# shoeffner/ann3depth

Hardware: AMD Instinct MI355X
Metric: images/sec (640x480->55x74 MSDN train step) (higher is better)
Workload: dtype f32

## Files before the change

### ann3depth_amd/_lib.py

```python
import ctypes
import os
from ctypes import c_char_p, c_float, c_int, c_int32, c_int64, c_size_t, c_uint8, c_uint32, c_void_p, POINTER

LIB_PATH = os.environ.get('A3D_LIB') or os.path.join(os.path.dirname(os.path.abspath(__file__)), 'liba3d.so')


class A3dError(RuntimeError):
    pass


class ConvDesc(ctypes.Structure):
    _fields_ = [(n, c_int32) for n in ('n', 'h', 'w', 'c', 'k', 'r', 's', 'stride', 'pad_t', 'pad_l', 'ho', 'wo',
                                       'ldx', 'ldy', 'precision', 'storage', 'hints')]


class SecondOutput(ctypes.Structure):
    _fields_ = [('ptr', c_void_p), ('ld', c_int32), ('step', c_int32), ('offset', c_int32), ('bf16', c_int32), ('cols', c_int32)]


class ExampleView(ctypes.Structure):
    _fields_ = [('image_height', c_int64), ('image_width', c_int64), ('image_channels', c_int64),
                ('depth_height', c_int64), ('depth_width', c_int64), ('depth_channels', c_int64),
                ('image', c_void_p), ('image_bytes', c_size_t), ('depth', c_void_p), ('depth_bytes', c_size_t)]


class TimingRecord(ctypes.Structure):
    _fields_ = [(n, c_int32) for n in ('mode', 'bm', 'bn', 'waves_m', 'nwaves', 'bk', 'avec', 'bvec', 'prec', 'lds_dma', 'splitk', 'm', 'n', 'k')] + \
               [('ms', c_float), ('flops', ctypes.c_double)]


_P = c_void_p
_D = POINTER(ConvDesc)

SIGNATURES = {
    'a3d_version': (c_char_p, []),
    'a3d_last_error': (c_int, [c_char_p, c_size_t]),
    'a3d_conv2d_fwd_ws_bytes': (c_size_t, [_D]),
    'a3d_conv2d_fwd': (c_int, [_D, _P, _P, _P, _P, c_int, _P, c_size_t, _P]),
    'a3d_conv2d_bwd_data_ws_bytes': (c_size_t, [_D]),
    'a3d_conv2d_bwd_data': (c_int, [_D, _P, _P, _P, _P, _P, c_size_t, _P]),
    'a3d_conv2d_bwd_filter_ws_bytes': (c_size_t, [_D]),
    'a3d_conv2d_bwd_filter': (c_int, [_D, _P, _P, _P, _P, _P, c_size_t, _P]),
    'a3d_conv2d_fwd_prepared_filter_bytes': (c_size_t, [_D]),
    'a3d_conv2d_fwd_prepare_filter': (c_int, [_D, _P, _P, c_size_t, _P]),
    'a3d_conv2d_bwd_filter_pooled_ws_bytes': (c_size_t, [_D]),
    'a3d_conv2d_bwd_filter_pooled': (c_int, [_D, _P, _P, c_int, _P, _P, c_int, c_int, _P, _P, _P, c_size_t, _P]),
    'a3d_conv2d_bwd_both_supported': (c_int, [_D]),
    'a3d_conv2d_bwd_both_ws_bytes': (c_size_t, [_D]),
    'a3d_conv2d_bwd_both': (c_int, [_D, _P, _P, _P, _P, _P, _P, c_int, c_int, c_int, _P, _P, c_size_t, _P]),
    'a3d_dense_fwd_ws_bytes': (c_size_t, [c_int, c_int, c_int]),
    'a3d_dense_fwd': (c_int, [c_int, c_int, c_int, _P, _P, _P, _P, c_int, _P, _P, c_size_t, _P]),
    'a3d_dense_bwd_data_ws_bytes': (c_size_t, [c_int, c_int, c_int]),
    'a3d_dense_bwd_data': (c_int, [c_int, c_int, c_int, _P, _P, _P, _P, c_int, c_float, _P, c_size_t, _P]),
    'a3d_dense_bwd_filter_ws_bytes': (c_size_t, [c_int, c_int, c_int]),
    'a3d_dense_bwd_filter': (c_int, [c_int, c_int, c_int, _P, _P, _P, _P, _P, c_size_t, _P]),
    'a3d_maxpool2x2_fwd': (c_int, [c_int, c_int, c_int, c_int, _P, _P, c_int, _P, _P]),
    'a3d_maxpool2x2_bwd': (c_int, [c_int, c_int, c_int, c_int, _P, _P, c_int, _P, c_int, _P]),
    'a3d_resize_bilinear_tf1': (c_int, [c_int, c_int, c_int, c_int, _P, c_int, c_int, _P, _P]),
    'a3d_resize_bilinear_tf1_pair': (c_int, [c_int, c_int, c_int, c_int, _P, c_int, c_int, _P, c_int, _P, c_int, c_int, _P, _P]),
    'a3d_resize_bilinear_tf1_ex': (c_int, [c_int, c_int, c_int, c_int, _P, c_int, c_int, c_int, _P, c_int, _P, c_int, c_int, c_int,
                                           _P, _P]),
    'a3d_warp_bilinear_pair': (c_int, [c_int, c_int, c_int, c_int, _P, c_int, c_int, c_int, _P, c_int, _P, c_int, c_int, c_int,
                                       _P, _P, _P]),
    'a3d_extract_patches': (c_int, [c_int, c_int, c_int, c_int, _P, c_int, c_int, _P, _P]),
    'a3d_silog_loss_fwd': (c_int, [c_int, c_int, _P, _P, _P, _P, _P]),
    'a3d_silog_loss_bwd': (c_int, [c_int, c_int, _P, _P, _P, _P, _P]),
    'a3d_dropout_keep_mask': (c_int, [c_size_t, ctypes.c_uint64, ctypes.c_uint64, c_float, _P, _P]),
    'a3d_adam_apply_tf1': (c_int, [c_size_t, _P, _P, _P, _P, c_float, c_float, c_float, c_float, c_float, c_float,
                                   c_float, _P]),
    'a3d_adam_apply_tf1_flag': (c_int, [c_size_t, _P, _P, _P, _P, c_float, c_float, c_float, c_float, c_float, c_float,
                                        c_float, _P, _P]),
    'a3d_dense_fwd_ex': (c_int, [c_int, c_int, c_int, _P, _P, _P, _P, c_int, _P, c_int, c_int, _P, c_size_t, _P]),
    'a3d_dense_bwd_data_ex': (c_int, [c_int, c_int, c_int, _P, _P, _P, _P, c_int, c_float, c_int, c_int, _P, c_size_t, _P]),
    'a3d_dense_fwd_ex2': (c_int, [c_int, c_int, c_int, _P, _P, _P, _P, c_int, c_int, c_int, _P, c_int, c_int, POINTER(SecondOutput), _P,
                                  c_size_t, _P]),
    'a3d_dense_bwd_data_ex2': (c_int, [c_int, c_int, c_int, _P, _P, _P, _P, c_int, c_float, c_int, c_int, POINTER(SecondOutput), _P,
                                       c_size_t, _P]),
    'a3d_conv2d_fwd_ex2': (c_int, [_D, _P, _P, _P, _P, c_int, POINTER(SecondOutput), _P, c_size_t, _P]),
    'a3d_silog_loss_bwd_ex': (c_int, [c_int, c_int, _P, _P, _P, _P, _P, c_int, _P]),
    'a3d_depth_metrics_ws_bytes': (c_size_t, [c_int, c_int, c_int]),
    'a3d_depth_metrics': (c_int, [c_int, c_int, c_int, _P, c_int, c_int, _P, c_int, c_float, c_float, c_float, c_float, _P, _P,
                                  c_size_t, _P]),
    'a3d_cast_bf16': (c_int, [c_size_t, _P, _P, c_int, _P]),
    'a3d_cast_rows': (c_int, [c_size_t, c_int, _P, c_int, c_int, _P, c_int, c_int, _P]),
    'a3d_pad_channels_bf16': (c_int, [c_size_t, c_int, _P, c_int, _P, _P]),
    'a3d_stream_create': (c_int, [c_int, ctypes.POINTER(ctypes.c_void_p)]),
    'a3d_stream_destroy': (c_int, [_P]),
    'a3d_maxpool2x2_fwd_bf16': (c_int, [c_int, c_int, c_int, c_int, _P, c_int, _P, c_int, _P, _P]),
    'a3d_maxpool2x2_bwd_bf16': (c_int, [c_int, c_int, c_int, c_int, _P, c_int, _P, c_int, _P, c_int, _P]),
    'a3d_copy_channel_bf16': (c_int, [c_size_t, _P, c_int, c_int, _P, c_int, c_int, _P]),
    'a3d_maxpool2x2_bwd_idx_bf16': (c_int, [c_int, c_int, c_int, c_int, _P, _P, c_int, _P, c_int, _P, c_int, _P]),
    'a3d_maxpool2x2_bwd_idx_bf16s': (c_int, [c_int, c_int, c_int, c_int, _P, _P, c_int, _P, c_int, _P, c_int, _P]),
    'a3d_dense_bwd_filter_adam_tf1': (c_int, [c_int, c_int, c_int, _P, _P, _P, _P, _P, _P, _P, _P, c_float, c_float, c_float,
                                              c_float, c_float, c_float, _P]),
    'a3d_dense_bwd_filter_adam_tf1_ex': (c_int, [c_int, c_int, c_int, _P, _P, _P, _P, _P, _P, _P, _P, c_float, c_float, c_float,
                                                 c_float, c_float, c_float, c_int, _P]),
    'a3d_superpixel_mean': (c_int, [c_int, c_int, c_int, c_int, _P, c_int, _P, _P]),
    'a3d_superpixel_hist': (c_int, [c_int, c_int, c_int, _P, c_int, _P, _P]),
    'a3d_pair_similarity': (c_int, [c_int, c_int, c_int, _P, c_int, _P, _P, _P, c_int, _P, _P, c_float, _P, _P, _P]),
    'a3d_crf_loss': (c_int, [c_int, c_int, _P, _P, _P, _P, _P, c_int, c_float, _P, _P, _P, _P]),
    'a3d_crf_map': (c_int, [c_int, c_int, _P, _P, _P, _P, c_int, _P, _P, _P]),
    'a3d_sgd_apply': (c_int, [c_size_t, _P, _P, c_float, _P]),
    'a3d_conv2d_pool_fwd': (c_int, [_D, _P, _P, _P, _P, c_int, _P, c_int, _P, c_size_t, _P]),
    'a3d_maxpool2x2_bwd_idx': (c_int, [c_int, c_int, c_int, c_int, _P, _P, c_int, _P, c_int, _P, c_int, _P]),
    'a3d_copy_channel': (c_int, [c_size_t, _P, c_int, c_int, _P, c_int, c_int, _P]),
    'a3d_comm_standin': (c_int, [_P, c_size_t, _P, c_size_t, c_int, c_float, _P]),
    'a3d_timing_enable': (c_int, [c_int]),
    'a3d_timing_collect': (c_int, [POINTER(TimingRecord), c_int]),
    'a3d_timing_select': (c_int, [POINTER(TimingRecord)]),
    'a3d_crc32c': (c_uint32, [_P, c_size_t]),
    'a3d_masked_crc32c': (c_uint32, [_P, c_size_t]),
    'a3d_tfrecord_next': (c_int, [_P, c_size_t, c_int, POINTER(c_size_t), POINTER(c_size_t), POINTER(c_size_t)]),
    'a3d_example_parse': (c_int, [_P, c_size_t, POINTER(ExampleView)]),
    'a3d_decode_raw_plus_half': (c_int, [_P, c_size_t, _P]),
    'a3d_record_decode': (c_int, [_P, c_size_t, c_int, _P, c_size_t, _P, c_size_t, POINTER(ExampleView)]),
    'a3d_record_decode_u8': (c_int, [_P, c_size_t, c_int, _P, _P, c_size_t, _P, _P, c_size_t, POINTER(ExampleView),
                                     POINTER(c_int)]),
    'a3d_records_decode': (c_int, [POINTER(c_void_p), POINTER(c_size_t), c_int, c_int, POINTER(c_int64), _P, _P, _P, _P,
                                   POINTER(c_int32), c_int, POINTER(c_int32)]),
    'a3d_h2d_gather': (c_int, [_P, _P, POINTER(c_int32), c_int, c_int, c_size_t, _P]),
    'a3d_sizeof_conv_desc': (c_size_t, []),
    'a3d_example_write': (c_int64, [_P, c_int, c_int, c_int, _P, c_int, c_int, c_int, _P, c_size_t]),
}

EXT_SIGNATURES = {
    'a3dx_resize_bilinear_tf1_valid': (c_int, [c_int, c_int, c_int, c_int, _P, c_int, c_int, c_int, _P, c_int, _P, c_int, c_int,
                                               c_int, _P, c_float, c_float, _P]),
    'a3dx_warp_bilinear_pair_valid': (c_int, [c_int, c_int, c_int, c_int, _P, c_int, c_int, c_int, _P, c_int, _P, c_int, c_int,
                                              c_int, _P, _P, c_float, c_float, _P]),
    'a3dx_silog_masked_loss_fwd': (c_int, [c_int, c_int, _P, _P, _P, _P, _P]),
    'a3dx_silog_masked_loss_bwd_ex': (c_int, [c_int, c_int, _P, _P, _P, _P, _P, c_int, _P]),
}

PAIR_SIGNATURES = {
    'a3dp_crf_loss_grad': (c_int, [c_int, c_int, _P, _P, _P, _P, _P, c_int, c_float, _P, _P, _P, _P, _P]),
    'a3dp_pair_dense_bwd': (c_int, [c_int, c_int, c_int, _P, _P, _P, _P, _P]),
    'a3dp_sgd_apply_floor': (c_int, [c_size_t, _P, _P, c_float, c_float, _P]),
}

TEXTURE_SIGNATURES = {
    'a3dt_superpixel_lbp_hist': (c_int, [c_int, c_int, c_int, _P, c_int, _P, _P]),
    'a3dt_pair_similarity3': (c_int, [c_int, c_int, c_int, _P, c_int, _P, _P, _P, _P, c_int, _P, _P, c_float, _P, _P, _P]),
}

GRADLOSS_SIGNATURES = {
    'a3dg_silog_grad_loss_fwd': (c_int, [c_int, c_int, c_int, _P, _P, c_int, c_float, _P, _P, _P]),
    'a3dg_silog_grad_loss_bwd_ex': (c_int, [c_int, c_int, c_int, _P, _P, c_int, c_float, _P, _P, _P, c_int, _P]),
}

CRF_VALID_SIGNATURES = {
    'a3dv_superpixel_mean_valid': (c_int, [c_int, c_int, c_int, _P, c_int, c_int, _P, _P, _P]),
    'a3dv_crf_loss_observed': (c_int, [c_int, c_int, _P, _P, _P, _P, _P, c_int, _P, _P, _P, _P, _P, _P, _P]),
}

FCSP_SIGNATURES = {
    'a3df_superpixel_pool_fwd': (c_int, [c_int, c_int, c_int, c_int, _P, c_int, c_int, c_int, c_int, _P, _P, _P, c_int, _P]),
    'a3df_superpixel_pool_bwd': (c_int, [c_int, c_int, c_int, c_int, _P, c_int, c_int, c_int, c_int, _P, _P, _P, c_int, _P]),
}

CRF_BAND_SIGNATURES = {
    'a3db_crf_band_nll': (c_int, [c_int, c_int, c_int, _P, _P, _P, _P, _P, c_int, _P, _P, _P, _P, _P, _P, _P]),
    'a3db_crf_band_map': (c_int, [c_int, c_int, c_int, _P, _P, _P, _P, c_int, _P, _P, _P]),
}

_lib = None


def load():
    global _lib
    if _lib is not None:
        return _lib
    if not os.path.exists(LIB_PATH):
        raise A3dError(f'{LIB_PATH} not found: build it with `python -c "import __graft_entry__ as g; g.build()"` '
                       f'or `make -C ann3depth_amd/csrc` (there is no fallback path)')
    import torch
    lib = ctypes.CDLL(LIB_PATH)
    for name, (res, args) in (list(SIGNATURES.items()) + list(EXT_SIGNATURES.items()) + list(PAIR_SIGNATURES.items())
                              + list(TEXTURE_SIGNATURES.items()) + list(GRADLOSS_SIGNATURES.items())
                              + list(CRF_VALID_SIGNATURES.items()) + list(FCSP_SIGNATURES.items())
                              + list(CRF_BAND_SIGNATURES.items())):
        try:
            fn = getattr(lib, name)
        except AttributeError as e:
            raise A3dError(f'liba3d.so lacks symbol {name}: stale build?') from e
        fn.restype = res
        fn.argtypes = args
    if lib.a3d_sizeof_conv_desc() != ctypes.sizeof(ConvDesc):
        raise A3dError(f'liba3d.so reads a {lib.a3d_sizeof_conv_desc()}-byte a3d_conv_desc, this binding passes '
                       f'{ctypes.sizeof(ConvDesc)} bytes: stale build?')
    _lib = lib
    return lib


def last_error():
    buf = ctypes.create_string_buffer(512)
    load().a3d_last_error(buf, 512)
    return buf.value.decode(errors='replace')


def check(rc, what):
    if rc != 0:
        raise A3dError(f'{what} failed ({rc}): {last_error()}')
```

### ann3depth_amd/csrc/a3d_internal.h

```cpp
#pragma once
#include <hip/hip_runtime.h>
#include <stddef.h>
#include <stdint.h>

#include <algorithm>

#include "../../include/a3d.h"
#include "igemm_plan.h"

namespace a3d {

int set_error(int code, const char* fmt, ...);

#define A3D_CHECK_ARG(cond, ...)                                 \
  do {                                                           \
    if (!(cond)) return ::a3d::set_error(A3D_EINVAL, __VA_ARGS__); \
  } while (0)

inline void clear_stale_error() { (void)hipGetLastError(); }

inline int check_launch(const char* what) {
  hipError_t e = hipGetLastError();
  if (e != hipSuccess) return set_error(A3D_ELAUNCH, "%s: %s", what, hipGetErrorString(e));
  return A3D_OK;
}

inline unsigned grid_for(size_t total, int per_block = 256, unsigned cap = 8192) {
  size_t g = (total + per_block - 1) / per_block;
  return (unsigned)std::min<size_t>(std::max<size_t>(g, 1), cap);
}

inline bool aligned16(const void* p) { return (reinterpret_cast<uintptr_t>(p) & 15) == 0; }

struct IgemmParams;
int launch_igemm(int mode, const GemmPlan& plan, int avec, int bvec, IgemmParams& p, void* ws, hipStream_t st);
int take_second_output(IgemmParams& p, const a3d_second_output* o);

struct TimingSlot {
  hipEvent_t start, stop;
  a3d_timing_record rec;
};
bool timing_wanted(const a3d_timing_record& r);
int timing_begin(TimingSlot& slot, hipStream_t st);
void timing_end(TimingSlot& slot, hipStream_t st);
a3d_timing_record timing_record(int mode, int prec, int bm, int bn, int waves_m, int nwaves, int bk, int avec, int bvec, int lds_dma,
                                int m, int n, int k);
template <typename Launch>
int timed_launch(const a3d_timing_record& rec, hipStream_t st, Launch&& launch) {
  if (!timing_wanted(rec)) return launch();
  TimingSlot slot{};
  slot.rec = rec;
  int rc = timing_begin(slot, st);
  if (rc != A3D_OK) return rc;
  rc = launch();
  timing_end(slot, st);
  return rc;
}

bool dense_dw_applicable(int m, int k, int n);
bool dense_stream_applicable(int m, int k, int n);
size_t dense_stream_ws_bytes(int m, int k, int n);
int dense_fwd_stream(int m, int k, int n, const float* x, const float* w, const float* bias, float* y, int act,
                     const uint8_t* keep, float keep_scale, void* ws, size_t ws_bytes, hipStream_t st);
struct ReduceParams;
int launch_splitk_reduce(const ReduceParams& r, hipStream_t st);
int dense_dw_launch(int m, int k, int n, const float* x, const float* dz, float* dw, float* db, hipStream_t st);

size_t colsum_bf16_ws_bytes(int n);
bool colsum_bf16_ok(int n);
int colsum_bf16(const void* dz, int rows, int n, int ld, float* out, void* ws, int* nparts, hipStream_t st);

bool stencil1_applicable(const a3d_conv_desc* d);
size_t stencil1_bwdf_ws_bytes(const a3d_conv_desc* d);
int stencil1_fwd(const a3d_conv_desc* d, const float* x, const float* w, const float* bias, float* y, int act,
                 hipStream_t st);
int stencil1_bwd_filter(const a3d_conv_desc* d, const float* x, const float* dz, float* dw, float* db, void* ws,
                        hipStream_t st);
bool stencil1_bwd_both_applicable(const a3d_conv_desc* d);
size_t stencil1_bwd_both_ws_bytes(const a3d_conv_desc* d);
int stencil1_bwd_both(const a3d_conv_desc* d, const float* x, const float* dz, const float* w, float* dw, float* db,
                      void* dx, int lddx, int dx_bf16, int relu_mask, unsigned* state, void* ws, hipStream_t st);

bool fewch_bwdf_applicable(const a3d_conv_desc* d, bool pooled);
size_t fewch_bwdf_ws_bytes(const a3d_conv_desc* d, bool pooled);
bool fewch_extents_ok(const a3d_conv_desc* d, bool pooled, int ldz, int esz, int ld_arg);
int fewch_bwd_filter(const a3d_conv_desc* d, const float* x, int src, const void* dz, int ldz, const void* pooled_act,
                     const uint8_t* argmax, int ld_arg, float* dw, float* db, void* ws, hipStream_t st);

int fewch_reduce_launch(const float* slabs, int splits, int Mp, int NP, int M, int N, float* dw, float* db, hipStream_t st);
bool fewch16_bwdf_applicable(const a3d_conv_desc* d, bool pooled);
size_t fewch16_bwdf_ws_bytes(const a3d_conv_desc* d, bool pooled);
int fewch16_bwd_filter(const a3d_conv_desc* d, const float* x, bool pooled, const void* dz, int ldz, const void* pooled_act,
                       const uint8_t* argmax, int ld_arg, float* dw, float* db, void* ws, hipStream_t st);

bool conv3_applicable(const a3d_conv_desc* d, unsigned x_off);
size_t conv3_ws_bytes(const a3d_conv_desc* d);
int conv3_pack(const a3d_conv_desc* d, const float* w, float* wp, hipStream_t st);
int conv3_fwd(const a3d_conv_desc* d, const float* x, const float* w, const float* bias, float* y, int act, int pool,
              int ld_out, uint8_t* argmax, void* ws, size_t ws_bytes, hipStream_t st, bool prepared = false);

bool conv3b_applicable(const a3d_conv_desc* d);
size_t conv3b_filter_bytes(const a3d_conv_desc* d);
int conv3b_pack(const a3d_conv_desc* d, const float* w, void* wp, hipStream_t st);
int conv3b_fwd(const a3d_conv_desc* d, const void* x, const float* w, const float* bias, void* y, int act, int pool, int ld_out,
               uint8_t* argmax, void* ws, size_t ws_bytes, hipStream_t st, bool prepared);

}
```

### ann3depth_amd/csrc/dense.hip

```cpp
#include <algorithm>
#include <cmath>
#include <cstdlib>

#include "a3d_internal.h"
#include "igemm.h"

namespace a3d {


template <int CW>
struct VecOf;
template <>
struct VecOf<4> { typedef float type __attribute__((ext_vector_type(4), aligned(4))); };
template <>
struct VecOf<2> { typedef float type __attribute__((ext_vector_type(2), aligned(4))); };

template <bool ADAM, int CW>
__global__ __launch_bounds__(256) void dense_dw_kernel(const float* __restrict__ x, const float* __restrict__ dz,
                                                       float* __restrict__ dw, float* __restrict__ db,
                                                       float* __restrict__ var_w, float* __restrict__ m_w,
                                                       float* __restrict__ v_w, float* __restrict__ var_b,
                                                       float* __restrict__ m_b, float* __restrict__ v_b, int M, int K,
                                                       int N, float omb1, float gscale) {
  typedef typename VecOf<CW>::type vec;
// ... 390 lines not shown
      m_b[col] = mn;
      const bool poison = !isfinite(__fmul_rn(g, g));
      if (poison) v_b[col] = qnan;
      if (poison || !isfinite(mn)) var_b[col] = qnan;
    }
  }
  __syncthreads();

  for (int g = g0; g < g1; ++g) {
    f32x16 acc[G][CW];
#pragma unroll
    for (int gq = 0; gq < G; ++gq)
#pragma unroll
      for (int j = 0; j < CW; ++j)
#pragma unroll
        for (int v = 0; v < 16; ++v) acc[gq][j][v] = 0.f;
    if constexpr (BF) {
#pragma unroll
      for (int t = 0; t < 4; ++t) {
        const dbf16x8 a = *reinterpret_cast<const dbf16x8*>(&xsb[li * XLD + 16 * t + 8 * lh]);
#pragma unroll
        for (int gq = 0; gq < G; ++gq)
#pragma unroll
          for (int j = 0; j < CW; ++j)
            acc[gq][j] = __builtin_amdgcn_mfma_f32_32x32x16_bf16(a, bqb[t][gq][j], acc[gq][j], 0, 0, 0);
      }
    } else {
#pragma unroll
    for (int u = 0; u < TSTEPS; ++u) {
      const float a = xs[(2 * u + lh) * 32 + li];
#pragma unroll
      for (int gq = 0; gq < G; ++gq)
#pragma unroll
        for (int j = 0; j < CW; ++j)
          acc[gq][j] = __builtin_amdgcn_mfma_f32_32x32x2f32(a, bq[u][gq][j], acc[gq][j], 0, 0, 0);
    }
    }
#pragma unroll
    for (int hh = 0; hh < 2; ++hh) {
      if (hh) __syncthreads();
#pragma unroll
      for (int gq = 0; gq < G; ++gq)
#pragma unroll
        for (int vv = 0; vv < 8; ++vv) {
          vec t;
#pragma unroll
          for (int j = 0; j < CW; ++j) t[j] = acc[gq][j][8 * hh + vv];
          *reinterpret_cast<vec*>(&tile[((vv & 3) + 8 * (vv >> 2) + 4 * lh) * TLD + wave * WCOLS + (32 * gq + li) * CW]) = t;
        }
      __syncthreads();
      if (hh == 0) {
        load_x(xv, g + 1);
        __builtin_amdgcn_sched_barrier(0);
      }
#pragma unroll
      for (int r = 4 * hh; r < 4 * hh + 4; ++r) {
        const __amdgpu_buffer_rsrc_t rr = row_rsrc(g, r), rn = row_rsrc(g + 1, r);
        const int row = 32 * g + wrow(r);
#pragma unroll
        for (int h = 0; h < NI; ++h) {
          const int c = (h * 64 + lane) * CW;
          const vec g4 = *reinterpret_cast<const vec*>(&tile[(4 * wave + (r & 3)) * TLD + c]);
          const uint32_t off = piece_off(h);
          uvec mn;
          float chk = 0.f;
#pragma unroll
          for (int j = 0; j < CW; ++j) {
            const float gr = use_scale ? __fmul_rn(g4[j], gscale) : g4[j];
            const float mo = mreg[NI * r + h][j];
            const float t = __fadd_rn(mo, __fmul_rn(__fsub_rn(gr, mo), omb1));
            mn[j] = __float_as_uint(t);
            chk += __fmul_rn(gr, gr) + fabsf(t);
          }
          if constexpr (CW == 4) __builtin_amdgcn_raw_buffer_store_b128(mn, rr, (int)off, 0, kAuxStream);
          else __builtin_amdgcn_raw_buffer_store_b64(mn, rr, (int)off, 0, kAuxStream);
          load_vec_buf<CW, kAuxStream>(rn, off, mreg[NI * r + h]);
          if (!isfinite(chk) & (off != kOOB) & (row < K)) {
#pragma unroll
            for (int j = 0; j < CW; ++j) {
              const float gr = use_scale ? __fmul_rn(g4[j], gscale) : g4[j];
              const bool poison = !isfinite(__fmul_rn(gr, gr));
              const size_t o = (size_t)row * N + nb + c + j;
              if (poison) v_w[o] = qnan;
              if (poison || !isfinite(__uint_as_float(mn[j]))) var_w[o] = qnan;
            }
          }
        }
      }
    }
    park_x(xv);
    __syncthreads();
  }
}

typedef float f32x4a __attribute__((ext_vector_type(4), aligned(4)));

struct DenseStreamParams {
  const float* x;
  const float* w;
  float* out;
  const float* bias;
  const uint8_t* keep;
  const float* mask;
  float scale;
  int act;
  int M, K, N, splits, span;
};

template <int MB>
__global__ __launch_bounds__(256) void dense_fwd_stream_kernel(const DenseStreamParams p) {
  __shared__ __attribute__((aligned(16))) float red[4 * 16 * 132];
  const int tid = threadIdx.x, lane = tid & 63, wave = tid >> 6, li = lane & 31, lh = lane >> 5;
  const int n0 = blockIdx.x * 128, split = blockIdx.y;
  const int kb0 = split * p.span, kb1 = min(p.K, kb0 + p.span);
  const int wspan = ((kb1 - kb0 + 3) / 4 + 15) / 16 * 16;
  const int k0 = kb0 + wave * wspan, k1 = min(kb1, k0 + wspan);
  const __amdgpu_buffer_rsrc_t rw = make_rsrc(p.w, (unsigned long long)p.K * p.N * 4ull);
  const __amdgpu_buffer_rsrc_t rx = make_rsrc(p.x, (unsigned long long)p.M * p.K * 4ull);
  const int col0 = n0 + 4 * li;

  f32x16 acc[MB][4];
#pragma unroll
  for (int b = 0; b < MB; ++b)
#pragma unroll
    for (int c = 0; c < 4; ++c)
#pragma unroll
      for (int v = 0; v < 16; ++v) acc[b][c][v] = 0.f;

  constexpr int U = MB == 1 ? 2 : 1, ROWS = 8 * U;
  struct Chunk { float w[U][4][4]; float a[MB][U][4]; };
  auto load = [&](Chunk& c, int kc) {
#pragma unroll
    for (int u = 0; u < U; ++u) {
#pragma unroll
      for (int j = 0; j < 4; ++j) {
        const int k = kc + 8 * u + 4 * lh + j;
        load_vec_buf<4, kAuxStream>(rw, ((k < k1) & (col0 < p.N)) ? (uint32_t)(((size_t)k * p.N + col0) * 4) : kOOB, c.w[u][j]);
      }
#pragma unroll
      for (int b = 0; b < MB; ++b) {
        const int m = 32 * b + li, k = kc + 8 * u + 4 * lh;
        load_vec_buf<4>(rx, ((m < p.M) & (k < k1)) ? (uint32_t)(((size_t)m * p.K + k) * 4) : kOOB, c.a[b][u]);
      }
    }
  };
  auto compute = [&](const Chunk& c) {
#pragma unroll
    for (int u = 0; u < U; ++u)
#pragma unroll
      for (int j = 0; j < 4; ++j)
#pragma unroll
        for (int b = 0; b < MB; ++b)
#pragma unroll
          for (int e = 0; e < 4; ++e)
            acc[b][e] = __builtin_amdgcn_mfma_f32_32x32x2f32(c.a[b][u][j], c.w[u][j][e], acc[b][e], 0, 0, 0);
  };
  if (k0 < k1) {
    Chunk ca, cb;
    load(ca, k0);
    for (int kc = k0; kc < k1; kc += 2 * ROWS) {
      load(cb, kc + ROWS);
      compute(ca);
      load(ca, kc + 2 * ROWS);
      compute(cb);
    }
  }

#pragma unroll
  for (int b = 0; b < MB; ++b) {
#pragma unroll
    for (int hh = 0; hh < 2; ++hh) {
      if (b || hh) __syncthreads();
      float* mine = red + wave * (16 * 132);
#pragma unroll
      for (int vv = 0; vv < 8; ++vv) {
        const int v = 8 * hh + vv;
        const f32x4 q = {acc[b][0][v], acc[b][1][v], acc[b][2][v], acc[b][3][v]};
        *reinterpret_cast<f32x4*>(mine + ((vv & 3) + 8 * (vv >> 2) + 4 * lh) * 132 + 4 * li) = q;
      }
      __syncthreads();
      float sv[4][2];
      bool okv[4][2];
#pragma unroll
      for (int r = 0; r < 4; ++r) {
        const int lr = wave * 4 + r, m = 32 * b + 16 * hh + lr;
#pragma unroll
        for (int h = 0; h < 2; ++h) {
          const int c = lane + 64 * h;
          okv[r][h] = m < p.M && n0 + c < p.N;
          float s = red[lr * 132 + c];
          s += red[(16 + lr) * 132 + c];
          s += red[(32 + lr) * 132 + c];
          s += red[(48 + lr) * 132 + c];
          sv[r][h] = s;
        }
      }
      if (p.splits > 1) {
#pragma unroll
        for (int r = 0; r < 4; ++r)
#pragma unroll
          for (int h = 0; h < 2; ++h)
            if (okv[r][h]) p.out[((size_t)split * p.M + 32 * b + 16 * hh + wave * 4 + r) * p.N + n0 + lane + 64 * h] = sv[r][h];
      } else {
        float bias[2] = {0.f, 0.f};
        uint8_t kp[4][2];
#pragma unroll
        for (int h = 0; h < 2; ++h)
          if (p.bias && n0 + lane + 64 * h < p.N) bias[h] = p.bias[n0 + lane + 64 * h];
        if (p.keep) {
#pragma unroll
          for (int r = 0; r < 4; ++r)
#pragma unroll
            for (int h = 0; h < 2; ++h)
              kp[r][h] = okv[r][h] ? p.keep[(size_t)(32 * b + 16 * hh + wave * 4 + r) * p.N + n0 + lane + 64 * h] : (uint8_t)0;
        }
#pragma unroll
        for (int r = 0; r < 4; ++r)
#pragma unroll
          for (int h = 0; h < 2; ++h) {
            float s = sv[r][h];
            if (p.bias) s += bias[h];
            if (p.act == EPI_RELU) s = fmaxf(s, 0.f);
            else if (p.act == EPI_SIGMOID) s = 1.f / (1.f + expf(-s));
            if (p.keep) s = kp[r][h] ? s * p.scale : 0.f;
            sv[r][h] = s;
          }
#pragma unroll
        for (int r = 0; r < 4; ++r)
#pragma unroll
          for (int h = 0; h < 2; ++h)
            if (okv[r][h]) p.out[(size_t)(32 * b + 16 * hh + wave * 4 + r) * p.N + n0 + lane + 64 * h] = sv[r][h];
      }
    }
  }
}

static int pick_span(int extent, int groups, int quantum) {
  const int target = 512;
  const int want = std::max(1, target / std::max(1, groups));
  int span = (extent + want - 1) / want;
  span = std::max(quantum, (span + quantum - 1) / quantum * quantum);
  return span;
}
bool dense_stream_applicable(int m, int k, int n) {
  return m >= 1 && m <= 64 && (long)k * n >= (1L << 20) && k % 4 == 0;
}
size_t dense_stream_ws_bytes(int m, int k, int n) {
  if (!dense_stream_applicable(m, k, n)) return 0;
  const int sf = pick_span(k, (n + 127) / 128, 64);
  return (size_t)((k + sf - 1) / sf) * m * n * 4;
}
int dense_fwd_stream(int m, int k, int n, const float* x, const float* w, const float* bias, float* y, int act,
                     const uint8_t* keep, float keep_scale, void* ws, size_t ws_bytes, hipStream_t st) {
  DenseStreamParams p{};
  p.x = x; p.w = w; p.bias = bias; p.keep = keep; p.scale = keep_scale; p.act = act; p.M = m; p.K = k; p.N = n;
  p.span = pick_span(k, (n + 127) / 128, 64);
  p.splits = (k + p.span - 1) / p.span;
  if (p.splits > 1 && (size_t)p.splits * m * n * 4 > ws_bytes) return set_error(A3D_EWORKSPACE, "dense_fwd: workspace too small");
  p.out = p.splits > 1 ? static_cast<float*>(ws) : y;
  clear_stale_error();
  const dim3 grid((n + 127) / 128, p.splits);
  if (m <= 32) hipLaunchKernelGGL(dense_fwd_stream_kernel<1>, grid, dim3(256), 0, st, p);
  else hipLaunchKernelGGL(dense_fwd_stream_kernel<2>, grid, dim3(256), 0, st, p);
  int rc = check_launch("dense_fwd_stream");
  if (rc != A3D_OK || p.splits == 1) return rc;
  ReduceParams r{};
  r.ws = p.out; r.C = y; r.bias = bias; r.keep = keep; r.mask_scale = keep_scale; r.M = m; r.N = n; r.ldc = n;
  r.splitk = p.splits; r.act = act; r.mode = MODE_FWD; r.slab = (size_t)m * n; r.sub_step = 1;
  r.div_phw = make_fastdiv(1); r.div_pw = make_fastdiv(1);
  return launch_splitk_reduce(r, st);
}
bool dense_dw_applicable(int m, int k, int n) { return m >= 1 && m <= 64 && k >= 1 && n >= 1; }

int dense_dw_launch(int m, int k, int n, const float* x, const float* dz, float* dw, float* db, hipStream_t st) {
  clear_stale_error();
  hipLaunchKernelGGL((dense_dw_kernel<false, 4>), dim3((n + 127) / 128, (k + 127) / 128), dim3(256), 0, st, x, dz, dw, db,
                     nullptr, nullptr, nullptr, nullptr, nullptr, nullptr, m, k, n, 0.f, 1.f);
  return check_launch("dense_dw");
}

}

using namespace a3d;

#ifdef A3D_STAMPS
extern "C" int a3d_debug_dense_stamps(unsigned long long* out, size_t bytes) {
  (void)hipDeviceSynchronize();
  return (int)hipMemcpyFromSymbol(out, HIP_SYMBOL(g_dense_stamps), std::min(bytes, sizeof(g_dense_stamps)));
}
#endif

extern "C" int a3d_dense_bwd_filter_adam_tf1(int m, int k, int n, const float* x, const float* dz, float* var_w, float* m_w,
                                             float* v_w, float* var_b, float* m_b, float* v_b, float lr, float beta1,
                                             float beta2, float beta1_power, float beta2_power, float grad_scale,
                                             void* stream) {
  return a3d_dense_bwd_filter_adam_tf1_ex(m, k, n, x, dz, var_w, m_w, v_w, var_b, m_b, v_b, lr, beta1, beta2, beta1_power,
                                          beta2_power, grad_scale, A3D_PREC_F32, stream);
}

extern "C" int a3d_dense_bwd_filter_adam_tf1_ex(int m, int k, int n, const float* x, const float* dz, float* var_w, float* m_w,
                                                float* v_w, float* var_b, float* m_b, float* v_b, float lr, float beta1,
                                                float beta2, float beta1_power, float beta2_power, float grad_scale,
                                                int precision, void* stream) {
  A3D_CHECK_ARG(precision == A3D_PREC_F32 || precision == A3D_PREC_BF16, "dense_bwd_filter_adam: precision %d (float32 or bf16)", precision);
  A3D_CHECK_ARG(m > 0 && k > 0 && n > 0 && x && dz && var_w && m_w && v_w, "dense_bwd_filter_adam: bad arguments");
  A3D_CHECK_ARG((var_b && m_b && v_b) || (!var_b && !m_b && !v_b), "dense_bwd_filter_adam: bias slots come as a set");
  A3D_CHECK_ARG(dense_dw_applicable(m, k, n), "dense_bwd_filter_adam: batches of at most 64 rows only");
  const float alpha = lr * sqrtf(1.f - beta2_power) / (1.f - beta1_power);
  A3D_CHECK_ARG(alpha == 0.f && 1.f - beta2 == 0.f,
                "dense_bwd_filter_adam: only the reference's frozen optimizer (beta2 == 1); otherwise call "
                "a3d_dense_bwd_filter and a3d_adam_apply_tf1");
  clear_stale_error();
  const uintptr_t slots = reinterpret_cast<uintptr_t>(m_w) | reinterpret_cast<uintptr_t>(dz) | reinterpret_cast<uintptr_t>(var_w) |
                          reinterpret_cast<uintptr_t>(v_w);
  const dim3 rows_grid((n + 511) / 512, (k + 31) / 32);
  static const bool no_stream = tune_int("A3D_NO_DENSE_STREAM", 0) != 0;
  const bool slim = m <= 32 && n % 2 == 0;
  const bool bf_cols = precision == A3D_PREC_BF16 && m > 32;
  const int bcols = slim ? 256 : ((m <= 32 || bf_cols) ? 512 : 256), colblocks = (n + bcols - 1) / bcols;
  const int gpb = std::max(1, ((k + 31) / 32 * colblocks + (slim ? 1023 : 511)) / (slim ? 1024 : 512));
  const dim3 stream_grid(colblocks, ((k + 31) / 32 + gpb - 1) / gpb);
  const bool stream_ok = m <= 64 && k % 4 == 0 && (reinterpret_cast<uintptr_t>(x) & 15) == 0 && !no_stream;
  const hipStream_t hst = static_cast<hipStream_t>(stream);
#define A3D_DW_STREAM(CWV, MBV, ...)                                                                                     \
  hipLaunchKernelGGL((dense_dw_adam_stream_kernel<CWV, MBV, ##__VA_ARGS__>), stream_grid, dim3(256), 0, hst, x, dz, var_w, m_w, v_w, var_b, \
                     m_b, v_b, m, k, n, 1.f - beta1, grad_scale, gpb)
  const bool bf = precision == A3D_PREC_BF16 && m > 32 && stream_ok;
  if (bf && n % 4 == 0 && (slots & 15) == 0) A3D_DW_STREAM(4, 2, 1, true);
  else if (bf && n % 2 == 0 && (slots & 7) == 0) A3D_DW_STREAM(2, 2, 1, true);
  else if (stream_ok && slim && (slots & 7) == 0) A3D_DW_STREAM(2, 1, 2);
  else if (stream_ok && m <= 32 && n % 4 == 0 && (slots & 15) == 0) A3D_DW_STREAM(4, 1);
  else if (stream_ok && m <= 32 && n % 2 == 0 && (slots & 7) == 0) A3D_DW_STREAM(2, 1);
  else if (stream_ok && n % 2 == 0 && (slots & 7) == 0) A3D_DW_STREAM(2, 2);
#undef A3D_DW_STREAM
  else if (n % 4 == 0 && (slots & 15) == 0)
    hipLaunchKernelGGL(dense_dw_adam_rows_kernel<4>, rows_grid, dim3(256), 0, static_cast<hipStream_t>(stream), x, dz, var_w,
                       m_w, v_w, var_b, m_b, v_b, m, k, n, 1.f - beta1, grad_scale);
  else if (n % 2 == 0 && (slots & 7) == 0)
    hipLaunchKernelGGL(dense_dw_adam_rows_kernel<2>, rows_grid, dim3(256), 0, static_cast<hipStream_t>(stream), x, dz, var_w,
                       m_w, v_w, var_b, m_b, v_b, m, k, n, 1.f - beta1, grad_scale);
  else
    hipLaunchKernelGGL((dense_dw_kernel<true, 4>), dim3((n + 127) / 128, (k + 127) / 128), dim3(256), 0,
                       static_cast<hipStream_t>(stream), x, dz, nullptr, nullptr, var_w, m_w, v_w, var_b, m_b, v_b, m, k, n,
                       1.f - beta1, grad_scale);
  return check_launch("dense_dw_adam");
}
```

### ann3depth_amd/csrc/igemm_host.hip

```cpp
#include <algorithm>

#include "a3d_internal.h"
#include "igemm.h"
#include "igemm_cfgs.h"

namespace a3d {

int launch_igemm_multi_bwd_d(int avec, int bvec, IgemmMulti& ps, unsigned grid_x, unsigned count, hipStream_t st);
int launch_igemm_bf16_multi_bwd_d(int bn, IgemmMulti& ps, unsigned grid_x, unsigned count, hipStream_t st);


struct RunForm {
  int vec;
  int rl, rlp;
  int kp;
  int np;
  size_t bytes;
};
static bool run_form_ok(const a3d_conv_desc* d, unsigned x_off, RunForm* rf, bool bwd_filter = false) {
  if (d->pad_t || d->pad_l || d->ldx != d->c || d->c % 4 == 0 || d->c > 4) return false;
  const int step = d->stride * d->c, row = d->w * d->c;
  int vec = 0;
  bool anywhere = false;
  if (step % 4 == 0 && row % 4 == 0 && x_off == 0) vec = 4;
  else if (step % 2 == 0 && row % 2 == 0 && (x_off & 7) == 0) vec = 2;
  else if (bwd_filter && d->precision == A3D_PREC_F32 && !d->storage && (x_off & 3) == 0) {
    vec = 2;
    anywhere = true;
  }
  if (vec == 4 && d->precision == A3D_PREC_F32) {
    const int rl = d->s * d->c;
    const int kp4 = d->r * ((rl + 3) / 4 * 4), kp2 = d->r * ((rl + 1) / 2 * 2);
    if ((kp2 + 127) / 128 < (kp4 + 127) / 128) vec = 2;
  }
  if (!vec) return false;
  rf->vec = vec;
  rf->rl = d->s * d->c;
  rf->rlp = (rf->rl + vec - 1) / vec * vec;
  rf->kp = d->r * rf->rlp;
  rf->np = (d->k + 3) / 4 * 4;
  rf->bytes = ((size_t)rf->kp * rf->np * 4 + 255) / 256 * 256;
  if (anywhere) return (d->wo - 1) * step + rf->rl <= row && (d->ho - 1) * d->stride + d->r <= d->h;
  return (d->wo - 1) * step + rf->rlp <= row;
}

__global__ __launch_bounds__(256) void pad_filter_kernel(const float* w, float* wp, int r, int rl, int rlp, int n, int np) {
  const int total = r * rlp * np;
  for (int i = blockIdx.x * 256 + threadIdx.x; i < total; i += gridDim.x * 256) {
    const int col = i % np, row = i / np;
    const int q = row % rlp, rr = row / rlp;
    wp[i] = (q < rl && col < n) ? w[(size_t)(rr * rl + q) * n + col] : 0.f;
  }
}
__global__ __launch_bounds__(256) void unpad_filter_kernel(const float* wp, float* w, int r, int rl, int rlp, int n) {
  const int total = r * rl * n;
  for (int i = blockIdx.x * 256 + threadIdx.x; i < total; i += gridDim.x * 256) {
    const int col = i % n, row = i / n;
    const int q = row % rl, rr = row / rl;
    w[i] = wp[(size_t)(rr * rlp + q) * n + col];
  }
}

struct Operands {
  bool known = false;
  unsigned x = 0, w = 0, y = 0;
  unsigned aux = 0;
  int act = A3D_ACT_NONE, pool = 0, ld_out = 0;
  bool argmax = false, prepared = false;
  bool db = true;
};
static const Operands kOnGrid{};
static Operands launch_operands(const void* x, const void* w, const void* y, const void* aux) {
  auto off16 = [](const void* p) { return (unsigned)(reinterpret_cast<uintptr_t>(p) & 15); };
  Operands o;
  o.known = true;
  o.x = off16(x); o.w = off16(w); o.y = off16(y); o.aux = off16(aux);
  return o;
}

enum GemmForm { kAsStored, kLdsDma, kRunForm, kBf16Image };
struct Route {
  bool ok = false;
  RunForm rf{};
  GemmProblem g{};
  GemmPlan plan{};
  size_t repack = 0;
  size_t bytes = 0;
};
static size_t upto(size_t need, const Route& r) { return r.ok ? std::max(need, r.bytes) : need; }
static void fit_workspace(Route& r, const Operands& o, size_t ws_bytes, size_t per_split = 0) {
  if (r.bytes <= ws_bytes || !(o.x | o.w | o.y | o.aux) || r.repack > ws_bytes) return;
  r.plan = plan_within(r.g, r.plan, ws_bytes - r.repack, per_split);
  r.bytes = r.repack + r.plan.ws_bytes + (r.plan.splitk > 1 ? (size_t)r.plan.splitk * per_split : 0);
}
#define A3D_CHECK_WS(ws, who) A3D_CHECK_ARG(aligned16(ws), who ": ws must be 16-byte aligned")

static const int kAll16 = A3D_STORE_X_BF16 | A3D_STORE_W_BF16 | A3D_STORE_Y_BF16;
static bool stored16(const a3d_conv_desc* d, int bits) { return (d->storage & bits) == bits; }
static bool ring_ok(const a3d_conv_desc* d, const Operands& o, int both, unsigned out_off, int taps) {
  if (d->precision != A3D_PREC_BF16 || !stored16(d, both) || d->c % 8 || d->k % 8) return false;
  return !o.known || (d->ldx % 8 == 0 && d->ldy % 8 == 0 && taps <= 128 && !out_off);
}

static int ilog2_exact(int v) {
  for (int l = 0; l < 8; ++l)
    if ((1 << l) == v) return l;
  return -1;
}

static int check_desc(const a3d_conv_desc* d) {
  A3D_CHECK_ARG(d != nullptr, "conv: null descriptor");
  A3D_CHECK_ARG(d->n > 0 && d->h > 0 && d->w > 0 && d->c > 0 && d->k > 0 && d->r > 0 && d->s > 0, "conv: bad dims");
  A3D_CHECK_ARG(ilog2_exact(d->stride) >= 0 && d->stride <= 4, "conv: stride %d unsupported (1, 2 or 4)", d->stride);
  A3D_CHECK_ARG(d->pad_t >= 0 && d->pad_l >= 0 && d->pad_t < d->r && d->pad_l < d->s, "conv: bad padding");
  A3D_CHECK_ARG(d->ho > 0 && d->wo > 0, "conv: bad output size");
  A3D_CHECK_ARG((d->ho - 1) * d->stride - d->pad_t < d->h && (d->wo - 1) * d->stride - d->pad_l < d->w,
                "conv: output size inconsistent with input");
  A3D_CHECK_ARG(d->ldx >= d->c && d->ldy >= d->k, "conv: pixel strides smaller than channel counts");
  A3D_CHECK_ARG(d->precision >= A3D_PREC_F32 && d->precision <= A3D_PREC_BF16, "conv: unknown precision %d", d->precision);
  const double lim = 2147483647.0;
  A3D_CHECK_ARG((double)d->n * d->h * d->w * d->ldx < lim && (double)d->n * d->ho * d->wo * d->ldy < lim &&
                    (double)d->r * d->s * d->c * d->k < lim,
                "conv: tensor too large for 31-bit indexing");
  return A3D_OK;
}

static GemmProblem fwd_problem(const a3d_conv_desc* d) {
  GemmProblem g;
  g.mode = MODE_FWD;
  g.M = d->n * d->ho * d->wo; g.N = d->k; g.K = d->r * d->s * d->c;
  g.avec = (d->c % 4 == 0 && d->ldx % 4 == 0) ? 4 : 1;
  g.bvec = (d->k % 4 == 0) ? 4 : 1;
  return g;
}
static GemmProblem bwd_d_problem(const a3d_conv_desc* d) {
  GemmProblem g;
  g.mode = MODE_BWD_D;
  g.M = d->n * d->h * d->w; g.N = d->c; g.K = d->r * d->s * d->k;
  g.avec = (d->k % 4 == 0 && d->ldy % 4 == 0) ? 4 : 1;
  g.bvec = (d->k % 4 == 0) ? 4 : 1;
  return g;
}
static GemmProblem bwd_f_problem(const a3d_conv_desc* d) {
  GemmProblem g;
  g.mode = MODE_BWD_F;
  g.M = d->r * d->s * d->c; g.N = d->k; g.K = d->n * d->ho * d->wo;
  g.avec = (d->c % 4 == 0 && d->ldx % 4 == 0) ? 4 : 1;
  g.bvec = (d->k % 4 == 0 && d->ldy % 4 == 0) ? 4 : 1;
  return g;
}

static void storage_vecs(GemmProblem& g, bool a16, bool b16, bool c16) {
  if (c16) g.no_glds = 1;
  if (a16) g.avec = 4;
  if (b16) g.bvec = 4;
}
static int apply_storage(IgemmParams& p, int precision, bool a16, bool b16, bool c16, int a_c, int a_ld, int b_c, int b_ld,
                         const void* a, const void* b, const void* c, const char* an, const char* bn, const char* cn) {
  if (!a16 && !b16 && !c16) return A3D_OK;
  A3D_CHECK_ARG(precision == A3D_PREC_BF16 || (precision == A3D_PREC_F32 && !a16 && !b16),
                "bf16 operands need precision A3D_PREC_BF16");
  A3D_CHECK_ARG(!a16 || (a_c % 8 == 0 && a_ld % 8 == 0 && aligned16(a)), "bf16 %s: channels / stride must be multiples of 8, base 16-byte aligned", an);
  A3D_CHECK_ARG(!b16 || ((b_c < 0 || b_c % 8 == 0) && b_ld % 8 == 0 && aligned16(b)), "bf16 %s: channels / stride must be multiples of 8, base 16-byte aligned", bn);
  A3D_CHECK_ARG(!c16 || aligned16(c), "bf16 %s: base must be 16-byte aligned", cn);
  p.a16 = a16; p.b16 = b16; p.c16 = c16;
  return A3D_OK;
}

static void fill_common(IgemmParams& p, const GemmProblem& g) {
  p = IgemmParams{};
  p.M = g.M; p.N = g.N; p.K = g.K;
  p.mask_scale = 1.f;
  p.mask_act = EPI_RELU;
  p.sub_step = 1;
}

static void fill_staging(IgemmParams& p, int mode, unsigned long long a_elems, unsigned long long b_elems, int taps_r,
                         int taps_s) {
  p.a_elems = a_elems;
  p.b_elems = b_elems;
  p.ntaps = std::max(1, taps_r * taps_s);
  p.cpt = std::max(1, p.Cg / 32);
  p.uni = (mode != MODE_BWD_F) && p.Cg % 32 == 0 && p.K == p.ntaps * p.Cg;
  p.kperm = p.uni && p.ntaps > 1 && p.cpt > 1;
  p.div_cpt = make_fastdiv(p.cpt);
  p.div_taps = make_fastdiv(p.ntaps);
  p.cpt64 = std::max(1, p.Cg / 64);
  p.uni64 = p.uni && p.Cg % 64 == 0;
  p.kperm64 = p.uni64 && p.ntaps > 1 && p.cpt64 > 1;
  p.div_cpt64 = make_fastdiv(p.cpt64);
}

static void fill_gather(IgemmParams& p, const a3d_conv_desc* d, int ld, int S, int Cg) {
  p.H = d->h; p.W = d->w; p.ld = ld; p.pHW = d->h * d->w;
  p.stride = d->stride; p.lstride = ilog2_exact(d->stride); p.pad_t = d->pad_t; p.pad_l = d->pad_l;
  p.S = S; p.Cg = Cg;
  p.div_phw = make_fastdiv(d->ho * d->wo); p.div_pw = make_fastdiv(d->wo);
  p.div_c = make_fastdiv(Cg); p.div_s = make_fastdiv(S);
  p.div_c_half = make_fastdiv(std::max(1, Cg / 2));
}
static void fill_pool(IgemmParams& p, const a3d_conv_desc* d, uint8_t* argmax, int ld_out) {
  const int ph = d->ho / 2, pw = d->wo / 2;
  p.pool = 1;
  p.argmax = argmax;
  p.div_phw = make_fastdiv(ph * pw * 4); p.div_pw = make_fastdiv(pw);
  p.ldc = ld_out;
}

static int fwd_rows(const a3d_conv_desc* d, int pool) {
  return pool ? d->n * (d->ho / 2) * (d->wo / 2) * 4 : d->n * d->ho * d->wo;
}

static a3d_timing_record conv3_record(const a3d_conv_desc* d, int m) {
  return timing_record(MODE_FWD, A3D_PREC_F32, 64, d->k > 64 ? 96 : 64, 1, 1, 8, 4, 4, 2, m, d->k, d->r * d->s * d->c);
}
static a3d_timing_record conv3b_record(const a3d_conv_desc* d, int m) {
  return timing_record(MODE_FWD, A3D_PREC_BF16, 64, d->k > 64 ? 96 : 64, 1, 1, 16, 4, 4, 2, m, d->k, d->r * d->s * 3);
}
static a3d_timing_record fewch_record(const a3d_conv_desc* d) {
  return timing_record(MODE_BWD_F, A3D_PREC_F32, 128, (d->k + 31) / 32 * 32, 4, 4, 2, 1, 1, 4, d->r * d->s * d->c, d->k, d->n * d->ho * d->wo);
}
static a3d_timing_record fewch16_record(const a3d_conv_desc* d) {
  return timing_record(MODE_BWD_F, A3D_PREC_BF16, 128, (d->k + 31) / 32 * 32, 4, 4, 16, 1, 1, 4, d->r * d->s * d->c, d->k, d->n * d->ho * d->wo);
}

static bool bf16_image_form_ok(const a3d_conv_desc* d, const Operands& o, RunForm* rf) {
  rf->vec = 4;
  rf->rl = d->s * 4;
  rf->rlp = (d->s * 2 + 3) / 4 * 4 * 2;
  rf->kp = d->r * rf->rlp;
  rf->np = (d->k + 7) / 8 * 8;
  rf->bytes = ((size_t)rf->kp * rf->np * 2 + 255) / 256 * 256;
  if (!(d->storage & A3D_STORE_X_BF16) || d->c != 4 || d->ldx != 4) return false;
  if (!o.known) return true;
  if ((d->storage & A3D_STORE_W_BF16) || d->precision != A3D_PREC_BF16) return false;
  if (d->pad_t || d->pad_l || d->stride % 2 || (d->w * 2) % 4 || o.x) return false;
  return (d->wo - 1) * d->stride * 2 + rf->rlp / 2 <= d->w * 2;
}
__global__ __launch_bounds__(256) void pad_filter_bf16_kernel(const float* w, __bf16* wp, int r, int rl, int rlp, int n, int np) {
  const int total = r * rlp * np;
  for (int i = blockIdx.x * 256 + threadIdx.x; i < total; i += gridDim.x * 256) {
    const int col = i % np, row = i / np;
    const int q = row % rlp, rr = row / rlp;
    wp[i] = (__bf16)((q < rl && col < n) ? w[(size_t)(rr * rl + q) * n + col] : 0.f);
  }
}
static int pad_filter(const a3d_conv_desc* d, const RunForm& rf, bool bf16, const float* w, void* wp, hipStream_t st) {
  const dim3 grid((rf.kp * rf.np + 255) / 256), block(256);
  clear_stale_error();
  if (bf16)
    hipLaunchKernelGGL(pad_filter_bf16_kernel, grid, block, 0, st, w, static_cast<__bf16*>(wp), d->r, rf.rl, rf.rlp, d->k, rf.np);
  else
    hipLaunchKernelGGL(pad_filter_kernel, grid, block, 0, st, w, static_cast<float*>(wp), d->r, rf.rl, rf.rlp, d->k, rf.np);
  return check_launch(bf16 ? "pad_filter_bf16" : "pad_filter");
}

static bool fwd_form_ok(const a3d_conv_desc* d, const Operands& o, GemmForm form, RunForm* rf) {
  if (form == kRunForm) return run_form_ok(d, o.x, rf);
  if (form == kBf16Image) return bf16_image_form_ok(d, o, rf);
  if (form == kAsStored || !ring_ok(d, o, A3D_STORE_X_BF16 | A3D_STORE_W_BF16, o.y, d->r * d->s)) return form == kAsStored;
  return !o.known || (o.act != A3D_ACT_SIGMOID && (!o.pool || ((d->storage & A3D_STORE_Y_BF16) && o.ld_out % 8 == 0 &&
                                                               (!o.argmax || (d->k % 16 == 0 && !o.aux)))));
}
static Route fwd_gemm(const a3d_conv_desc* d, const Operands& o, GemmForm form) {
  Route r;
  if (!(r.ok = fwd_form_ok(d, o, form, &r.rf))) return r;
  GemmProblem& g = r.g;
  g = fwd_problem(d);
  g.M = fwd_rows(d, o.pool); g.plain = o.pool ? 1 : 0;
  if (o.x) g.avec = 1;
  if (o.w) g.bvec = 1;
  if (form == kRunForm || form == kBf16Image) {
    g.K = r.rf.kp; g.avec = r.rf.vec;
    if (!o.prepared) r.repack = r.rf.bytes;
  }
  if (form == kBf16Image) { g.bvec = 4; g.no_glds = 1; }
  if (form == kLdsDma) { g.ring_ok = 1; g.avec = g.bvec = 4; }
  if (o.known) {
    if (d->hints & A3D_HINT_SHARE_CU) g.no_glds = 1;
    if (form == kRunForm) g.bvec = 4;
    storage_vecs(g, d->storage & A3D_STORE_X_BF16, d->storage & A3D_STORE_W_BF16, d->storage & A3D_STORE_Y_BF16);
  }
  r.plan = plan_gemm(g, d->precision);
  r.bytes = r.repack + r.plan.ws_bytes;
  return r;
}

}

using namespace a3d;

extern "C" {

size_t a3d_conv2d_fwd_ws_bytes(const a3d_conv_desc* d) {
  if (check_desc(d) != A3D_OK || stencil1_applicable(d)) return 0;
  size_t need = 0;
  for (GemmForm form : {kAsStored, kLdsDma, kRunForm, kBf16Image}) need = upto(need, fwd_gemm(d, kOnGrid, form));
  RunForm rf;
  if (bf16_image_form_ok(d, kOnGrid, &rf)) need = std::max(need, conv3b_filter_bytes(d));
  if (conv3_applicable(d, kOnGrid.x)) need = std::max(need, conv3_ws_bytes(d));
  return need;
}

static int conv_fwd_impl(const a3d_conv_desc* d, const float* x, const float* w, const float* bias, float* y, int act,
                         int pool, int ld_out, uint8_t* argmax, void* ws, size_t ws_bytes, void* stream,
                         const a3d_second_output* out2 = nullptr) {
  int rc = check_desc(d);
  if (rc != A3D_OK) return rc;
  if (!ws) ws_bytes = 0;
  Operands o = launch_operands(x, w, y, argmax);
  o.act = act; o.pool = pool; o.ld_out = ld_out; o.argmax = argmax != nullptr;
  o.prepared = (d->hints & A3D_HINT_W_PREPARED) != 0;
  RunForm rf;
  const bool image = fwd_form_ok(d, o, kBf16Image, &rf);
  A3D_CHECK_ARG(!(out2 && out2->ptr) || (!pool && !stencil1_applicable(d) && !image && !conv3_applicable(d, o.x)),
                "conv2d_fwd_ex2: a second output on the implicit-GEMM forwards only (no fused pool, no few-channel / one-filter kernels)");
  A3D_CHECK_ARG(x && w && y, "conv2d_fwd: null tensor");
  A3D_CHECK_WS(ws, "conv2d_fwd");
  A3D_CHECK_ARG(act == A3D_ACT_NONE || act == A3D_ACT_RELU || act == A3D_ACT_SIGMOID, "conv2d_fwd: bad act");
  if (pool) {
    A3D_CHECK_ARG(d->precision == A3D_PREC_F32 || image ||
                      (d->precision == A3D_PREC_BF16 && (stored16(d, kAll16) || d->storage == A3D_STORE_Y_BF16)),
                  "conv2d_pool_fwd: fp32, the bf16 image form (4-channel bf16 image, a3d_pad_channels_bf16), or bf16 arithmetic on "
                  "bf16 x, w and y (LDS-DMA kernel)");
    A3D_CHECK_ARG(d->ho >= 2 && d->wo >= 2 && ld_out >= d->k, "conv2d_pool_fwd: output smaller than one pool window");
    A3D_CHECK_ARG(!stencil1_applicable(d), "conv2d_pool_fwd: single-output-channel convs are not supported");
  } else if (stencil1_applicable(d)) {
    A3D_CHECK_ARG(!d->storage, "conv2d_fwd: single-output-channel convs take float32 tensors");
    return stencil1_fwd(d, x, w, bias, y, act, static_cast<hipStream_t>(stream));
  }
  hipStream_t st = static_cast<hipStream_t>(stream);
  if (image && conv3b_applicable(d))
    return timed_launch(conv3b_record(d, fwd_rows(d, pool)), st,
                        [&] { return conv3b_fwd(d, x, w, bias, y, act, pool, ld_out, argmax, ws, ws_bytes, st, o.prepared); });
  if (!image && conv3_applicable(d, o.x))
    return timed_launch(conv3_record(d, fwd_rows(d, pool)), st,
                        [&] { return conv3_fwd(d, x, w, bias, y, act, pool, ld_out, argmax, ws, ws_bytes, st, o.prepared); });
  const bool run = !image && fwd_form_ok(d, o, kRunForm, &rf) && (o.prepared || rf.bytes <= ws_bytes), padded = run || image;
  Route r = fwd_gemm(d, o, image ? kBf16Image : run ? kRunForm : fwd_form_ok(d, o, kLdsDma, &rf) ? kLdsDma : kAsStored);
  fit_workspace(r, o, ws_bytes);
  A3D_CHECK_ARG(!o.prepared || (padded && !o.w && !o.x),
                "conv2d_fwd: A3D_HINT_W_PREPARED on a launch that reads the filter as stored, or with x off the 16-byte grid");
  IgemmParams p;
  fill_common(p, r.g);
  const int sb = d->storage;
  if (image) {
    p.a16 = 1; p.b16 = 1; p.c16 = (sb & A3D_STORE_Y_BF16) ? 1 : 0;
  } else {
    A3D_CHECK_ARG(!sb || ((!pool || sb == A3D_STORE_Y_BF16 || (sb == kAll16 && d->precision == A3D_PREC_BF16)) &&
                          !(run && (sb & A3D_STORE_W_BF16))),
                  "conv2d_fwd: the fused pool takes float32 inputs (its output may be bf16) or bf16 x, w and y; 3-channel filters stay float32");
    rc = apply_storage(p, d->precision, sb & A3D_STORE_X_BF16, sb & A3D_STORE_W_BF16, sb & A3D_STORE_Y_BF16, d->c, d->ldx, d->k, d->k,
                       x, w, y, "x", "w", "y");
    if (rc != A3D_OK) return rc;
    A3D_CHECK_ARG(!(pool && (p.a16 || p.b16)) || r.plan.ring,
                  "conv2d_pool_fwd: on bf16 inputs the fused pool is the LDS-DMA kernel's (channels and strides in whole 16-byte pieces, k %% 16 == 0)");
  }
  if (r.bytes > ws_bytes) return set_error(A3D_EWORKSPACE, "conv2d_fwd: need %zu workspace bytes", r.bytes);
  A3D_CHECK_ARG(!image || (r.plan.prec == A3D_PREC_BF16 && !o.y), "conv2d_fwd: bf16 image form needs the bf16 kernel");
  A3D_CHECK_ARG(!(p.a16 || p.b16) || r.plan.prec == A3D_PREC_BF16, "conv2d_fwd: bf16 operands need vectorisable tensors");
  A3D_CHECK_ARG(!p.c16 || r.plan.prec == A3D_PREC_BF16 || !is_glds_cfg(r.plan.cfg), "conv2d_fwd: no bf16 output from the LDS-DMA kernels");
  const float* filter = w;
  if (padded && !o.prepared) {
    rc = pad_filter(d, r.rf, image, w, ws, st);
    if (rc != A3D_OK) return rc;
    filter = static_cast<const float*>(ws);
  }
  const int ldb = padded ? r.rf.np : d->k;
  p.A = x; p.B = filter; p.C = y; p.bias = bias; p.act = act;
  p.share = (d->hints & A3D_HINT_SHARE_CU) ? 1 : 0;
  p.npix = r.g.M; p.nrsc = r.g.K;
  fill_gather(p, d, d->ldx, padded ? 1 : d->s, padded ? r.rf.rlp : d->c);
  p.ldb = ldb; p.ldc = d->ldy;
  if (pool) fill_pool(p, d, argmax, ld_out);
  fill_staging(p, MODE_FWD, (unsigned long long)d->n * d->h * d->w * d->ldx, (unsigned long long)r.g.K * ldb, d->r, padded ? 1 : d->s);
  rc = take_second_output(p, out2);
  if (rc != A3D_OK) return rc;
  return launch_igemm(MODE_FWD, r.plan, r.g.avec, r.g.bvec, p, static_cast<char*>(ws) + r.repack, st);
}

int a3d_conv2d_fwd(const a3d_conv_desc* d, const float* x, const float* w, const float* bias, float* y, int act,
                   void* ws, size_t ws_bytes, void* stream) {
  return conv_fwd_impl(d, x, w, bias, y, act, 0, 0, nullptr, ws, ws_bytes, stream);
}

static int fwd_filter_form(const a3d_conv_desc* d, RunForm* rf) {
  if (check_desc(d) != A3D_OK || stencil1_applicable(d)) return 0;
  const Operands o = launch_operands(nullptr, nullptr, nullptr, nullptr);
  if (bf16_image_form_ok(d, o, rf)) return 1;
  if (conv3_applicable(d, o.x)) return 2;
  if (run_form_ok(d, o.x, rf)) return 3;
  return 0;
}

size_t a3d_conv2d_fwd_prepared_filter_bytes(const a3d_conv_desc* d) {
  RunForm rf{};
  switch (fwd_filter_form(d, &rf)) {
    case 1: return conv3b_applicable(d) ? conv3b_filter_bytes(d) : rf.bytes;
    case 2: return conv3_ws_bytes(d);
    case 3: return rf.bytes;
    default: return 0;
  }
}

int a3d_conv2d_fwd_prepare_filter(const a3d_conv_desc* d, const float* w, void* prepared, size_t prepared_bytes, void* stream) {
  int rc = check_desc(d);
  if (rc != A3D_OK) return rc;
  A3D_CHECK_ARG(w && prepared && aligned16(prepared), "conv2d_fwd_prepare_filter: null or misaligned buffer");
  const size_t need = a3d_conv2d_fwd_prepared_filter_bytes(d);
  A3D_CHECK_ARG(need > 0, "conv2d_fwd_prepare_filter: this forward reads the filter as stored");
  if (prepared_bytes < need) return set_error(A3D_EWORKSPACE, "conv2d_fwd_prepare_filter: need %zu bytes", need);
  hipStream_t st = static_cast<hipStream_t>(stream);
  RunForm rf{};
  switch (fwd_filter_form(d, &rf)) {
    case 1: return conv3b_applicable(d) ? conv3b_pack(d, w, prepared, st) : pad_filter(d, rf, true, w, prepared, st);
    case 2: return conv3_pack(d, w, static_cast<float*>(prepared), st);
    default: return pad_filter(d, rf, false, w, prepared, st);
  }
}

int a3d_conv2d_fwd_ex2(const a3d_conv_desc* d, const float* x, const float* w, const float* bias, float* y, int act,
                       const a3d_second_output* out2, void* ws, size_t ws_bytes, void* stream) {
  return conv_fwd_impl(d, x, w, bias, y, act, 0, 0, nullptr, ws, ws_bytes, stream, out2);
}

int a3d_conv2d_pool_fwd(const a3d_conv_desc* d, const float* x, const float* w, const float* bias, float* y_pooled,
                        int ld_pooled, uint8_t* argmax, int act, void* ws, size_t ws_bytes, void* stream) {
  return conv_fwd_impl(d, x, w, bias, y_pooled, act, 1, ld_pooled, argmax, ws, ws_bytes, stream);
}

struct BwdDClass {
  int ph, pw, hc, wc, r0, s0, rp, sp, off_y, off_x;
  GemmProblem g;
};
static bool bwd_d_class(const a3d_conv_desc* d, int ph, int pw, BwdDClass* c) {
  const int st = d->stride;
  c->ph = ph; c->pw = pw;
  c->hc = (d->h - ph + st - 1) / st;
  c->wc = (d->w - pw + st - 1) / st;
  if (c->hc <= 0 || c->wc <= 0) return false;
  c->r0 = (ph + d->pad_t) % st;
  c->s0 = (pw + d->pad_l) % st;
  c->rp = c->r0 < d->r ? (d->r - c->r0 + st - 1) / st : 0;
  c->sp = c->s0 < d->s ? (d->s - c->s0 + st - 1) / st : 0;
  c->off_y = (ph + d->pad_t - c->r0) / st;
  c->off_x = (pw + d->pad_l - c->s0) / st;
  c->g = bwd_d_problem(d);
  c->g.M = d->n * c->hc * c->wc;
  c->g.K = c->rp * c->sp * d->k;
  return true;
}
static int bwd_d_classes(const a3d_conv_desc* d, BwdDClass (&cls)[16]) {
  int n = 0;
  for (int ph = 0; ph < d->stride; ++ph)
    for (int pw = 0; pw < d->stride; ++pw)
      if (bwd_d_class(d, ph, pw, &cls[n])) ++n;
  return n;
}

static Route bwd_d_gemm(const a3d_conv_desc* d, const BwdDClass& c, const Operands& o, GemmForm form, const GemmPlan* tiles = nullptr) {
  Route r;
  r.ok = form == kAsStored || (d->stride == 1 && !o.aux && ring_ok(d, o, A3D_STORE_Y_BF16 | A3D_STORE_W_BF16, o.x, c.rp * c.sp));
  if (!r.ok) return r;
  r.g = c.g;
  if (o.y) r.g.avec = 1;
  if (o.w) r.g.bvec = 1;
  if (form == kLdsDma) { r.g.ring_ok = 1; r.g.avec = r.g.bvec = 4; }
  if (o.known) storage_vecs(r.g, d->storage & A3D_STORE_Y_BF16, d->storage & A3D_STORE_W_BF16, d->storage & A3D_STORE_X_BF16);
  r.plan = tiles ? *tiles : plan_gemm(r.g, d->precision);
  r.bytes = r.plan.ws_bytes;
  return r;
}

size_t a3d_conv2d_bwd_data_ws_bytes(const a3d_conv_desc* d) {
  if (check_desc(d) != A3D_OK) return 0;
  BwdDClass cls[16];
  const int ncls = bwd_d_classes(d, cls);
  size_t need = 0;
  for (int i = 0; i < ncls; ++i)
    for (GemmForm form : {kAsStored, kLdsDma}) need = upto(need, bwd_d_gemm(d, cls[i], kOnGrid, form));
  return need;
}

static void fill_bwd_d_class(IgemmParams& p, const a3d_conv_desc* d, const BwdDClass& c, const float* dz, const float* w, float* dx,
                             const float* relu_mask) {
  p.A = dz; p.B = w; p.C = dx; p.mask = relu_mask;
  p.npix = p.M; p.nrsc = p.K;
  p.H = d->ho; p.W = d->wo; p.ld = d->ldy; p.pHW = d->ho * d->wo;
  p.stride = 1; p.lstride = 0; p.pad_t = c.off_y; p.pad_l = c.off_x;
  p.S = std::max(c.sp, 1); p.Cg = d->k; p.Cn = d->c;
  p.div_phw = make_fastdiv(c.hc * c.wc); p.div_pw = make_fastdiv(c.wc);
  p.div_c = make_fastdiv(d->k); p.div_s = make_fastdiv(std::max(c.sp, 1));
  p.div_c_half = make_fastdiv(std::max(1, d->k / 2));
  p.ldb = 0; p.ldc = d->ldx;
  p.sub_step = d->stride; p.sub_ph = c.ph; p.sub_pw = c.pw; p.tap_r0 = c.r0; p.tap_s0 = c.s0; p.S_full = d->s;
  p.outW = d->w; p.outHW = d->h * d->w;
  fill_staging(p, MODE_BWD_D, (unsigned long long)d->n * d->ho * d->wo * d->ldy, (unsigned long long)d->r * d->s * d->c * d->k, c.rp,
               c.sp);
}

int a3d_conv2d_bwd_data(const a3d_conv_desc* d, const float* dz, const float* w, float* dx, const float* relu_mask,
                        void* ws, size_t ws_bytes, void* stream) {
  int rc = check_desc(d);
  if (rc != A3D_OK) return rc;
  A3D_CHECK_ARG(dz && w && dx, "conv2d_bwd_data: null tensor");
  A3D_CHECK_WS(ws, "conv2d_bwd_data");
  if (!ws) ws_bytes = 0;
  const Operands o = launch_operands(dx, w, dz, relu_mask);
  hipStream_t st = static_cast<hipStream_t>(stream);
  BwdDClass cls[16];
  const int ncls = bwd_d_classes(d, cls);
  long tiles64 = 0;
  for (int i = 0; i < ncls; ++i) tiles64 += (long)((cls[i].g.M + 63) / 64) * ((cls[i].g.N + 63) / 64);
  const bool multi32 = d->stride == 2 && d->precision == A3D_PREC_F32 && !d->storage && tune_int("A3D_FORCE_CFG", -1) < 0 && tiles64 >= 256;
  const bool multi16 = d->stride == 2 && d->precision == A3D_PREC_BF16 && stored16(d, kAll16) && !o.y && !o.w &&
                       tune_int("A3D_FORCE_SPLITK", 0) <= 0;
  IgemmMulti multi;
  int avec = 4, bvec = 4, multi16_bn = 0;
  unsigned multi_grid = 0;
  double multi_flops = 0;
  for (int i = 0; i < ncls; ++i) {
    const BwdDClass& c = cls[i];
    GemmPlan tiles64{};
    tiles64.cfg = 4; tiles64.splitk = 1; tiles64.ktiles_per_split = std::max(1, (c.g.K + 31) / 32);
    tiles64.tiles_m = (c.g.M + 63) / 64; tiles64.tiles_n = (c.g.N + 63) / 64;
    Route r = bwd_d_gemm(d, c, o, kLdsDma);
    if (!r.ok) r = bwd_d_gemm(d, c, o, kAsStored, multi32 ? &tiles64 : nullptr);
    IgemmParams p;
    fill_common(p, r.g);
    rc = apply_storage(p, d->precision, d->storage & A3D_STORE_Y_BF16, d->storage & A3D_STORE_W_BF16, d->storage & A3D_STORE_X_BF16,
                       d->k, d->ldy, d->k, d->k, dz, w, dx, "dz", "w", "dx");
    if (rc != A3D_OK) return rc;
    A3D_CHECK_ARG(!p.c16 || !o.aux, "conv2d_bwd_data: bf16 mask must be 16-byte aligned");
    A3D_CHECK_ARG(!d->storage || r.plan.prec == A3D_PREC_BF16, "conv2d_bwd_data: bf16 storage needs vectorisable operands");
    if (multi16) {
      multi16_bn = r.plan.bf16_bn;
      r.plan.splitk = 1; r.plan.ktiles_per_split = std::max(1, (r.g.K + 63) / 64);
    } else if (!multi32) {
      fit_workspace(r, o, ws_bytes);
      if (r.bytes > ws_bytes) return set_error(A3D_EWORKSPACE, "conv2d_bwd_data: need %zu workspace bytes", r.bytes);
    }
    fill_bwd_d_class(p, d, c, dz, w, dx, relu_mask);
    if (!multi32 && !multi16) {
      rc = launch_igemm(MODE_BWD_D, r.plan, r.g.avec, r.g.bvec, p, ws, st);
      if (rc != A3D_OK) return rc;
      continue;
    }
    p.splitk = 1; p.ktiles_per_split = r.plan.ktiles_per_split; p.tiles_m = r.plan.tiles_m; p.tiles_n = r.plan.tiles_n;
    p.slab = (size_t)p.M * p.N;
    multi.p[i] = p;
    avec = std::min(avec, r.g.avec); bvec = std::min(bvec, r.g.bvec);
    multi_grid = std::max(multi_grid, (unsigned)((long)r.plan.tiles_m * r.plan.tiles_n));
    multi_flops += 2.0 * p.M * p.N * p.K;
  }
  if (!multi32 && !multi16) return A3D_OK;
  a3d_timing_record rec = multi16 ? timing_record(MODE_BWD_D, A3D_PREC_BF16, 128, multi16_bn, 4, 8, 64, 4, 4, 0, d->n * d->h * d->w, d->c,
                                                  d->r * d->s * d->k)
                                  : timing_record(MODE_BWD_D, A3D_PREC_F32, 64, 64, 2, 4, 32, avec, bvec, 0, d->n * d->h * d->w, d->c,
                                                  d->r * d->s * d->k);
  rec.flops = multi_flops;
  return timed_launch(rec, st, [&] {
    return multi16 ? launch_igemm_bf16_multi_bwd_d(multi16_bn, multi, multi_grid, (unsigned)ncls, st)
                   : launch_igemm_multi_bwd_d(avec, bvec, multi, multi_grid, (unsigned)ncls, st);
  });
}

static bool bwd_f_ring_ok(const a3d_conv_desc* d, const Operands& o) {
  return d->precision == A3D_PREC_BF16 && stored16(d, A3D_STORE_X_BF16 | A3D_STORE_Y_BF16) && d->c % 8 == 0 && d->ldx % 8 == 0 &&
         d->k % 8 == 0 && d->ldy % 8 == 0 && (double)d->n * d->h * d->w * d->ldx * 2.0 < 2147483647.0 && colsum_bf16_ok(d->k) &&
         d->ldy == d->k && !o.w;
}
static Route bwd_f_gemm(const a3d_conv_desc* d, const Operands& o, GemmForm form) {
  Route r;
  r.ok = form == kRunForm ? run_form_ok(d, o.x, &r.rf, true) : form == kLdsDma ? bwd_f_ring_ok(d, o) : true;
  if (!r.ok) return r;
  GemmProblem& g = r.g;
  g = bwd_f_problem(d);
  if (o.x) g.avec = 1;
  if (o.y) g.bvec = 1;
  if (form == kRunForm) {
    g.M = r.rf.kp; g.avec = r.rf.vec;
    r.repack = r.rf.bytes;
  }
  if (o.known) storage_vecs(g, d->storage & A3D_STORE_X_BF16, d->storage & A3D_STORE_Y_BF16, false);
  g.ring_ok = form == kLdsDma;
  r.plan = plan_gemm(g, d->precision);
  if (r.plan.ring) r.bytes = r.plan.ws_bytes + (o.db ? colsum_bf16_ws_bytes(d->k) : 0);
  else r.bytes = r.repack + r.plan.ws_bytes + (r.plan.splitk > 1 && o.db ? (size_t)r.plan.splitk * g.N * 4 : 0);
  return r;
}

int a3d_conv2d_bwd_both_supported(const a3d_conv_desc* d) {
  return check_desc(d) == A3D_OK && !d->storage && stencil1_bwd_both_applicable(d);
}

size_t a3d_conv2d_bwd_both_ws_bytes(const a3d_conv_desc* d) {
  return a3d_conv2d_bwd_both_supported(d) ? stencil1_bwd_both_ws_bytes(d) : 0;
}

int a3d_conv2d_bwd_both(const a3d_conv_desc* d, const float* x, const float* dz, const float* w, float* dw, float* db,
                        void* dx, int lddx, int dx_bf16, int relu_mask, uint32_t* state, void* ws, size_t ws_bytes,
                        void* stream) {
  int rc = check_desc(d);
  if (rc != A3D_OK) return rc;
  A3D_CHECK_ARG(x && dz && w && dw && dx && state, "conv2d_bwd_both: null tensor");
  A3D_CHECK_ARG(a3d_conv2d_bwd_both_supported(d),
                "conv2d_bwd_both: one output channel, 5x5, stride 1, an even channel count <= 64, float32 tensors, x below 1 GiB");
  A3D_CHECK_ARG(lddx >= d->c && lddx % 2 == 0, "conv2d_bwd_both: lddx must be even and >= c");
  A3D_CHECK_ARG((reinterpret_cast<uintptr_t>(x) & 7) == 0 && (reinterpret_cast<uintptr_t>(w) & 7) == 0 &&
                    (reinterpret_cast<uintptr_t>(dx) & (dx_bf16 ? 3 : 7)) == 0 && (reinterpret_cast<uintptr_t>(ws) & 3) == 0,
                "conv2d_bwd_both: x, w and dx must be aligned to a channel pair");
  if (stencil1_bwd_both_ws_bytes(d) > ws_bytes) return set_error(A3D_EWORKSPACE, "conv2d_bwd_both: workspace too small");
  return stencil1_bwd_both(d, x, dz, w, dw, db, dx, lddx, dx_bf16, relu_mask, state, ws, static_cast<hipStream_t>(stream));
}

static bool fewch_wanted(const a3d_conv_desc* d, bool pooled) {
  return !d->storage && fewch_bwdf_applicable(d, pooled) && tune_int("A3D_FEWCH", 1) != 0;
}

static int fewch_timed(const a3d_conv_desc* d, const float* x, int src, const void* dz, int ldz, const void* pooled_act,
                       const uint8_t* argmax, int ld_arg, float* dw, float* db, void* ws, hipStream_t st) {
  return timed_launch(fewch_record(d), st, [&] { return fewch_bwd_filter(d, x, src, dz, ldz, pooled_act, argmax, ld_arg, dw, db, ws, st); });
}

static bool fewch16_wanted(const a3d_conv_desc* d, bool pooled) {
  return !d->storage && fewch16_bwdf_applicable(d, pooled) && tune_int("A3D_FEWCH16", 1) != 0;
}

static bool fewch_pooled_ok(const a3d_conv_desc* d) { return !d->storage && fewch_bwdf_applicable(d, true); }

size_t a3d_conv2d_bwd_filter_pooled_ws_bytes(const a3d_conv_desc* d) {
  if (check_desc(d) != A3D_OK) return 0;
  if (fewch16_wanted(d, true)) return fewch16_bwdf_ws_bytes(d, true);
  return fewch_pooled_ok(d) ? fewch_bwdf_ws_bytes(d, true) : 0;
}

int a3d_conv2d_bwd_filter_pooled(const a3d_conv_desc* d, const float* x, const void* dpool, int ld_dpool, const void* pooled,
                                 const uint8_t* argmax, int ld_argmax, int pooled_bf16, float* dw, float* db, void* ws,
                                 size_t ws_bytes, void* stream) {
  int rc = check_desc(d);
  if (rc != A3D_OK) return rc;
  A3D_CHECK_ARG(x && dpool && argmax && dw, "conv2d_bwd_filter_pooled: null tensor");
  A3D_CHECK_WS(ws, "conv2d_bwd_filter_pooled");
  if (fewch16_wanted(d, true)) {
    A3D_CHECK_ARG(pooled_bf16 && ld_dpool >= d->k && ld_argmax >= d->k && ld_dpool % 4 == 0 &&
                      (reinterpret_cast<uintptr_t>(dpool) & 7) == 0 && (reinterpret_cast<uintptr_t>(pooled) & 7) == 0 &&
                      (reinterpret_cast<uintptr_t>(x) & 15) == 0,
                  "conv2d_bwd_filter_pooled: bf16 arithmetic takes bf16 pooled tensors in whole aligned 4-channel groups");
    A3D_CHECK_ARG(fewch_extents_ok(d, true, ld_dpool, 2, ld_argmax), "conv2d_bwd_filter_pooled: pooled tensors of 2 GiB or more");
    if (fewch16_bwdf_ws_bytes(d, true) > ws_bytes) return set_error(A3D_EWORKSPACE, "conv2d_bwd_filter_pooled: workspace too small");
    hipStream_t st = static_cast<hipStream_t>(stream);
    return timed_launch(fewch16_record(d), st,
                        [&] { return fewch16_bwd_filter(d, x, true, dpool, ld_dpool, pooled, argmax, ld_argmax, dw, db, ws, st); });
  }
  A3D_CHECK_ARG(fewch_pooled_ok(d),
                "conv2d_bwd_filter_pooled: an unpadded conv of <= 4 densely packed float32 input channels and 33..96 filters (fp32 "
                "arithmetic; or bf16 arithmetic with bf16 pooled tensors)");
  A3D_CHECK_ARG(ld_dpool >= d->k && ld_argmax >= d->k, "conv2d_bwd_filter_pooled: pixel strides below the filter count");
  A3D_CHECK_ARG(ld_dpool % 4 == 0 && aligned16(x) && (reinterpret_cast<uintptr_t>(dpool) & (pooled_bf16 ? 7 : 15)) == 0 &&
                    (reinterpret_cast<uintptr_t>(pooled) & (pooled_bf16 ? 7 : 15)) == 0,
                "conv2d_bwd_filter_pooled: x, dpool and pooled in whole aligned 4-channel groups (ld_dpool % 4 == 0)");
  A3D_CHECK_ARG(fewch_extents_ok(d, true, ld_dpool, pooled_bf16 ? 2 : 4, ld_argmax), "conv2d_bwd_filter_pooled: pooled tensors of 2 GiB or more");
  if (fewch_bwdf_ws_bytes(d, true) > ws_bytes) return set_error(A3D_EWORKSPACE, "conv2d_bwd_filter_pooled: workspace too small");
  return fewch_timed(d, x, pooled_bf16 ? 2 : 1, dpool, ld_dpool, pooled, argmax, ld_argmax, dw, db, ws,
                     static_cast<hipStream_t>(stream));
}

size_t a3d_conv2d_bwd_filter_ws_bytes(const a3d_conv_desc* d) {
  if (check_desc(d) != A3D_OK) return 0;
  if (stencil1_applicable(d)) return stencil1_bwdf_ws_bytes(d);
  size_t need = fewch_wanted(d, false) ? fewch_bwdf_ws_bytes(d, false) : 0;
  for (GemmForm form : {kAsStored, kLdsDma, kRunForm}) need = upto(need, bwd_f_gemm(d, kOnGrid, form));
  return need;
}

int a3d_conv2d_bwd_filter(const a3d_conv_desc* d, const float* x, const float* dz, float* dw, float* db, void* ws,
                          size_t ws_bytes, void* stream) {
  int rc = check_desc(d);
  if (rc != A3D_OK) return rc;
  A3D_CHECK_ARG(x && dz && dw, "conv2d_bwd_filter: null tensor");
  A3D_CHECK_WS(ws, "conv2d_bwd_filter");
  if (!ws) ws_bytes = 0;
  if (stencil1_applicable(d)) {
    A3D_CHECK_ARG(!d->storage, "conv2d_bwd_filter: single-output-channel convs take float32 tensors");
    if (stencil1_bwdf_ws_bytes(d) > ws_bytes) return set_error(A3D_EWORKSPACE, "conv2d_bwd_filter: workspace too small");
    return stencil1_bwd_filter(d, x, dz, dw, db, ws, static_cast<hipStream_t>(stream));
  }
  if (fewch_wanted(d, false) && aligned16(x) && fewch_extents_ok(d, false, d->ldy, 4, 0)) {
    if (fewch_bwdf_ws_bytes(d, false) > ws_bytes) return set_error(A3D_EWORKSPACE, "conv2d_bwd_filter: workspace too small");
    return fewch_timed(d, x, 0, dz, d->ldy, nullptr, nullptr, 0, dw, db, ws, static_cast<hipStream_t>(stream));
  }
  Operands o = launch_operands(x, dw, dz, nullptr);
  o.db = db != nullptr;
  RunForm rf;
  const bool run = run_form_ok(d, o.x, &rf, true) && rf.bytes <= ws_bytes;
  Route r = bwd_f_gemm(d, o, run ? kRunForm : bwd_f_ring_ok(d, o) ? kLdsDma : kAsStored);
  fit_workspace(r, o, ws_bytes, o.db ? (size_t)r.g.N * 4 : 0);
  const GemmPlan& plan = r.plan;
  float* out = run ? static_cast<float*>(ws) : dw;
  IgemmParams p;
  fill_common(p, r.g);
  rc = apply_storage(p, d->precision, d->storage & A3D_STORE_X_BF16, d->storage & A3D_STORE_Y_BF16, false, d->c, d->ldx, -1, d->ldy,
                     x, dz, dw, "x", "dz", "dw");
  if (rc != A3D_OK) return rc;
  A3D_CHECK_ARG(!d->storage || plan.prec == A3D_PREC_BF16, "conv2d_bwd_filter: bf16 storage needs vectorisable operands");
  if (r.bytes > ws_bytes) return set_error(A3D_EWORKSPACE, "conv2d_bwd_filter: need %zu workspace bytes", r.bytes);
  hipStream_t st = static_cast<hipStream_t>(stream);
  if (plan.ring && db) {
    float* parts = reinterpret_cast<float*>(static_cast<char*>(ws) + plan.ws_bytes);
    int nparts = 0;
    rc = colsum_bf16(dz, r.g.K, d->k, d->ldy, plan.splitk > 1 ? nullptr : db, parts, &nparts, st);
    if (rc != A3D_OK) return rc;
    if (plan.splitk > 1) { p.dbias_parts = parts; p.dbias_parts_out = db; p.dbias_parts_n = nparts; }
    db = nullptr;
  }
  p.A = x; p.B = dz; p.C = out; p.dbias = db;
  p.npix = r.g.K; p.nrsc = r.g.M;
  fill_gather(p, d, d->ldx, run ? 1 : d->s, run ? rf.rlp : d->c);
  p.ldb = d->ldy; p.ldc = d->k;
  fill_staging(p, MODE_BWD_F, (unsigned long long)d->n * d->h * d->w * d->ldx, (unsigned long long)d->n * d->ho * d->wo * d->ldy, d->r,
               run ? 1 : d->s);
  if (run) { p.unpad_dst = dw; p.unpad_rl = rf.rl; p.unpad_rlp = rf.rlp; }
  rc = launch_igemm(MODE_BWD_F, plan, r.g.avec, r.g.bvec, p, static_cast<char*>(ws) + r.repack, st);
  if (rc != A3D_OK || !run || p.unpad_done) return rc;
  clear_stale_error();
  hipLaunchKernelGGL(unpad_filter_kernel, dim3((d->r * rf.rl * d->k + 255) / 256), dim3(256), 0, st, out, dw, d->r,
                     rf.rl, rf.rlp, d->k);
  return check_launch("unpad_filter");
}

static a3d_conv_desc dense_desc(int m, int k, int n) {
  a3d_conv_desc d{};
  d.n = m; d.h = 1; d.w = 1; d.c = k; d.k = n; d.r = 1; d.s = 1; d.stride = 1; d.ho = 1; d.wo = 1;
  d.ldx = k; d.ldy = n;
  return d;
}

size_t a3d_dense_fwd_ws_bytes(int m, int k, int n) {
  a3d_conv_desc d = dense_desc(m, k, n);
  if (check_desc(&d) != A3D_OK) return 0;
  return std::max(plan_gemm(fwd_problem(&d), A3D_PREC_F32).ws_bytes, dense_stream_ws_bytes(m, k, n));
}

int a3d_dense_fwd(int m, int k, int n, const float* x, const float* w, const float* bias, float* y, int act,
                  const uint8_t* drop_keep, void* ws, size_t ws_bytes, void* stream) {
  return a3d_dense_fwd_ex(m, k, n, x, w, bias, y, act, drop_keep, A3D_PREC_F32, 0, ws, ws_bytes, stream);
}

int a3d_dense_fwd_ex(int m, int k, int n, const float* x, const float* w, const float* bias, float* y, int act,
                     const uint8_t* drop_keep, int precision, int storage, void* ws, size_t ws_bytes, void* stream) {
  return a3d_dense_fwd_ex2(m, k, n, x, w, bias, y, n, n, act, drop_keep, precision, storage, nullptr, ws, ws_bytes, stream);
}

int a3d_dense_fwd_ex2(int m, int k, int n, const float* x, const float* w, const float* bias, float* y, int ldy, int ncols_y, int act,
                      const uint8_t* drop_keep, int precision, int storage, const a3d_second_output* out2, void* ws,
                      size_t ws_bytes, void* stream) {
  A3D_CHECK_ARG(m > 0 && k > 0 && n > 0, "dense_fwd: bad dims");
  A3D_CHECK_ARG(ncols_y > 0 && ncols_y <= n && ldy >= ncols_y, "dense_fwd: y rows of %d columns at pitch %d from a GEMM of %d", ncols_y, ldy, n);
  A3D_CHECK_ARG((storage & ~(A3D_STORE_W_BF16 | A3D_STORE_X_BF16)) == 0, "dense_fwd: the weights and x may be bf16, y is float32");
  a3d_conv_desc d = dense_desc(m, k, n);
  d.precision = precision;
  int rc = check_desc(&d);
  if (rc != A3D_OK) return rc;
  A3D_CHECK_ARG(x && w && y, "dense_fwd: null tensor");
  A3D_CHECK_WS(ws, "dense_fwd");
  if (precision == A3D_PREC_F32 && !storage && dense_stream_applicable(m, k, n) && aligned16(x) && !out2 && ldy == n && ncols_y == n &&
      !tune_int("A3D_NO_DENSE_KERNELS", 0))
    return dense_fwd_stream(m, k, n, x, w, bias, y, act, drop_keep, 2.f, ws, ws_bytes, static_cast<hipStream_t>(stream));
  GemmProblem g = fwd_problem(&d);
  if (!aligned16(x)) g.avec = 1;
  if (!aligned16(w)) g.bvec = 1;
  IgemmParams p;
  fill_common(p, g);
  rc = apply_storage(p, precision, storage & A3D_STORE_X_BF16, storage & A3D_STORE_W_BF16, false, k, k, n, n, x, w, y, "x", "w", "y");
  if (rc != A3D_OK) return rc;
  A3D_CHECK_ARG(!p.a16 || aligned16(y), "dense_fwd: beside a bf16 x, y must be 16-byte aligned (the LDS-DMA kernel alone reads a bf16 x)");
  storage_vecs(g, p.a16, p.b16, p.c16);
  g.ring_ok = p.a16 && p.b16 && precision == A3D_PREC_BF16 && k % 8 == 0 && n % 8 == 0 && aligned16(y) && act != A3D_ACT_SIGMOID;
  g.need_reduce = ncols_y != n;
  GemmPlan plan = plan_gemm(g, precision);
  if (!aligned16(x) || !aligned16(w) || !aligned16(y)) plan = plan_within(g, plan, ws ? ws_bytes : 0, 0);
  A3D_CHECK_ARG(!storage || plan.prec == A3D_PREC_BF16, "dense_fwd: bf16 weights need vectorisable operands");
  A3D_CHECK_ARG(!p.a16 || plan.ring, "dense_fwd: a bf16 x is taken by the LDS-DMA kernel only (bf16 weights, k and n multiples of 8)");
  if (plan.ws_bytes > ws_bytes) return set_error(A3D_EWORKSPACE, "dense_fwd: need %zu workspace bytes", plan.ws_bytes);
  p.A = x; p.B = w; p.C = y; p.bias = bias; p.act = act; p.keep = drop_keep; p.mask_scale = 2.f;
  p.npix = m; p.nrsc = k;
  fill_gather(p, &d, k, 1, k);
  p.ldb = n; p.ldc = ldy; p.c_cols = ncols_y == n ? 0 : ncols_y;
  rc = take_second_output(p, out2);
  if (rc != A3D_OK) return rc;
  fill_staging(p, MODE_FWD, (unsigned long long)m * k, (unsigned long long)k * n, 1, 1);
  return launch_igemm(MODE_FWD, plan, g.avec, g.bvec, p, ws, static_cast<hipStream_t>(stream));
}

size_t a3d_dense_bwd_data_ws_bytes(int m, int k, int n) {
  a3d_conv_desc d = dense_desc(m, k, n);
  return a3d_conv2d_bwd_data_ws_bytes(&d);
}

int a3d_dense_bwd_data(int m, int k, int n, const float* dz, const float* w, float* dx, const float* mask,
                       int mask_act, float scale, void* ws, size_t ws_bytes, void* stream) {
  return a3d_dense_bwd_data_ex(m, k, n, dz, w, dx, mask, mask_act, scale, A3D_PREC_F32, 0, ws, ws_bytes, stream);
}

int a3d_dense_bwd_data_ex(int m, int k, int n, const float* dz, const float* w, float* dx, const float* mask, int mask_act,
                          float scale, int precision, int storage, void* ws, size_t ws_bytes, void* stream) {
  return a3d_dense_bwd_data_ex2(m, k, n, dz, w, dx, mask, mask_act, scale, precision, storage, nullptr, ws, ws_bytes, stream);
}

int a3d_dense_bwd_data_ex2(int m, int k, int n, const float* dz, const float* w, float* dx, const float* mask, int mask_act,
                           float scale, int precision, int storage, const a3d_second_output* out2, void* ws, size_t ws_bytes,
                           void* stream) {
  A3D_CHECK_ARG(m > 0 && k > 0 && n > 0, "dense_bwd_data: bad dims");
  A3D_CHECK_ARG(precision >= A3D_PREC_F32 && precision <= A3D_PREC_BF16, "dense_bwd_data: unknown precision %d", precision);
  A3D_CHECK_ARG(!mask || mask_act == A3D_ACT_RELU || mask_act == A3D_ACT_SIGMOID, "dense_bwd_data: bad mask_act");
  a3d_conv_desc d = dense_desc(m, k, n);
  int rc = check_desc(&d);
  if (rc != A3D_OK) return rc;
  A3D_CHECK_ARG(dz && w && dx, "dense_bwd_data: null tensor");
  A3D_CHECK_WS(ws, "dense_bwd_data");
  GemmProblem g = bwd_d_problem(&d);
  if (!aligned16(dz)) g.avec = 1;
  if (!aligned16(w)) g.bvec = 1;
  IgemmParams p;
  fill_common(p, g);
  rc = apply_storage(p, precision, storage & A3D_STORE_Y_BF16, storage & A3D_STORE_W_BF16, storage & A3D_STORE_X_BF16, n, n, n, n, dz, w,
                     dx, "dz", "w", "dx");
  if (rc != A3D_OK) return rc;
  A3D_CHECK_ARG(!p.c16 || aligned16(mask), "dense_bwd_data: bf16 mask must be 16-byte aligned");
  storage_vecs(g, p.a16, p.b16, p.c16);
  g.ring_ok = p.a16 && p.b16 && precision == A3D_PREC_BF16 && k % 8 == 0 && n % 8 == 0 && aligned16(dx) &&
              (!mask || (aligned16(mask) && mask_act == A3D_ACT_RELU));
  GemmPlan plan = plan_gemm(g, precision);
  if (!aligned16(dz) || !aligned16(w) || !aligned16(dx) || !aligned16(mask)) plan = plan_within(g, plan, ws ? ws_bytes : 0, 0);
  A3D_CHECK_ARG(!storage || plan.prec == A3D_PREC_BF16, "dense_bwd_data: bf16 weights need vectorisable operands");
  A3D_CHECK_ARG(!(p.a16 || p.c16) || plan.ring, "dense_bwd_data: bf16 dz / dx are taken by the LDS-DMA kernel only (bf16 weights, k and n multiples of 8, ReLU mask)");
  if (plan.ws_bytes > ws_bytes) return set_error(A3D_EWORKSPACE, "dense_bwd_data: need %zu workspace bytes", plan.ws_bytes);
  p.A = dz; p.B = w; p.C = dx; p.mask = mask; p.mask_scale = scale; p.mask_act = mask_act;
  p.npix = m; p.nrsc = n;
  fill_gather(p, &d, n, 1, n);
  p.Cn = k;
  p.ldc = k;
  p.S_full = 1;
  rc = take_second_output(p, out2);
  if (rc != A3D_OK) return rc;
  fill_staging(p, MODE_BWD_D, (unsigned long long)m * n, (unsigned long long)k * n, 1, 1);
  return launch_igemm(MODE_BWD_D, plan, g.avec, g.bvec, p, ws, static_cast<hipStream_t>(stream));
}

size_t a3d_dense_bwd_filter_ws_bytes(int m, int k, int n) {
  a3d_conv_desc d = dense_desc(m, k, n);
  return a3d_conv2d_bwd_filter_ws_bytes(&d);
}

int a3d_dense_bwd_filter(int m, int k, int n, const float* x, const float* dz, float* dw, float* db, void* ws,
                         size_t ws_bytes, void* stream) {
  A3D_CHECK_ARG(m > 0 && k > 0 && n > 0, "dense_bwd_filter: bad dims");
  A3D_CHECK_WS(ws, "dense_bwd_filter");
  if (dense_dw_applicable(m, k, n) && (long)k * n >= (1L << 16) && !tune_int("A3D_NO_DENSE_KERNELS", 0)) {
    A3D_CHECK_ARG(x && dz && dw, "dense_bwd_filter: null tensor");
    return dense_dw_launch(m, k, n, x, dz, dw, db, static_cast<hipStream_t>(stream));
  }
  a3d_conv_desc d = dense_desc(m, k, n);
  return a3d_conv2d_bwd_filter(&d, x, dz, dw, db, ws, ws_bytes, stream);
}

}
```

### ann3depth_amd/models.py

```python
import collections
import contextlib
import ctypes
import math
import os

import numpy as np
import torch

from . import _lib, augment as augment_, ops

NET_H, NET_W = 228, 304
OUT_H, OUT_W = 55, 74
SAMPLES_COARSE = 2000000
SAMPLES_FINE = 1500000

ConvSpec = collections.namedtuple('ConvSpec', 'name cin cout k stride padding relu')

MSDN_CONVS = [
    ConvSpec('coarse/conv/conv2d_0', 3, 96, 11, 4, 'VALID', True),
    ConvSpec('coarse/conv/conv2d_1', 96, 256, 5, 1, 'SAME', True),
    ConvSpec('coarse/conv/conv2d_2', 256, 384, 3, 1, 'SAME', True),
    ConvSpec('coarse/conv/conv2d_3', 384, 384, 3, 1, 'SAME', True),
    ConvSpec('coarse/conv/conv2d_4', 384, 256, 3, 2, 'VALID', True),
    ConvSpec('fine/first/conv2d', 3, 63, 9, 2, 'VALID', True),
    ConvSpec('fine/second/conv2d', 64, 64, 5, 1, 'SAME', True),
    ConvSpec('fine/third', 64, 1, 5, 1, 'SAME', False),
]
MSDN_DENSES = [('coarse/dense/dense_0', 12288, 4096), ('coarse/dense/dense_1', 4096, OUT_H * OUT_W)]

MSDN_OPTIMIZERS = collections.OrderedDict([
    ('CoarseConv', (0.001, ['coarse/conv'])),
    ('CoarseDense', (0.1, ['coarse/dense'])),
    ('FineA', (0.001, ['fine/first', 'fine/third'])),
    ('FineB', (0.01, ['fine/second'])),
])


def glorot_uniform(rng, shape):
    if len(shape) == 2:
        fan_in, fan_out = shape
    else:
        rf = int(np.prod(shape[:-2]))
        fan_in, fan_out = shape[-2] * rf, shape[-1] * rf
    limit = math.sqrt(6.0 / (fan_in + fan_out))
    return rng.uniform(-limit, limit, size=shape).astype(np.float32)


def phase_of(global_step, batchsize):
    steps_coarse = SAMPLES_COARSE // batchsize
    steps_fine = SAMPLES_FINE // batchsize
    if global_step < steps_coarse:
        return 1
    if global_step < steps_coarse + steps_fine:
        return 2
    return 3


class ParamGroup:
    ALIGN = 64

    def __init__(self, name, lr, shapes, device, beta1=0.9, beta2=1.0, eps=1e-8, slots=True, multiple=1):
        self.name, self.lr, self.beta1, self.beta2, self.eps = name, lr, beta1, beta2, eps
        self.offsets = collections.OrderedDict()
        off = 0
        for n, shp in shapes.items():
            self.offsets[n] = (off, tuple(shp))
            off += -(-int(np.prod(shp)) // self.ALIGN) * self.ALIGN
        off = -(-off // (multiple * self.ALIGN)) * (multiple * self.ALIGN)
        self.count = off
        self.var = torch.zeros(off, device=device)
        self.grad = torch.zeros(off, device=device)
        self.m = torch.zeros(off, device=device) if slots else None
        self.v = torch.zeros(off, device=device) if slots else None
        self.beta1_power = np.float32(beta1)
        self.beta2_power = np.float32(beta2)

    def view(self, buf, name):
        off, shp = self.offsets[name]
        return buf[off:off + int(np.prod(shp))].view(shp)

    def apply(self, grad_scale=1.0):
        ops.adam_apply_tf1(self.var, self.m, self.v, self.grad, self.lr, self.beta1, self.beta2, self.eps,
                           float(self.beta1_power), float(self.beta2_power), grad_scale)
        self.beta1_power = self.beta1_power * np.float32(self.beta1)
        self.beta2_power = self.beta2_power * np.float32(self.beta2)

    def apply_slice(self, a, b, grad_scale=1.0, poisoned=None):
        ops.adam_apply_tf1(self.var[a:b], self.m[a:b], self.v[a:b], self.grad[a:b], self.lr, self.beta1, self.beta2,
                           self.eps, float(self.beta1_power), float(self.beta2_power), grad_scale, poisoned=poisoned)

    def frozen(self):
        return self.beta2 == 1.0 and float(self.beta2_power) == 1.0

    def advance(self):
        self.beta1_power = self.beta1_power * np.float32(self.beta1)
        self.beta2_power = self.beta2_power * np.float32(self.beta2)

    def apply_sgd(self, grad_scale=1.0):
        ops.sgd_apply(self.var, self.grad, self.lr * grad_scale)


class MSDNReplica:

    def __init__(self, batchsize, device='cuda', params=None, seed=3000, global_step=0, beta2=1.0, reducer=None,
                 precision='fp32', keep_dense_grads=True, overlap=True, valid_range=None, grad_weight=0.0):
        grad_weight = float(grad_weight)
        if not grad_weight >= 0:
            raise ValueError(f'grad_weight {grad_weight!r}: the weight of the gradient-matching term is a number >= 0')
        self.grad_weight = grad_weight
        if valid_range is not None:
            lo, hi = (float(v) for v in valid_range)
            if not lo <= hi:
                raise ValueError(f'valid_range {valid_range!r}: (min_depth, max_depth) with min_depth <= max_depth')
            valid_range = (lo, hi)
        self.valid_range = valid_range
        self.keep_dense_grads = keep_dense_grads or reducer is not None or batchsize > 64
        self.bf16s = precision == 'bf16s'
        self._c4_32_fresh = False
        if self.bf16s:
            precision = 'bf16'
        self.precision = precision
        self.B = B = batchsize
        self.device = torch.device(device)
        self.global_step = global_step
        self.reducer = reducer
        dev = self.device
        self.overlap = overlap
        self._shared_desc = {}
        self._prep = {}
        self._alone = ()
        self._deferred = None
        self._m_sharded = False
        self.dense_exchange = None
        if reducer is not None:
            want = os.environ.get('A3D_DP_DENSE', 'scatter')
            if want not in ('scatter', 'allreduce'):
                raise ValueError(f'A3D_DP_DENSE={want!r}: scatter or allreduce')
            self.dense_exchange = 'reduce_scatter' if (want == 'scatter' and reducer.inplace_ok(dev)) else 'all_reduce'
            if want == 'scatter' and self.dense_exchange == 'all_reduce':
                print('MSDNReplica: in-place reduce-scatter failed its self-check on this backend; the dense bucket is '
                      'all-reduced instead', flush=True)
        self._dense_pieces = None
        self._poison = None
        self._poison_seen = []
        self.fuse_pool = precision == 'fp32'
        self.side = None
        if self.overlap and dev.type == 'cuda':
            handle = ctypes.c_void_p()
            with torch.cuda.device(dev):
                ops.check(_lib.load().a3d_stream_create(1, ctypes.byref(handle)), 'a3d_stream_create')
            self.side = torch.cuda.ExternalStream(handle.value, device=dev)
            self._side_handle = handle.value
        shapes = collections.OrderedDict()
        for c in MSDN_CONVS:
            shapes[c.name + '/kernel'] = (c.k, c.k, c.cin, c.cout)
            shapes[c.name + '/bias'] = (c.cout,)
        for n, i, o in MSDN_DENSES:
            shapes[n + '/kernel'] = (i, o)
            shapes[n + '/bias'] = (o,)
        self.shapes = shapes
        self.groups = collections.OrderedDict()
        self.group_of = {}
        for gname, (lr, scopes) in MSDN_OPTIMIZERS.items():
            gshapes = collections.OrderedDict((n, s) for n, s in shapes.items()
                                              if any(n.startswith(sc + '/') for sc in scopes))
            world = reducer.world_size if (reducer is not None and gname == 'CoarseDense') else 1
            self.groups[gname] = ParamGroup(gname, lr, gshapes, dev, beta2=beta2, multiple=world)
            for n in gshapes:
                self.group_of[n] = gname
        if params is None:
            rng = np.random.default_rng(seed)
            params = {n: (glorot_uniform(rng, s) if n.endswith('/kernel') else np.zeros(s, np.float32))
                      for n, s in shapes.items()}
        self.load_params(params)

        def buf(*shape):
            return torch.empty(shape, device=dev)

        def abuf(*shape):
            return torch.empty(shape, device=dev, dtype=torch.bfloat16 if self.bf16s else torch.float32)
        self.conv = {c.name: c for c in MSDN_CONVS}
        self.x = buf(B, NET_H, NET_W, 3)
        self.t = buf(B, OUT_H, OUT_W, 1)
        self.c0 = None if self.bf16s else buf(B, 55, 74, 96)
        self.c1 = None if self.bf16s else buf(B, 27, 37, 256)
        self.p0 = abuf(B, 27, 37, 96); self.p1 = abuf(B, 13, 18, 256)
        self.c2 = abuf(B, 13, 18, 384); self.c3 = abuf(B, 13, 18, 384); self.c4 = abuf(B, 6, 8, 256)
        self.drop = buf(B, 4096)
        self.coarse = buf(B, OUT_H, OUT_W, 1)
        self.f1 = buf(B, 110, 148, 63) if not self.bf16s else None
        self.cat = abuf(B, OUT_H, OUT_W, 64)
        self.f2 = buf(B, OUT_H, OUT_W, 64)
        self.fine = buf(B, OUT_H, OUT_W, 1)
        self.loss_coarse = buf(1); self.loss_fine = buf(1)
        if grad_weight > 0:
            self.loss_quad_c = buf(4); self.loss_quad_f = buf(4)
            self.loss_pair_c = self.loss_quad_c[:2]; self.loss_pair_f = self.loss_quad_f[:2]
            self.loss_coarse = self.loss_pair_c[:1]; self.loss_fine = self.loss_pair_f[:1]
        elif valid_range is not None:
            self.loss_pair_c = buf(2); self.loss_pair_f = buf(2)
            self.loss_coarse = self.loss_pair_c[:1]; self.loss_fine = self.loss_pair_f[:1]
        self.loss_out_c, self.loss_out_f = ((self.loss_quad_c, self.loss_quad_f) if grad_weight > 0 else
                                            (self.loss_pair_c, self.loss_pair_f) if valid_range is not None else
                                            (self.loss_coarse, self.loss_fine))
        self.a0 = torch.empty((B, 27, 37, 96), dtype=torch.uint8, device=dev)
        self.a1 = torch.empty((B, 13, 18, 256), dtype=torch.uint8, device=dev)
        self.af1 = torch.empty((B, OUT_H, OUT_W, 63), dtype=torch.uint8, device=dev)
        self.pooled_fwd = None
        silog_ws = ops.silog_grad_ws if grad_weight > 0 else ops.silog_ws if valid_range is None else ops.silog_masked_ws
        self.ws_c = silog_ws(B, dev); self.ws_f = silog_ws(B, dev)
        self.t_one = buf(B, 1, 1, 1) if valid_range is not None else None
        self.dz1 = buf(B, OUT_H * OUT_W); self.dz0 = buf(B, 4096)
        self.dc4 = abuf(B, 6, 8, 256); self.dc3 = abuf(B, 13, 18, 384); self.dc2 = abuf(B, 13, 18, 384)
        self.dp1 = abuf(B, 13, 18, 256); self.dc1 = abuf(B, 27, 37, 256)
        self.dp0 = abuf(B, 27, 37, 96); self.dc0 = None
        self.dfine = buf(B, OUT_H, OUT_W, 1); self.df2 = abuf(B, OUT_H, OUT_W, 64)
        self.dcat = abuf(B, OUT_H, OUT_W, 64); self.df1 = None
        if self.bf16s:
            self.c4_32 = buf(B, 6, 8, 256)
            self.dz0_16 = torch.empty((B, 4096), device=dev, dtype=torch.bfloat16)
            self.dense_bf16_x = B <= 64
            if not self.dense_bf16_x:
                self.dc4_32 = buf(B, 6, 8, 256)
            NP = (OUT_H * OUT_W + 7) // 8 * 8
            self.w1pad = torch.zeros((4096, NP), device=dev, dtype=torch.bfloat16)
            self.b1pad = torch.zeros((1, NP), device=dev)
            self.drop16 = torch.empty((B, 4096), device=dev, dtype=torch.bfloat16)
            self.dz1_16 = torch.zeros((B, NP), device=dev, dtype=torch.bfloat16)
        def D(*a):
            return ops.conv_desc(*a, precision=precision)
        self.d = {
            'coarse/conv/conv2d_0': D(B, NET_H, NET_W, 3, 96, 11, 11, 4, 'VALID'),
            'coarse/conv/conv2d_1': D(B, 27, 37, 96, 256, 5, 5, 1, 'SAME'),
            'coarse/conv/conv2d_2': D(B, 13, 18, 256, 384, 3, 3, 1, 'SAME'),
            'coarse/conv/conv2d_3': D(B, 13, 18, 384, 384, 3, 3, 1, 'SAME'),
            'coarse/conv/conv2d_4': D(B, 13, 18, 384, 256, 3, 3, 2, 'VALID'),
            'fine/first/conv2d': D(B, NET_H, NET_W, 3, 63, 9, 9, 2, 'VALID'),
            'fine/second/conv2d': D(B, OUT_H, OUT_W, 64, 64, 5, 5, 1, 'SAME'),
            'fine/third': D(B, OUT_H, OUT_W, 64, 1, 5, 5, 1, 'SAME'),
        }
        self.d_few = {}
        if dev.type == 'cuda':
            few_prec = 'bf16' if self.bf16s else 'fp32'
            for n, dd in (('coarse/conv/conv2d_0', ops.conv_desc(B, NET_H, NET_W, 3, 96, 11, 11, 4, 'VALID', precision=few_prec)),
                          ('fine/first/conv2d', ops.conv_desc(B, NET_H, NET_W, 3, 63, 9, 9, 2, 'VALID', precision=few_prec))):
                if ops.conv2d_bwd_filter_pooled_supported(dd):
                    self.d_few[n] = dd
        self.store = {}
        self.wcopy = {}
        if self.bf16s:
            X, W, Y = ops.STORE_X, ops.STORE_W, ops.STORE_Y
            for n in ('coarse/conv/conv2d_1', 'coarse/conv/conv2d_2', 'coarse/conv/conv2d_3', 'coarse/conv/conv2d_4'):
                self.store[n] = {'fwd': X | W | Y, 'bwd_d': X | W | Y, 'bwd_f': X | Y}
            self.store['coarse/conv/conv2d_0'] = {'bwd_f': Y}
            self.d['fine/first/conv2d'].precision = ops.PREC['fp32']
            self.store['fine/second/conv2d'] = {'fwd': X | W, 'bwd_d': W | X | Y, 'bwd_f': X | Y}
            self.x4 = torch.empty((B, NET_H, NET_W, 4), device=dev, dtype=torch.bfloat16)
            self.w0_4 = torch.zeros((11, 11, 4, 96), device=dev)
            self.d0_4 = ops.with_storage(ops.conv_desc(B, NET_H, NET_W, 4, 96, 11, 11, 4, 'VALID', ldy=96, precision='bf16'),
                                         X | Y)
            self.w4 = torch.zeros((9, 9, 4, 63), device=dev)
            self.d4 = ops.with_storage(ops.conv_desc(B, NET_H, NET_W, 4, 63, 9, 9, 2, 'VALID', ldy=64, precision='bf16'),
                                       X | Y)
            for n in list(self.store) + ['coarse/dense/dense_0']:
                if n == 'coarse/dense/dense_0' or self.store[n].get('fwd', 0) & W:
                    self.wcopy[n] = torch.empty(self.shapes[n + '/kernel'], device=dev, dtype=torch.bfloat16)
            self.refresh_weight_copies()

    def __del__(self):
        handle, self._side_handle = getattr(self, '_side_handle', None), None
        if handle:
            try:
                torch.cuda.synchronize(self.device)
                ops.drop_workspace(handle)
                _lib.load().a3d_stream_destroy(handle)
            except Exception:
                pass

    SHARE_CU = ('fine/first/conv2d', 'fine/second/conv2d')

    def _desc(self, name, which):
        d = self.d[name]
        bits = self.store.get(name, {}).get(which, 0)
        if which == 'fwd' and self.side is not None and name in self.SHARE_CU and name not in self._alone:
            key = (name, bits)
            if key not in self._shared_desc:
                e = ops.with_storage(d, bits)
                e.hints = ops.HINT_SHARE_CU
                self._shared_desc[key] = e
            return self._shared_desc[key]
        return ops.with_storage(d, bits) if bits else d

    def _w(self, name, which='fwd'):
        if name in self.wcopy and (name not in self.store or self.store[name][which] & ops.STORE_W):
            return self.wcopy[name]
        return self._v(name + '/kernel')

    def _prepared(self, key, desc, w):
        if self.device.type != 'cuda':
            return desc, w
        pf = self._prep.get(key)
        if pf is None:
            pf = self._prep[key] = ops.PreparedFilter(desc, self.device)
            pf.source = w
            if pf.ok:
                pf.refresh(w)
        return (pf.desc_prepared, pf.buf) if pf.ok else (desc, w)

    def _refresh_prepared(self):
        for pf in self._prep.values():
            if pf.ok:
                pf.refresh(pf.source)

    def refresh_weight_copies(self):
        for n, c in self.wcopy.items():
            ops.cast_bf16(self._v(n + '/kernel'), c)
        if self.bf16s:
            self.w4[:, :, :3, :] = self._v('fine/first/conv2d/kernel')
            self.w0_4[:, :, :3, :] = self._v('coarse/conv/conv2d_0/kernel')
            n = 'coarse/dense/dense_1'
            ops.cast_rows(self._v(n + '/kernel'), self.w1pad)
            ops.cast_rows(self._v(n + '/bias').view(1, -1), self.b1pad)

    def _weights_moved(self, *groups):
        if not all(g.frozen() for g in groups):
            if self.wcopy:
                self.refresh_weight_copies()
            self._refresh_prepared()

    def settle(self):
        if self._deferred is not None:
            works, group, scale = self._deferred
            self._deferred = None
            if works and isinstance(works[0], tuple):
                self._poll_poison()
                for work, a, b in works:
                    self.reducer.wait(work)
                    group.apply_slice(a, b, scale, poisoned=self._poison)
                group.advance()
                self._m_sharded = True
                self._watch_poison()
                return
            for work in works:
                self.reducer.wait(work)
            group.apply(scale)
            self._weights_moved(group)

    def _dense_buckets(self):
        if self._dense_pieces is None:
            gd = self.groups['CoarseDense']
            q = self.reducer.world_size * ParamGroup.ALIGN
            c = -(-gd.offsets['coarse/dense/dense_1/kernel'][0] // q) * q
            third = -(-(c // 3) // q) * q
            self._dense_pieces = ([(c, gd.count)], [(0, third), (third, 2 * third), (2 * third, c)])
        return self._dense_pieces

    def _my_slice(self, a, b):
        n = (b - a) // self.reducer.world_size
        return a + self.reducer.rank * n, a + (self.reducer.rank + 1) * n

    def _watch_poison(self):
        red = self.reducer
        work = red.any(self._poison)
        red.wait(work)
        if not hasattr(self, '_poison_ring'):
            ring = torch.empty(4, dtype=torch.int32)
            self._poison_ring = (ring.pin_memory() if self.device.type == 'cuda' else ring, 0)
        ring, nxt = self._poison_ring
        self._poison_ring = (ring, (nxt + 1) % 4)
        host = ring[nxt:nxt + 1]
        host.copy_(self._poison, non_blocking=True)
        ev = None
        if self.device.type == 'cuda':
            ev = torch.cuda.Event()
            ev.record()
        self._poison_seen.append((ev, host))

    def _poll_poison(self, block=False):
        while self._poison_seen and (block or len(self._poison_seen) >= 2):
            ev, host = self._poison_seen.pop(0)
            if ev is not None:
                ev.synchronize()
            if int(host.item()):
                self._resync()

    def _resync(self):
        gd = self.groups['CoarseDense']
        early, late = self._dense_buckets()
        for a, b in early + late:
            for buf in (gd.var, gd.v, gd.m):
                self.reducer.all_gather(buf[a:b])
        self._poison.zero_()
        self._poison_seen = []
        self._m_sharded = False

    def gather_state(self):
        self.settle()
        if self._m_sharded:
            self._poll_poison(block=True)
        if self._m_sharded:
            gd = self.groups['CoarseDense']
            early, late = self._dense_buckets()
            for a, b in early + late:
                self.reducer.all_gather(gd.m[a:b])
            self._m_sharded = False

    def load_params(self, params):
        self.settle()
        for n, shp in self.shapes.items():
            g = self.groups[self.group_of[n]]
            a = np.asarray(params[n], np.float32)
            assert a.shape == tuple(shp), (n, a.shape, shp)
            g.view(g.var, n).copy_(torch.from_numpy(np.ascontiguousarray(a)))
        if getattr(self, 'wcopy', None):
            self.refresh_weight_copies()
        if getattr(self, '_prep', None):
            self._refresh_prepared()

    def _v(self, name):
        g = self.groups[self.group_of[name]]
        return g.view(g.var, name)

    def _g(self, name):
        g = self.groups[self.group_of[name]]
        return g.view(g.grad, name)

    def var(self, name):
        self.settle()
        return self._v(name)

    def grad(self, name):
        self.settle()
        return self._g(name)

    def slot(self, name, which):
        self.gather_state()
        g = self.groups[self.group_of[name]]
        return g.view(g.m if which == 'm' else g.v, name)

    def state_dict(self):
        self.gather_state()
        sd = collections.OrderedDict()
        for n in self.shapes:
            sd[n] = self.var(n)
            sd[n + '/' + self.group_of[n]] = self.slot(n, 'm')
            sd[n + '/' + self.group_of[n] + '_1'] = self.slot(n, 'v')
        for gname, g in self.groups.items():
            sd[gname + '/beta1_power'] = torch.tensor(float(g.beta1_power))
            sd[gname + '/beta2_power'] = torch.tensor(float(g.beta2_power))
        sd['global_step'] = torch.tensor(self.global_step, dtype=torch.int64)
        return sd

    def load_state_dict(self, sd):
        self.gather_state()
        for n in self.shapes:
            self.var(n).copy_(sd[n])
            self.slot(n, 'm').copy_(sd[n + '/' + self.group_of[n]])
            self.slot(n, 'v').copy_(sd[n + '/' + self.group_of[n] + '_1'])
        for gname, g in self.groups.items():
            g.beta1_power = np.float32(sd[gname + '/beta1_power'].item())
            g.beta2_power = np.float32(sd[gname + '/beta2_power'].item())
        self.global_step = int(sd['global_step'].item())
        if self.wcopy:
            self.refresh_weight_copies()
        self._refresh_prepared()

    uses_dropout = True

    def load_tf_variables(self, tensors):
        missing = [n for n in self.shapes if n not in tensors]
        if missing:
            raise KeyError(f'TensorFlow checkpoint lacks {len(missing)} model variables, e.g. {missing[:3]}')
        self.load_params(tensors)
        for n in self.shapes:
            for which, suffix in (('m', ''), ('v', '_1')):
                key = n + '/' + self.group_of[n] + suffix
                if key in tensors:
                    self.slot(n, which).copy_(torch.from_numpy(np.ascontiguousarray(tensors[key], np.float32)))
        if 'global_step' in tensors:
            self.global_step = int(np.asarray(tensors['global_step']).reshape(-1)[0])
        steps_coarse, steps_fine = SAMPLES_COARSE // self.B, SAMPLES_FINE // self.B
        applied = {'CoarseConv': min(self.global_step, steps_coarse), 'CoarseDense': min(self.global_step, steps_coarse),
                   'FineA': min(max(self.global_step - steps_coarse, 0), steps_fine),
                   'FineB': min(max(self.global_step - steps_coarse, 0), steps_fine)}
        for gname, g in self.groups.items():
            for attr, beta in (('beta1_power', g.beta1), ('beta2_power', g.beta2)):
                key = f'{gname}/{attr}'
                if key in tensors:
                    setattr(g, attr, np.float32(np.asarray(tensors[key]).reshape(-1)[0]))
                else:
                    power = np.float32(beta)
                    for _ in range(min(applied[gname], 4096)):
                        power = power * np.float32(beta)
                    setattr(g, attr, power)

    def tf_variables(self):
        out = {}
        for k, v in self.state_dict().items():
            a = v.detach().cpu().numpy()
            out[k] = a.astype(np.int64) if k == 'global_step' else a.astype(np.float32)
        return out

    def summary_scalars(self, out):
        rec = {'loss/coarse_loss': float(out['coarse_loss']), 'loss/fine_loss': float(out['fine_loss']),
               'optimizers/Phase': out['phase']}
        if self.valid_range is not None:
            rec['valid_fraction'] = float(self.loss_pair_c[1])
        if self.grad_weight > 0:
            rec['loss/coarse_grad'] = float(self.loss_quad_c[3])
            rec['loss/fine_grad'] = float(self.loss_quad_f[3])
        return rec

    def summary_images(self):
        target = self.t if self.valid_range is None else torch.nan_to_num(self.t[:3], nan=0.0)
        return [('summaries/Input', self.x, 3), ('summaries/Coarse', self.coarse, 3), ('summaries/Fine', self.fine, 3),
                ('summaries/Target', target, 3)]

    def broadcast_state(self, dist, src=0):
        self.gather_state()
        for g in self.groups.values():
            for buf in (g.var, g.m, g.v):
                dist.broadcast(buf, src)
        st = torch.tensor([self.global_step] + [float(x) for g in self.groups.values()
                                                for x in (g.beta1_power, g.beta2_power)],
                          dtype=torch.float64, device=self.device)
        dist.broadcast(st, src)
        self.global_step = int(st[0].item())
        for i, g in enumerate(self.groups.values()):
            g.beta1_power, g.beta2_power = np.float32(st[1 + 2 * i].item()), np.float32(st[2 + 2 * i].item())
        if self.wcopy:
            self.refresh_weight_copies()
        self._refresh_prepared()

    def _kb(self, name):
        return self._v(name + '/kernel'), self._v(name + '/bias')

    FEW_CHANNEL = ('coarse/conv/conv2d_0', 'fine/first/conv2d')

    def _fwd_operands(self, name):
        d, w = self._desc(name, 'fwd'), self._w(name)
        if name in self.FEW_CHANNEL:
            d, w = self._prepared((name, d.storage, d.hints, d.precision), d, w)
        return d, w

    def _conv(self, name, x, y):
        d, w = self._fwd_operands(name)
        ops.conv2d_fwd(d, x, w, self._v(name + '/bias'), y, 'relu' if self.conv[name].relu else None)

    @contextlib.contextmanager
    def _beside(self):
        if self.side is None:
            yield
            return
        self.side.wait_stream(torch.cuda.current_stream())
        with torch.cuda.stream(self.side):
            yield

    def _join(self):
        if self.side is not None:
            torch.cuda.current_stream().wait_stream(self.side)

    def prepool_equivalent(self, which):
        src = {'c0': (self.c0, self.p0, self.a0, 1), 'c1': (self.c1, self.p1, self.a1, 1),
               'f1': (self.f1, self.cat, self.af1, 2)}[which]
        full, pooled, arg, phase = src
        if self.pooled_fwd != phase and not self.bf16s:
            return full
        if full is None:
            full = torch.empty((pooled.shape[0],) + {'c0': (55, 74, 96), 'c1': (27, 37, 256), 'f1': (110, 148, 63)}[which],
                               device=self.device)
        pooled = pooled.float()
        c = arg.shape[-1]
        out = torch.zeros_like(full)
        ph, pw = arg.shape[1], arg.shape[2]
        win = out[:, :2 * ph, :2 * pw, :].reshape(full.shape[0], ph, 2, pw, 2, c)
        a = arg.long()
        for pos in range(4):
            win[:, :, pos >> 1, :, pos & 1, :] = torch.where(a == pos, pooled[..., :c], torch.zeros_like(pooled[..., :c]))
        return out

    def _conv_pool(self, name, x, y_pooled, argmax=None):
        d, w = self._fwd_operands(name)
        ops.conv2d_pool_fwd(d, x, w, self._v(name + '/bias'), y_pooled, 'relu', argmax)

    def _fine_first_image_form(self, argmax=None):
        d, w = self._prepared(('fine/first/image', 0, 0, 0), self.d4, self.w4)
        ops.conv2d_pool_fwd(d, self.x4, w, self._v('fine/first/conv2d/bias'), self.cat, 'relu', argmax)

    def forward(self, images, depths, keep_mask, join=True, phase=None, warp=None):
        if depths is None:
            pass
        elif self.valid_range is not None:
            lo, hi = self.valid_range
            if warp is not None:
                ops.warp_bilinear_pair_valid(images, self.x, depths, self.t, warp, lo, hi)
            elif images.shape[:3] == depths.shape[:3]:
                ops.resize_bilinear_tf1_pair_valid(images, self.x, depths, self.t, lo, hi)
            else:
                ops.resize_bilinear_tf1(images, self.x)
                ops.resize_bilinear_tf1_valid(depths, self.t, lo, hi, scratch=self.t_one)
        elif warp is not None:
            ops.warp_bilinear_pair(images, self.x, depths, self.t, warp)
        elif images.shape[:3] == depths.shape[:3]:
            ops.resize_bilinear_tf1_pair(images, self.x, depths, self.t)
        else:
            ops.resize_bilinear_tf1(images, self.x)
            ops.resize_bilinear_tf1(depths, self.t)
        B = self.B
        self.dropout_on = keep_mask is not None
        self._alone = ('fine/second/conv2d',) if phase == 2 else ()
        if self.bf16s:
            ops.pad_channels_bf16(self.x, self.x4)
        fused = self.fuse_pool and phase in (1, 2, 3)
        self.pooled_fwd = phase if fused else None
        lean_fine = fused
        if fused:
            train = phase == 1
            self._conv_pool('coarse/conv/conv2d_0', self.x, self.p0, self.a0 if train else None)
            self._conv_pool('coarse/conv/conv2d_1', self.p0, self.p1, self.a1 if train else None)
        elif self.bf16s:
            d, w = self._prepared(('conv2d_0/image', 0, 0, 0), self.d0_4, self.w0_4)
            ops.conv2d_pool_fwd(d, self.x4, w, self._v('coarse/conv/conv2d_0/bias'), self.p0, 'relu', self.a0)
            self._conv_pool('coarse/conv/conv2d_1', self.p0, self.p1, self.a1)
        else:
            self._conv('coarse/conv/conv2d_0', self.x, self.c0)
            ops.maxpool2x2_fwd(self.c0, self.p0)
            self._conv('coarse/conv/conv2d_1', self.p0, self.c1)
            ops.maxpool2x2_fwd(self.c1, self.p1)
        def fine_first():
            with self._beside():
                if lean_fine:
                    self._conv_pool('fine/first/conv2d', self.x, self.cat, self.af1 if phase == 2 else None)
                elif self.bf16s:
                    self._fine_first_image_form(None if phase in (1, 3) else self.af1)
                else:
                    self._conv('fine/first/conv2d', self.x, self.f1)
        self._conv('coarse/conv/conv2d_2', self.p1, self.c2)
        self._conv('coarse/conv/conv2d_3', self.c2, self.c3)
        fine_first()
        self._c4_32_fresh = False
        if self.bf16s and self.dense_bf16_x and phase == 1:
            n4 = 'coarse/conv/conv2d_4'
            ops.conv2d_fwd(self._desc(n4, 'fwd'), self.c3, self._w(n4), self._v(n4 + '/bias'), self.c4, 'relu',
                           out2=ops.second_output(self.c4_32.view(-1, 256)))
            self._c4_32_fresh = True
        else:
            self._conv('coarse/conv/conv2d_4', self.c3, self.c4)
        if not self._sharded_in_flight():
            self.settle()
        w, b = self._kb('coarse/dense/dense_0')
        if self.bf16s and self.dense_bf16_x:
            ops.dense_fwd_ex(self.c4.view(B, -1), self.wcopy['coarse/dense/dense_0'], b, self.drop, 'relu',
                             drop_keep=keep_mask, precision='bf16', storage=ops.STORE_W | ops.STORE_X,
                             out2=ops.second_output(self.drop16))
        elif self.bf16s:
            ops.cast_bf16(self.c4, self.c4_32)
            ops.dense_fwd_ex(self.c4_32.view(B, -1), self.wcopy['coarse/dense/dense_0'], b, self.drop, 'relu',
                             drop_keep=keep_mask, precision='bf16', storage=ops.STORE_W)
        else:
            ops.dense_fwd(self.c4.view(B, -1), w, b, self.drop, 'relu', drop_keep=keep_mask)
        w, b = self._kb('coarse/dense/dense_1')
        cat_done = self.bf16s and self.dense_bf16_x
        if cat_done:
            ops.dense_fwd_ex(self.drop16, self.w1pad, self.b1pad, self.coarse.view(B, -1), None, precision='bf16',
                             storage=ops.STORE_W | ops.STORE_X, n=self.w1pad.shape[1],
                             out2=ops.second_output(self.cat, cols=OUT_H * OUT_W, step=64, offset=63, ld=OUT_H * OUT_W))
        else:
            ops.dense_fwd(self.drop, w, b, self.coarse.view(B, -1))
        with self._beside():
            if cat_done:
                pass
            elif lean_fine or self.bf16s:
                ops.copy_channel(self.coarse, 0, self.cat, 63)
            else:
                ops.maxpool2x2_fwd(self.f1, self.cat, extra=self.coarse)
            self._conv('fine/second/conv2d', self.cat, self.f2)
            self._conv('fine/third', self.f2, self.fine)
            if depths is not None:
                self._loss_fwd(self.fine, self.loss_out_f, self.ws_f)
        if depths is not None:
            self._loss_fwd(self.coarse, self.loss_out_c, self.ws_c)
        if join:
            self._join()

    def predict(self, images, n=None):
        B = self.B
        n = images.shape[0] if n is None else int(n)
        if not 0 < n <= min(B, images.shape[0]):
            raise ValueError(f'predict: n = {n} rows of a batch of {images.shape[0]} images, replica batch {B}')
        ops.resize_bilinear_tf1(images[:n], self.x[:n])
        if n < B:
            self.x[n:].zero_()
        self.forward(images, None, None, join=True, phase=3)
        return self.coarse.view(B, OUT_H, OUT_W), self.fine.view(B, OUT_H, OUT_W)

    def _loss_fwd(self, out, loss, ws):
        if self.grad_weight > 0:
            ops.silog_grad_loss_fwd(out, self.t, OUT_H, OUT_W, self.valid_range is not None, self.grad_weight, loss, ws)
        elif self.valid_range is None:
            ops.silog_loss_fwd(out, self.t, loss, ws)
        else:
            ops.silog_masked_loss_fwd(out, self.t, loss, ws)

    def _loss_bwd(self, out, ws, dout, dout16=None):
        if self.grad_weight > 0:
            ops.silog_grad_loss_bwd(out, self.t, OUT_H, OUT_W, self.valid_range is not None, self.grad_weight, ws, dout, dout16)
        elif self.valid_range is None:
            ops.silog_loss_bwd(out, self.t, ws, dout, dout16)
        else:
            ops.silog_masked_loss_bwd(out, self.t, ws, dout, dout16)

    def _sharded_in_flight(self):
        d = self._deferred
        return d is not None and bool(d[0]) and isinstance(d[0][0], tuple)

    def _fused_dense_adam(self):
        return not self.keep_dense_grads and self.groups['CoarseDense'].frozen()

    def _bwd_data(self, name, dz, dx, relu_mask=None):
        ops.conv2d_bwd_data(self._desc(name, 'bwd_d'), dz, self._w(name, 'bwd_d'), dx, relu_mask=relu_mask)

    def _bwd_filter(self, name, x, dz):
        if name in self.d:
            ops.conv2d_bwd_filter(self._desc(name, 'bwd_f'), x, dz, self._g(name + '/kernel'), self._g(name + '/bias'))
        elif self._fused_dense_adam():
            g = self.groups[self.group_of[name + '/kernel']]
            kw = [g.view(buf, name + '/kernel') for buf in (g.var, g.m, g.v)]
            kb = [g.view(buf, name + '/bias') for buf in (g.var, g.m, g.v)]
            ops.dense_bwd_filter_adam_tf1(x, dz, *kw, *kb, g.lr, g.beta1, g.beta2, float(g.beta1_power),
                                          float(g.beta2_power), 1.0, precision='bf16' if self.bf16s else 'fp32')
        else:
            ops.dense_bwd_filter(x, dz, self._g(name + '/kernel'), self._g(name + '/bias'))

    def backward_coarse(self, after_dense=None, after_conv2=None, after_dense1=None):
        B = self.B
        bf16_x = self.bf16s and self.dense_bf16_x
        self._loss_bwd(self.coarse, self.ws_c, self.dz1.view(B, OUT_H, OUT_W, 1),
                       dout16=self.dz1_16 if bf16_x else None)
        self.settle()
        n = 'coarse/dense/dense_1'
        self._bwd_filter(n, self.drop, self.dz1)
        if after_dense1 is not None:
            after_dense1()
        if bf16_x:
            ops.dense_bwd_data_ex(self.dz1_16, self.w1pad, self.dz0, mask=self.drop, scale=2.0 if self.dropout_on else 1.0,
                                  precision='bf16', storage=ops.STORE_W | ops.STORE_Y,
                                  out2=ops.second_output(self.dz0_16))
        else:
            ops.dense_bwd_data(self.dz1, self._v(n + '/kernel'), self.dz0, mask=self.drop, scale=2.0 if self.dropout_on else 1.0)
        n = 'coarse/dense/dense_0'
        if bf16_x and not self._c4_32_fresh:
            ops.cast_bf16(self.c4, self.c4_32)
        flat = (self.c4_32 if self.bf16s else self.c4).view(B, -1)
        self._bwd_filter(n, flat, self.dz0)
        if bf16_x:
            ops.dense_bwd_data_ex(self.dz0_16, self.wcopy[n], self.dc4.view(B, -1), mask=self.c4.view(B, -1), scale=1.0,
                                  precision='bf16', storage=ops.STORE_W | ops.STORE_X | ops.STORE_Y)
        elif self.bf16s:
            ops.dense_bwd_data_ex(self.dz0, self.wcopy[n], self.dc4_32.view(B, -1), mask=flat, scale=1.0, precision='bf16',
                                  storage=ops.STORE_W)
            ops.cast_bf16(self.dc4_32, self.dc4)
        else:
            ops.dense_bwd_data(self.dz0, self._v(n + '/kernel'), self.dc4.view(B, -1), mask=flat, scale=1.0)
        if after_dense is not None:
            after_dense()
        n = 'coarse/conv/conv2d_4'
        self._bwd_filter(n, self.c3, self.dc4)
        self._bwd_data(n, self.dc4, self.dc3, relu_mask=self.c3)
        self._join()
        dw = self._bwd_filter
        n = 'coarse/conv/conv2d_3'
        dw(n, self.c2, self.dc3)
        self._bwd_data(n, self.dc3, self.dc2, relu_mask=self.c2)
        n = 'coarse/conv/conv2d_2'
        dw(n, self.p1, self.dc2)
        if after_conv2 is not None:
            after_conv2()
        self._bwd_data(n, self.dc2, self.dp1)
        pooled = self.pooled_fwd == 1 or self.bf16s
        if pooled:
            ops.maxpool2x2_bwd_idx(self.a1, self.p1, self.dp1, self.dc1, relu_mask=True)
        else:
            ops.maxpool2x2_bwd(self.c1, self.dp1, self.dc1, relu_mask=True)
        n = 'coarse/conv/conv2d_1'
        dw(n, self.p0, self.dc1)
        self._bwd_data(n, self.dc1, self.dp0)
        n = 'coarse/conv/conv2d_0'
        if pooled and n in self.d_few:
            ops.conv2d_bwd_filter_pooled(self.d_few[n], self.x, self.dp0, self.p0, self.a0, self._g(n + '/kernel'),
                                         self._g(n + '/bias'))
            return
        if self.dc0 is None:
            self.dc0 = torch.empty((self.B, 55, 74, 96), device=self.device, dtype=self.dp0.dtype)
        if pooled:
            ops.maxpool2x2_bwd_idx(self.a0, self.p0, self.dp0, self.dc0, relu_mask=True)
        else:
            ops.maxpool2x2_bwd(self.c0, self.dp0, self.dc0, relu_mask=True)
        dw(n, self.x, self.dc0)

    def backward_fine(self):
        self._join()
        self._loss_bwd(self.fine, self.ws_f, self.dfine)
        n = 'fine/third'
        if ops.conv2d_bwd_both_supported(self.d[n]):
            ops.conv2d_bwd_both(self.d[n], self.f2, self.dfine, self._v(n + '/kernel'), self._g(n + '/kernel'),
                                self._g(n + '/bias'), self.df2, relu_mask=True)
        else:
            assert not self.bf16s, 'bf16 storage: df2 is a bf16 tensor only the fused backward writes'
            self._bwd_filter(n, self.f2, self.dfine)
            self._bwd_data(n, self.dfine, self.df2, relu_mask=self.f2)
        n = 'fine/second/conv2d'
        self._bwd_filter(n, self.cat, self.df2)
        self._bwd_data(n, self.df2, self.dcat)
        n = 'fine/first/conv2d'
        if (self.pooled_fwd == 2 or self.bf16s) and n in self.d_few:
            ops.conv2d_bwd_filter_pooled(self.d_few[n], self.x, self.dcat, self.cat, self.af1, self._g(n + '/kernel'),
                                         self._g(n + '/bias'))
            return
        if self.df1 is None:
            self.df1 = torch.empty((self.B, 110, 148, 63), device=self.device)
        if self.pooled_fwd == 2 or self.bf16s:
            ops.maxpool2x2_bwd_idx(self.af1, self.cat, self.dcat, self.df1, relu_mask=True)
        else:
            ops.maxpool2x2_bwd(self.f1, self.dcat, self.df1, relu_mask=True)
        self._bwd_filter(n, self.x, self.df1)

    def step(self, images, depths, keep_mask, warp=None):
        if keep_mask is not None and keep_mask.dtype != torch.uint8:
            keep_mask = keep_mask.to(torch.uint8)
        phase = phase_of(self.global_step, self.B)
        self.forward(images, depths, keep_mask, join=False, phase=phase, warp=warp)
        red = self.reducer
        scale = 1.0 / red.world_size if red is not None else 1.0
        if phase == 1:
            gc, gd = self.groups['CoarseConv'], self.groups['CoarseDense']
            if red is None:
                fused = self._fused_dense_adam()
                self.backward_coarse()
                gc.apply(scale)
                if fused:
                    gd.advance()
                else:
                    gd.apply(scale)
                self._weights_moved(gc, gd)
            else:
                handle, tail = [], []
                cut = gc.offsets['coarse/conv/conv2d_2/kernel'][0]
                if gd.frozen() and self.dense_exchange == 'reduce_scatter':
                    early, late = self._dense_buckets()
                    if self._poison is None:
                        self._poison = torch.zeros(1, dtype=torch.int32, device=self.device)

                    def scatter(pieces):
                        for a, b in pieces:
                            work, _ = red.reduce_scatter(gd.grad[a:b])
                            handle.append((work,) + self._my_slice(a, b))
                    after_dense1, after_dense = (lambda: scatter(early)), (lambda: scatter(late))
                else:
                    d1 = gd.offsets['coarse/dense/dense_1/kernel'][0]
                    third = -(-(d1 // 3) // ParamGroup.ALIGN) * ParamGroup.ALIGN
                    pieces0 = [(0, third), (third, 2 * third), (2 * third, d1)]
                    after_dense1 = lambda: handle.append(red.start(gd.grad[d1:]))
                    after_dense = lambda: handle.extend(red.start(gd.grad[a:b]) for a, b in pieces0)
                self.backward_coarse(after_dense1=after_dense1, after_dense=after_dense,
                                     after_conv2=lambda: tail.append(red.start(gc.grad[cut:], urgent=True)))
                head = red.start(gc.grad[:cut], urgent=True)
                red.wait(tail[0])
                red.wait(head)
                gc.apply(scale)
                self._weights_moved(gc)
                self._deferred = (handle, gd, scale)
        elif phase == 2:
            ga, gb = self.groups['FineA'], self.groups['FineB']
            self.backward_fine()
            if red is not None:
                red.start(ga.grad)
                red.start(gb.grad)
                red.finish()
            ga.apply(scale)
            gb.apply(scale)
            self._weights_moved(ga, gb)
        self._join()
        self.global_step += 1
        return {'coarse_loss': self.loss_coarse, 'fine_loss': self.loss_fine, 'phase': phase}


DCNF_IMG_H, DCNF_IMG_W = 240, 320
DCNF_PATCH, DCNF_SP = 100, 40
DCNF_PREFIX = 'unary/unary_layers/'
DCNF_CONVS = [('conv2d', 3, 64, 11), ('conv2d_1', 64, 256, 5), ('conv2d_2', 256, 256, 3),
              ('conv2d_3', 256, 256, 3), ('conv2d_4', 256, 256, 3)]
DCNF_POOL_AFTER = ('conv2d', 'conv2d_1', 'conv2d_4')
DCNF_DENSES = [('dense', 12544, 128, 'relu'), ('dense_1', 128, 16, 'sigmoid'), ('dense_2', 16, 1, None)]


class DCNFUnary:

    def __init__(self, batchsize, device='cuda', params=None, seed=3000, precision='fp32'):
        self.B = batchsize
        self.device = dev = torch.device(device)
        self.rows, _ = ops.same_pad(DCNF_IMG_H, DCNF_PATCH, DCNF_SP)
        self.cols, _ = ops.same_pad(DCNF_IMG_W, DCNF_PATCH, DCNF_SP)
        self.P = P = batchsize * self.rows * self.cols
        shapes = collections.OrderedDict()
        for n, ci, co, k in DCNF_CONVS:
            shapes[DCNF_PREFIX + n + '/kernel'] = (k, k, ci, co)
            shapes[DCNF_PREFIX + n + '/bias'] = (co,)
        for n, i, o, _ in DCNF_DENSES:
            shapes[DCNF_PREFIX + n + '/kernel'] = (i, o)
            shapes[DCNF_PREFIX + n + '/bias'] = (o,)
        self.shapes = shapes
        self.group = ParamGroup('unary', 0.1, shapes, dev, slots=False)
        if params is None:
            rng = np.random.default_rng(seed)
            params = {n: (glorot_uniform(rng, s) if n.endswith('/kernel') else np.zeros(s, np.float32))
                      for n, s in shapes.items()}
        for n, s in shapes.items():
            self.group.view(self.group.var, n).copy_(torch.from_numpy(np.ascontiguousarray(params[n], np.float32)))

        def buf(*shape):
            return torch.empty(shape, device=dev)
        self.resized = buf(batchsize, DCNF_IMG_H, DCNF_IMG_W, 3)
        self.act = collections.OrderedDict()
        self.dact = {}
        self.desc = {}
        self.fuse_pool = precision == 'fp32'
        self.argmax, self.conv_hw = {}, {}
        self.few_pooled = False
        self.act['x'] = buf(P, DCNF_PATCH, DCNF_PATCH, 3)
        h = DCNF_PATCH
        for n, ci, co, k in DCNF_CONVS:
            self.desc[n] = ops.conv_desc(P, h, h, ci, co, k, k, 1, 'VALID', precision=precision)
            h = h - k + 1
            self.conv_hw[n] = h
            if not (self.fuse_pool and n in DCNF_POOL_AFTER):
                self.act[n] = buf(P, h, h, co)
            if n in DCNF_POOL_AFTER:
                h //= 2
                self.act[n + '/pool'] = buf(P, h, h, co)
                if self.fuse_pool:
                    self.argmax[n] = torch.empty((P, h, h, co), dtype=torch.uint8, device=dev)
        for n, i, o, _ in DCNF_DENSES:
            self.act[n] = buf(P, o)
        self.z = self.act['dense_2']
        self.few_pooled = (self.fuse_pool and dev.type == 'cuda'
                           and ops.conv2d_bwd_filter_pooled_supported(self.desc['conv2d']))

    def var(self, name):
        return self.group.view(self.group.var, DCNF_PREFIX + name)

    def grad(self, name):
        return self.group.view(self.group.grad, DCNF_PREFIX + name)

    def forward(self, images, record_argmax=True):
        ops.resize_bilinear_tf1(images, self.resized)
        return self.forward_resized(record_argmax)

    def forward_resized(self, record_argmax=True):
        ops.extract_patches(self.resized, DCNF_PATCH, DCNF_SP, self.act['x'])
        t = self._forward_convs(self.act['x'], record_argmax)
        self._forward_denses(t.view(self.P, -1))
        return self.z.view(self.B, self.rows * self.cols, 1)

    def _forward_convs(self, t, record_argmax):
        for n, _, _, _ in DCNF_CONVS:
            if self.fuse_pool and n in DCNF_POOL_AFTER:
                t = ops.conv2d_pool_fwd(self.desc[n], t, self.var(n + '/kernel'), self.var(n + '/bias'),
                                        self.act[n + '/pool'], 'relu', self.argmax[n] if record_argmax else None)
                continue
            ops.conv2d_fwd(self.desc[n], t, self.var(n + '/kernel'), self.var(n + '/bias'), self.act[n], 'relu')
            t = self.act[n]
            if n in DCNF_POOL_AFTER:
                ops.maxpool2x2_fwd(t, self.act[n + '/pool'])
                t = self.act[n + '/pool']
        return t

    def _forward_denses(self, t):
        for n, _, _, act in DCNF_DENSES:
            ops.dense_fwd(t, self.var(n + '/kernel'), self.var(n + '/bias'), self.act[n], act)
            t = self.act[n]

    def activations(self):
        out = {k: v.cpu().numpy() for k, v in self.act.items()}
        for n, arg in self.argmax.items():
            pooled = self.act[n + '/pool']
            (hh, ww), c = self._conv_hw(n), pooled.shape[-1]
            N, ph, pw = pooled.shape[:3]
            full = torch.zeros((N, hh, ww, c), device=self.device)
            win = full[:, :2 * ph, :2 * pw, :].reshape(N, ph, 2, pw, 2, c)
            a = arg.long()
            for pos in range(4):
                win[:, :, pos >> 1, :, pos & 1, :] = torch.where(a == pos, pooled, torch.zeros_like(pooled))
            out[n] = full.cpu().numpy()
        return out

    def _conv_hw(self, n):
        hw = self.conv_hw[n]
        return hw if isinstance(hw, tuple) else (hw, hw)

    def _dbuf(self, key, like):
        if key not in self.dact:
            self.dact[key] = torch.empty_like(like)
        return self.dact[key]

    def backward(self, dz):
        P = self.P
        a = self.act
        flat = a['conv2d_4/pool'].view(P, -1)
        d0 = self._backward_denses(flat, dz)
        dflat = self._dbuf('flat', a['conv2d_4/pool'])
        ops.dense_bwd_data(d0, self.var('dense/kernel'), dflat.view(P, -1))
        self._backward_convs(dflat)

    def _backward_denses(self, flat, dz):
        P = self.P
        a = self.act
        d2 = dz.reshape(P, 1).contiguous()
        ops.dense_bwd_filter(a['dense_1'], d2, self.grad('dense_2/kernel'), self.grad('dense_2/bias'))
        d1 = self._dbuf('dense_1', a['dense_1'])
        ops.dense_bwd_data(d2, self.var('dense_2/kernel'), d1, mask=a['dense_1'], mask_act='sigmoid')
        ops.dense_bwd_filter(a['dense'], d1, self.grad('dense_1/kernel'), self.grad('dense_1/bias'))
        d0 = self._dbuf('dense', a['dense'])
        ops.dense_bwd_data(d1, self.var('dense_1/kernel'), d0, mask=a['dense'], scale=1.0)
# ... 590 lines not shown
```

### ann3depth_amd/ops.py

```python
import ctypes

import torch

from . import _lib
from ._lib import ConvDesc, check

ACT = {None: 0, 'relu': 1, 'sigmoid': 2}
PREC = {'fp32': 0, 'f32': 0, 'bf16x3': 1, 'bf16': 2}


def _ptr(t):
    return None if t is None else ctypes.c_void_p(t.data_ptr())


def _stream():
    return ctypes.c_void_p(torch.cuda.current_stream().cuda_stream)


class Workspace:

    def __init__(self):
        self.buf = None

    def reserve(self, nbytes, device):
        if self.buf is None or self.buf.numel() < nbytes or self.buf.device != device:
            if torch.cuda.is_current_stream_capturing():
                raise RuntimeError(f'workspace of {nbytes} bytes must be reserved before graph capture')
            self.buf = torch.empty(max(nbytes, 1 << 20), dtype=torch.uint8, device=device)
        return self.buf

    def get(self, nbytes, device):
        buf = self.reserve(nbytes, device)
        return ctypes.c_void_p(buf.data_ptr()), buf.numel()


_WS = {}


def _ws():
    key = torch.cuda.current_stream().cuda_stream
    w = _WS.get(key)
    if w is None:
        w = _WS[key] = Workspace()
    return w


def drop_workspace(stream_handle):
    _WS.pop(stream_handle, None)


def same_pad(in_size, k, stride):
    out = -(-in_size // stride)
    pad = max((out - 1) * stride + k - in_size, 0)
    return out, pad // 2


STORE_X, STORE_W, STORE_Y = 1, 2, 4


HINT_SHARE_CU = 1
HINT_W_PREPARED = 2


class PreparedFilter:

    def __init__(self, desc, device):
        lib = _lib.load()
        nbytes = lib.a3d_conv2d_fwd_prepared_filter_bytes(ctypes.byref(desc))
        self.ok = nbytes > 0
        self.desc = desc
        if self.ok:
            self.buf = torch.empty(nbytes, dtype=torch.uint8, device=device)
            self.desc_prepared = ConvDesc.from_buffer_copy(desc)
            self.desc_prepared.hints = desc.hints | HINT_W_PREPARED

    def refresh(self, w):
        check(_lib.load().a3d_conv2d_fwd_prepare_filter(ctypes.byref(self.desc), _ptr(w), _ptr(self.buf), self.buf.numel(), _stream()),
              'a3d_conv2d_fwd_prepare_filter')


def conv_desc(n, h, w, c, k, r, s, stride, padding, ldx=None, ldy=None, precision='fp32', storage=0, hints=0):
    padding = padding.upper()
    if padding == 'SAME':
        ho, pt = same_pad(h, r, stride)
        wo, pl = same_pad(w, s, stride)
    elif padding == 'VALID':
        ho, pt = (h - r) // stride + 1, 0
        wo, pl = (w - s) // stride + 1, 0
    else:
        raise ValueError(padding)
    return ConvDesc(n=n, h=h, w=w, c=c, k=k, r=r, s=s, stride=stride, pad_t=pt, pad_l=pl, ho=ho, wo=wo,
                    ldx=ldx or c, ldy=ldy or k, precision=PREC[precision], storage=storage, hints=hints)


def second_output(t, cols=None, step=1, offset=0, ld=None):
    if t is None:
        return None
    ld = t.shape[-1] if ld is None else ld
    o = _lib.SecondOutput(t.data_ptr(), ld, step, offset, int(t.dtype == torch.bfloat16), ld if cols is None else cols)
    o._keep = t
    return o


def _o2(out2):
    return None if out2 is None else ctypes.byref(out2)


def conv2d_fwd(d, x, w, bias, y, act=None, out2=None):
    lib = _lib.load()
    ws, n = _ws().get(lib.a3d_conv2d_fwd_ws_bytes(ctypes.byref(d)), x.device)
    if out2 is not None:
        check(lib.a3d_conv2d_fwd_ex2(ctypes.byref(d), _ptr(x), _ptr(w), _ptr(bias), _ptr(y), ACT[act], _o2(out2), ws, n, _stream()),
              'a3d_conv2d_fwd_ex2')
        return y
    check(lib.a3d_conv2d_fwd(ctypes.byref(d), _ptr(x), _ptr(w), _ptr(bias), _ptr(y), ACT[act], ws, n, _stream()),
          'a3d_conv2d_fwd')
    return y


def conv2d_pool_fwd(d, x, w, bias, y_pooled, act='relu', argmax=None):
    lib = _lib.load()
    ws, n = _ws().get(lib.a3d_conv2d_fwd_ws_bytes(ctypes.byref(d)), x.device)
    check(lib.a3d_conv2d_pool_fwd(ctypes.byref(d), _ptr(x), _ptr(w), _ptr(bias), _ptr(y_pooled), y_pooled.shape[-1],
                                  _ptr(argmax), ACT[act], ws, n, _stream()), 'a3d_conv2d_pool_fwd')
    return y_pooled


def maxpool2x2_bwd_idx(argmax, y_pooled, dy, dx, relu_mask=True):
    n, h, w, c = dx.shape
    if y_pooled.dtype == torch.bfloat16 and dx.dtype == torch.bfloat16:
        assert dy.dtype == torch.bfloat16
        name = 'a3d_maxpool2x2_bwd_idx_bf16s'
    elif y_pooled.dtype == torch.bfloat16:
        assert dy.dtype == torch.bfloat16 and dx.dtype == torch.float32
        name = 'a3d_maxpool2x2_bwd_idx_bf16'
    else:
        name = 'a3d_maxpool2x2_bwd_idx'
    check(getattr(_lib.load(), name)(n, h, w, c, _ptr(argmax), _ptr(y_pooled), y_pooled.shape[-1], _ptr(dy), dy.shape[-1],
                                     _ptr(dx), int(relu_mask), _stream()), name)
    return dx


def copy_channel(src, c_src, dst, c_dst):
    npix = src.numel() // src.shape[-1]
    assert dst.numel() // dst.shape[-1] == npix
    fn = _lib.load().a3d_copy_channel_bf16 if dst.dtype == torch.bfloat16 else _lib.load().a3d_copy_channel
    check(fn(npix, _ptr(src), src.shape[-1], c_src, _ptr(dst), dst.shape[-1], c_dst, _stream()), 'a3d_copy_channel')
    return dst


def conv2d_bwd_data(d, dz, w, dx, relu_mask=None):
    lib = _lib.load()
    ws, n = _ws().get(lib.a3d_conv2d_bwd_data_ws_bytes(ctypes.byref(d)), dz.device)
    check(lib.a3d_conv2d_bwd_data(ctypes.byref(d), _ptr(dz), _ptr(w), _ptr(dx), _ptr(relu_mask), ws, n, _stream()),
          'a3d_conv2d_bwd_data')
    return dx


def conv2d_bwd_filter(d, x, dz, dw, db=None):
    lib = _lib.load()
    ws, n = _ws().get(lib.a3d_conv2d_bwd_filter_ws_bytes(ctypes.byref(d)), x.device)
    check(lib.a3d_conv2d_bwd_filter(ctypes.byref(d), _ptr(x), _ptr(dz), _ptr(dw), _ptr(db), ws, n, _stream()),
          'a3d_conv2d_bwd_filter')
    return dw, db


def conv2d_bwd_filter_pooled_supported(d):
    return _lib.load().a3d_conv2d_bwd_filter_pooled_ws_bytes(ctypes.byref(d)) > 0


def conv2d_bwd_filter_pooled(d, x, dpool, pooled, argmax, dw, db=None):
    lib = _lib.load()
    ws, n = _ws().get(lib.a3d_conv2d_bwd_filter_pooled_ws_bytes(ctypes.byref(d)), x.device)
    assert pooled is None or (pooled.dtype == dpool.dtype and pooled.shape[-1] == dpool.shape[-1])
    check(lib.a3d_conv2d_bwd_filter_pooled(ctypes.byref(d), _ptr(x), _ptr(dpool), dpool.shape[-1], _ptr(pooled), _ptr(argmax),
                                           argmax.shape[-1], int(dpool.dtype == torch.bfloat16), _ptr(dw), _ptr(db), ws, n,
                                           _stream()), 'a3d_conv2d_bwd_filter_pooled')
    return dw, db


_BOTH_STATE = {}


def conv2d_bwd_both_supported(d):
    return bool(_lib.load().a3d_conv2d_bwd_both_supported(ctypes.byref(d)))


def conv2d_bwd_both(d, x, dz, w, dw, db, dx, relu_mask=True):
    lib = _lib.load()
    key = (torch.cuda.current_stream().cuda_stream, x.device)
    state = _BOTH_STATE.get(key)
    if state is None:
        state = _BOTH_STATE[key] = torch.zeros(64, dtype=torch.int32, device=x.device)
    ws, n = _ws().get(lib.a3d_conv2d_bwd_both_ws_bytes(ctypes.byref(d)), x.device)
    check(lib.a3d_conv2d_bwd_both(ctypes.byref(d), _ptr(x), _ptr(dz), _ptr(w), _ptr(dw), _ptr(db), _ptr(dx), dx.shape[-1],
                                  int(dx.dtype == torch.bfloat16), int(bool(relu_mask)), _ptr(state), ws, n, _stream()),
          'a3d_conv2d_bwd_both')
    return dw, db, dx


def dense_fwd(x, w, bias, y, act=None, drop_keep=None):
    m, k = x.shape
    n = w.shape[1]
    lib = _lib.load()
    ws, nb = _ws().get(lib.a3d_dense_fwd_ws_bytes(m, k, n), x.device)
    check(lib.a3d_dense_fwd(m, k, n, _ptr(x), _ptr(w), _ptr(bias), _ptr(y), ACT[act], _ptr(drop_keep), ws, nb,
                            _stream()), 'a3d_dense_fwd')
    return y


def dense_bwd_data(dz, w, dx, mask=None, scale=1.0, mask_act='relu'):
    m, n = dz.shape
    k = w.shape[0]
    lib = _lib.load()
    ws, nb = _ws().get(lib.a3d_dense_bwd_data_ws_bytes(m, k, n), dz.device)
    check(lib.a3d_dense_bwd_data(m, k, n, _ptr(dz), _ptr(w), _ptr(dx), _ptr(mask), ACT[mask_act], scale, ws, nb,
                                 _stream()),
          'a3d_dense_bwd_data')
    return dx


def dense_bwd_filter(x, dz, dw, db=None):
    m, k = x.shape
    n = dz.shape[1]
    lib = _lib.load()
    ws, nb = _ws().get(lib.a3d_dense_bwd_filter_ws_bytes(m, k, n), x.device)
    check(lib.a3d_dense_bwd_filter(m, k, n, _ptr(x), _ptr(dz), _ptr(dw), _ptr(db), ws, nb, _stream()),
          'a3d_dense_bwd_filter')
    return dw, db


def maxpool2x2_fwd(x, y, extra=None):
    n, h, w, c = x.shape
    check(_lib.load().a3d_maxpool2x2_fwd(n, h, w, c, _ptr(x), _ptr(y), y.shape[-1], _ptr(extra), _stream()),
          'a3d_maxpool2x2_fwd')
    return y


def maxpool2x2_bwd(x, dy, dx, relu_mask=True):
    n, h, w, c = x.shape
    check(_lib.load().a3d_maxpool2x2_bwd(n, h, w, c, _ptr(x), _ptr(dy), dy.shape[-1], _ptr(dx), int(relu_mask),
                                         _stream()), 'a3d_maxpool2x2_bwd')
    return dx


def _pair_args(x0, y0, x1=None, y1=None):
    def one(x, y):
        if x is None:
            return 0, None, 0, 0, 0, None
        return x.shape[3], _ptr(x), int(x.dtype == torch.uint8), y.shape[1], y.shape[2], _ptr(y)
    return tuple(x0.shape[:3]) + one(x0, y0) + one(x1, y1)


def resize_bilinear_tf1(x, y):
    n, h, w, c = x.shape
    if x.dtype == torch.uint8:
        check(_lib.load().a3d_resize_bilinear_tf1_ex(*_pair_args(x, y), _stream()), 'a3d_resize_bilinear_tf1_ex')
        return y
    check(_lib.load().a3d_resize_bilinear_tf1(n, h, w, c, _ptr(x), y.shape[1], y.shape[2], _ptr(y), _stream()),
          'a3d_resize_bilinear_tf1')
    return y


def resize_bilinear_tf1_pair(x0, y0, x1, y1):
    n, h, w, c0 = x0.shape
    assert x1.shape[:3] == (n, h, w)
    if x0.dtype == torch.uint8 or x1.dtype == torch.uint8:
        check(_lib.load().a3d_resize_bilinear_tf1_ex(*_pair_args(x0, y0, x1, y1), _stream()), 'a3d_resize_bilinear_tf1_ex')
        return
    check(_lib.load().a3d_resize_bilinear_tf1_pair(n, h, w, c0, _ptr(x0), y0.shape[1], y0.shape[2], _ptr(y0), x1.shape[3],
                                                   _ptr(x1), y1.shape[1], y1.shape[2], _ptr(y1), _stream()),
          'a3d_resize_bilinear_tf1_pair')


WARP_STRIDE = 12


def _check_pair(who, x0, y0, x1, y1, table):
    if x0.dim() != 4 or y0.dim() != 4 or y0.shape[0] != x0.shape[0] or y0.shape[3] != x0.shape[3]:
        raise ValueError(f'{who}: {tuple(x0.shape)} -> {tuple(y0.shape)}')
    n, h, w, c0 = x0.shape
    if (x1 is None) != (y1 is None):
        raise ValueError(f'{who}: x1 and y1 go together')
    if x1 is not None and (x1.dim() != 4 or tuple(x1.shape[:3]) != (n, h, w) or y1.dim() != 4
                           or y1.shape[0] != n or y1.shape[3] != x1.shape[3]):
        raise ValueError(f'{who}: second tensor {tuple(x1.shape)} -> {tuple(y1.shape)} beside '
                         f'{tuple(x0.shape)}')
    if table is not None and (tuple(table.shape) != (n, WARP_STRIDE) or table.dtype != torch.float32):
        raise ValueError(f'{who}: table {tuple(table.shape)} {table.dtype}, want [{n}, {WARP_STRIDE}] float32')
    for name, t, dtypes in (('x0', x0, (torch.float32, torch.uint8)), ('y0', y0, (torch.float32,)),
                            ('x1', x1, (torch.float32, torch.uint8)), ('y1', y1, (torch.float32,)),
                            ('table', table, (torch.float32,))):
        if t is None:
            continue
        if t.dtype not in dtypes:
            raise ValueError(f'{who}: {name} is {t.dtype}')
        if not t.is_cuda or t.device != x0.device:
            raise ValueError(f'{who}: {name} is on {t.device}, x0 on {x0.device}')
        if not t.is_contiguous():
            raise ValueError(f'{who}: {name} is not contiguous')
    return n, h, w, c0


def warp_bilinear_pair(x0, y0, x1, y1, table):
    if table is None:
        raise ValueError('warp_bilinear_pair: no table')
    _check_pair('warp_bilinear_pair', x0, y0, x1, y1, table)
    check(_lib.load().a3d_warp_bilinear_pair(*_pair_args(x0, y0, x1, y1), _ptr(table), _stream()), 'a3d_warp_bilinear_pair')


def _valid_range(who, x1, min_depth, max_depth):
    if x1 is None:
        raise ValueError(f'{who}: the depth map x1 is required')
    lo, hi = float(min_depth), float(max_depth)
    if not lo <= hi:
        raise ValueError(f'{who}: min_depth {lo}, max_depth {hi}')
    return lo, hi


def resize_bilinear_tf1_pair_valid(x0, y0, x1, y1, min_depth=0., max_depth=float('inf')):
    who = 'resize_bilinear_tf1_pair_valid'
    lo, hi = _valid_range(who, x1, min_depth, max_depth)
    _check_pair(who, x0, y0, x1, y1, None)
    check(_lib.load().a3dx_resize_bilinear_tf1_valid(*_pair_args(x0, y0, x1, y1), lo, hi, _stream()),
          'a3dx_resize_bilinear_tf1_valid')


def resize_bilinear_tf1_valid(x, y, min_depth=0., max_depth=float('inf'), scratch=None):
    if scratch is None:
        scratch = torch.empty((x.shape[0], 1, 1, x.shape[3]), device=x.device)
    resize_bilinear_tf1_pair_valid(x, scratch, x, y, min_depth, max_depth)
    return y


def warp_bilinear_pair_valid(x0, y0, x1, y1, table, min_depth=0., max_depth=float('inf')):
    who = 'warp_bilinear_pair_valid'
    if table is None:
        raise ValueError(f'{who}: no table')
    lo, hi = _valid_range(who, x1, min_depth, max_depth)
    _check_pair(who, x0, y0, x1, y1, table)
    check(_lib.load().a3dx_warp_bilinear_pair_valid(*_pair_args(x0, y0, x1, y1), _ptr(table), lo, hi, _stream()),
          'a3dx_warp_bilinear_pair_valid')


def extract_patches(x, k, stride, y):
    n, h, w, c = x.shape
    check(_lib.load().a3d_extract_patches(n, h, w, c, _ptr(x), k, stride, _ptr(y), _stream()), 'a3d_extract_patches')
    return y


SILOG_PARTS = 8


def silog_ws(b, device):
    return torch.zeros(2 * b + 1 + 2 * b * SILOG_PARTS, device=device)


def silog_loss_fwd(out, tgt, loss, ws):
    b = out.shape[0]
    assert ws.numel() >= 2 * b + 1 + 2 * b * SILOG_PARTS, 'silog workspace too small: allocate it with ops.silog_ws(b, device)'
    npix = out.numel() // b
    check(_lib.load().a3d_silog_loss_fwd(b, npix, _ptr(out), _ptr(tgt), _ptr(loss), _ptr(ws), _stream()),
          'a3d_silog_loss_fwd')
    return loss


def silog_loss_bwd(out, tgt, ws, dout, dout16=None):
    b = out.shape[0]
    npix = out.numel() // b
    check(_lib.load().a3d_silog_loss_bwd_ex(b, npix, _ptr(out), _ptr(tgt), _ptr(ws), _ptr(dout), _ptr(dout16),
                                            0 if dout16 is None else dout16.shape[-1], _stream()), 'a3d_silog_loss_bwd_ex')
    return dout


def silog_masked_ws(b, device):
    return torch.zeros(3 * b + 1 + 3 * b * SILOG_PARTS, device=device)


def silog_masked_loss_fwd(out, tgt, loss, ws):
    b = out.shape[0]
    assert ws.numel() >= 3 * b + 1 + 3 * b * SILOG_PARTS, \
# ... 480 lines not shown
```

### include/a3d.h

```cpp
#ifndef A3D_H_
#define A3D_H_

#include <stddef.h>
#include <stdint.h>

#ifdef __cplusplus
extern "C" {
#endif

#define A3D_OK 0
#define A3D_EINVAL (-1)
#define A3D_EWORKSPACE (-2)
#define A3D_ELAUNCH (-3)
#define A3D_EFORMAT (-4)
#define A3D_EIO (-5)

#define A3D_ACT_NONE 0
#define A3D_ACT_RELU 1
#define A3D_ACT_SIGMOID 2

typedef struct a3d_conv_desc {
  int32_t n, h, w, c;
  int32_t k, r, s;
  int32_t stride;
  int32_t pad_t, pad_l;
  int32_t ho, wo;
  int32_t ldx;
  int32_t ldy;
  int32_t precision;
  int32_t storage;
  int32_t hints;
} a3d_conv_desc;

#define A3D_HINT_SHARE_CU 1
#define A3D_HINT_W_PREPARED 2

#define A3D_STORE_X_BF16 1
#define A3D_STORE_W_BF16 2
#define A3D_STORE_Y_BF16 4

#define A3D_PREC_F32 0
#define A3D_PREC_BF16X3 1
#define A3D_PREC_BF16 2

const char* a3d_version(void);
int a3d_last_error(char* buf, size_t len);
size_t a3d_sizeof_conv_desc(void);

int a3d_stream_create(int level, void** stream);
int a3d_stream_destroy(void* stream);

size_t a3d_conv2d_fwd_ws_bytes(const a3d_conv_desc* d);
int a3d_conv2d_fwd(const a3d_conv_desc* d, const float* x, const float* w, const float* bias, float* y,
                   int act, void* ws, size_t ws_bytes, void* stream);

size_t a3d_conv2d_fwd_prepared_filter_bytes(const a3d_conv_desc* d);
int a3d_conv2d_fwd_prepare_filter(const a3d_conv_desc* d, const float* w, void* prepared, size_t prepared_bytes, void* stream);

int a3d_conv2d_pool_fwd(const a3d_conv_desc* d, const float* x, const float* w, const float* bias, float* y_pooled,
                        int ld_pooled, uint8_t* argmax, int act, void* ws, size_t ws_bytes, void* stream);

size_t a3d_conv2d_bwd_data_ws_bytes(const a3d_conv_desc* d);
int a3d_conv2d_bwd_data(const a3d_conv_desc* d, const float* dz, const float* w, float* dx,
                        const float* relu_mask, void* ws, size_t ws_bytes, void* stream);

size_t a3d_conv2d_bwd_filter_ws_bytes(const a3d_conv_desc* d);
int a3d_conv2d_bwd_filter(const a3d_conv_desc* d, const float* x, const float* dz, float* dw, float* db,
                          void* ws, size_t ws_bytes, void* stream);

size_t a3d_conv2d_bwd_filter_pooled_ws_bytes(const a3d_conv_desc* d);
int a3d_conv2d_bwd_filter_pooled(const a3d_conv_desc* d, const float* x, const void* dpool, int ld_dpool, const void* pooled,
                                 const uint8_t* argmax, int ld_argmax, int pooled_bf16, float* dw, float* db, void* ws,
                                 size_t ws_bytes, void* stream);

int a3d_conv2d_bwd_both_supported(const a3d_conv_desc* d);
size_t a3d_conv2d_bwd_both_ws_bytes(const a3d_conv_desc* d);
int a3d_conv2d_bwd_both(const a3d_conv_desc* d, const float* x, const float* dz, const float* w, float* dw, float* db,
                        void* dx, int lddx, int dx_bf16, int relu_mask, uint32_t* state, void* ws, size_t ws_bytes,
                        void* stream);

typedef struct a3d_second_output {
  void* ptr;
  int32_t ld, step, offset;
  int32_t bf16;
  int32_t cols;
} a3d_second_output;

int a3d_conv2d_fwd_ex2(const a3d_conv_desc* d, const float* x, const float* w, const float* bias, float* y, int act,
                       const a3d_second_output* out2, void* ws, size_t ws_bytes, void* stream);

size_t a3d_dense_fwd_ws_bytes(int m, int k, int n);
int a3d_dense_fwd(int m, int k, int n, const float* x, const float* w, const float* bias, float* y, int act,
                  const uint8_t* drop_keep, void* ws, size_t ws_bytes, void* stream);
size_t a3d_dense_bwd_data_ws_bytes(int m, int k, int n);
int a3d_dense_bwd_data(int m, int k, int n, const float* dz, const float* w, float* dx, const float* mask,
                       int mask_act, float scale, void* ws, size_t ws_bytes, void* stream);
size_t a3d_dense_bwd_filter_ws_bytes(int m, int k, int n);
int a3d_dense_bwd_filter(int m, int k, int n, const float* x, const float* dz, float* dw, float* db,
                         void* ws, size_t ws_bytes, void* stream);

int a3d_maxpool2x2_fwd(int n, int h, int w, int c, const float* x, float* y, int ldy, const float* extra,
                       void* stream);
int a3d_maxpool2x2_bwd_idx(int n, int h, int w, int c, const uint8_t* argmax, const float* y, int ldy, const float* dy,
                           int lddy, float* dx, int relu_mask, void* stream);
int a3d_comm_standin(const float* src, size_t read_bytes, float* dst, size_t write_bytes, int workgroups, float gbytes_per_s,
                     void* stream);

int a3d_copy_channel(size_t npix, const float* src, int ld_src, int c_src, float* dst, int ld_dst, int c_dst,
                     void* stream);
int a3d_maxpool2x2_bwd(int n, int h, int w, int c, const float* x, const float* dy, int lddy, float* dx,
                       int relu_mask, void* stream);

int a3d_resize_bilinear_tf1(int n, int h, int w, int c, const float* x, int oh, int ow, float* y, void* stream);
int a3d_resize_bilinear_tf1_pair(int n, int h, int w, int c0, const float* x0, int oh0, int ow0, float* y0, int c1,
                                 const float* x1, int oh1, int ow1, float* y1, void* stream);
int a3d_resize_bilinear_tf1_ex(int n, int h, int w, int c0, const void* x0, int u8_0, int oh0, int ow0, float* y0, int c1,
                               const void* x1, int u8_1, int oh1, int ow1, float* y1, void* stream);
#define A3D_WARP_STRIDE 12
int a3d_warp_bilinear_pair(int n, int h, int w, int c0, const void* x0, int u8_0, int oh0, int ow0, float* y0, int c1,
                           const void* x1, int u8_1, int oh1, int ow1, float* y1, const float* table, void* stream);

int a3d_extract_patches(int n, int h, int w, int c, const float* x, int k, int stride, float* y, void* stream);

#define A3D_SILOG_PARTS 8
#define A3D_SILOG_WS_FLOATS(b) ((b) * 2 + 1 + (b) * 2 * A3D_SILOG_PARTS)
int a3d_silog_loss_fwd(int b, int npix, const float* out, const float* tgt, float* loss, float* ws, void* stream);
int a3d_silog_loss_bwd(int b, int npix, const float* out, const float* tgt, const float* ws, float* dout,
                       void* stream);
int a3d_silog_loss_bwd_ex(int b, int npix, const float* out, const float* tgt, const float* ws, float* dout, void* dout_bf16,
                          int ld_bf16, void* stream);

#define A3D_METRIC_COLS 11
#define A3D_METRIC_N 0
#define A3D_METRIC_ABS_REL 1
#define A3D_METRIC_SQ_REL 2
#define A3D_METRIC_SQ 3
#define A3D_METRIC_LOG 4
#define A3D_METRIC_LOG_SQ 5
#define A3D_METRIC_LOG10 6
#define A3D_METRIC_DELTA1 7
#define A3D_METRIC_DELTA2 8
#define A3D_METRIC_DELTA3 9
#define A3D_METRIC_NONFINITE 10
size_t a3d_depth_metrics_ws_bytes(int n, int th, int tw);
int a3d_depth_metrics(int n, int ph, int pw, const float* pred, int th, int tw, const void* target, int target_u8,
                      float min_depth, float max_depth, float clamp_lo, float clamp_hi, double* rows, void* ws,
                      size_t ws_bytes, void* stream);

int a3d_dropout_keep_mask(size_t count, uint64_t seed, uint64_t step, float rate, uint8_t* keep, void* stream);

int a3d_dense_fwd_ex(int m, int k, int n, const float* x, const float* w, const float* bias, float* y, int act,
                     const uint8_t* drop_keep, int precision, int storage, void* ws, size_t ws_bytes, void* stream);
int a3d_dense_bwd_data_ex(int m, int k, int n, const float* dz, const float* w, float* dx, const float* mask, int mask_act,
                          float scale, int precision, int storage, void* ws, size_t ws_bytes, void* stream);
int a3d_dense_fwd_ex2(int m, int k, int n, const float* x, const float* w, const float* bias, float* y, int ldy, int ncols_y, int act,
                      const uint8_t* drop_keep, int precision, int storage, const a3d_second_output* out2, void* ws,
                      size_t ws_bytes, void* stream);
int a3d_dense_bwd_data_ex2(int m, int k, int n, const float* dz, const float* w, float* dx, const float* mask, int mask_act,
                           float scale, int precision, int storage, const a3d_second_output* out2, void* ws, size_t ws_bytes,
                           void* stream);

int a3d_cast_bf16(size_t count, const void* src, void* dst, int to_bf16, void* stream);
int a3d_cast_rows(size_t rows, int cols, const void* src, int ld_src, int src_bf16, void* dst, int ld_dst, int dst_bf16,
                  void* stream);

int a3d_pad_channels_bf16(size_t pixels, int c_src, const float* src, int c_dst, void* dst, void* stream);

int a3d_maxpool2x2_fwd_bf16(int n, int h, int w, int c, const void* x, int ldx, void* y, int ldy, const float* extra,
                            void* stream);
int a3d_maxpool2x2_bwd_bf16(int n, int h, int w, int c, const void* x, int ldx, const void* dy, int lddy, void* dx,
                            int relu_mask, void* stream);

int a3d_copy_channel_bf16(size_t npix, const float* src, int ld_src, int c_src, void* dst, int ld_dst, int c_dst, void* stream);
int a3d_maxpool2x2_bwd_idx_bf16(int n, int h, int w, int c, const uint8_t* argmax, const void* y, int ldy, const void* dy,
                                int lddy, float* dx, int relu_mask, void* stream);
int a3d_maxpool2x2_bwd_idx_bf16s(int n, int h, int w, int c, const uint8_t* argmax, const void* y, int ldy, const void* dy,
                                 int lddy, void* dx, int relu_mask, void* stream);

int a3d_dense_bwd_filter_adam_tf1(int m, int k, int n, const float* x, const float* dz, float* var_w, float* m_w,
                                  float* v_w, float* var_b, float* m_b, float* v_b, float lr, float beta1, float beta2,
                                  float beta1_power, float beta2_power, float grad_scale, void* stream);
int a3d_dense_bwd_filter_adam_tf1_ex(int m, int k, int n, const float* x, const float* dz, float* var_w, float* m_w,
                                  float* v_w, float* var_b, float* m_b, float* v_b, float lr, float beta1, float beta2,
                                  float beta1_power, float beta2_power, float grad_scale, int precision, void* stream);

int a3d_adam_apply_tf1(size_t count, float* var, float* m, float* v, const float* g, float lr, float beta1,
                       float beta2, float eps, float beta1_power, float beta2_power, float grad_scale,
                       void* stream);

int a3d_adam_apply_tf1_flag(size_t count, float* var, float* m, float* v, const float* g, float lr, float beta1,
                            float beta2, float eps, float beta1_power, float beta2_power, float grad_scale,
                            unsigned int* poisoned, void* stream);


int a3d_superpixel_mean(int n, int h, int w, int c, const float* x, int sp, float* out, void* stream);

int a3d_superpixel_hist(int n, int h, int w, const float* x, int sp, float* hist, void* stream);

int a3d_pair_similarity(int n, int h, int w, const float* x, int sp, const float* hist, const int32_t* left,
                        const int32_t* right, int npairs, const float* dense_w, const float* dense_b, float gamma,
                        float* sims, float* r, void* stream);

int a3d_crf_loss(int n, int nsp, const float* z, const float* y, const float* r, const int32_t* left,
                 const int32_t* right, int npairs, float eps, float* loss_per_image, float* loss_mean, float* dz,
                 void* stream);

int a3d_crf_map(int n, int nsp, const float* z, const float* r, const int32_t* left, const int32_t* right, int npairs,
                float* y, int32_t* status, void* stream);

int a3d_sgd_apply(size_t count, float* var, const float* g, float lr, void* stream);

typedef struct a3d_timing_record {
  int32_t mode;
  int32_t bm, bn, waves_m, nwaves, bk, avec, bvec;
  int32_t prec;
  int32_t lds_dma;
  int32_t splitk;
  int32_t m, n, k;
  float ms;
  double flops;
} a3d_timing_record;
int a3d_timing_enable(int on);
int a3d_timing_collect(a3d_timing_record* out, int cap);
int a3d_timing_select(const a3d_timing_record* like);

uint32_t a3d_crc32c(const void* data, size_t len);
uint32_t a3d_masked_crc32c(const void* data, size_t len);

typedef struct a3d_example_view {
  int64_t image_height, image_width, image_channels;
  int64_t depth_height, depth_width, depth_channels;
  const uint8_t* image; size_t image_bytes;
  const uint8_t* depth; size_t depth_bytes;
} a3d_example_view;

int a3d_tfrecord_next(const uint8_t* buf, size_t len, int verify_crc, size_t* payload_off, size_t* payload_len,
                      size_t* consumed);
int a3d_example_parse(const uint8_t* payload, size_t len, a3d_example_view* out);
int a3d_decode_raw_plus_half(const uint8_t* src, size_t bytes, float* dst);
int a3d_record_decode(const uint8_t* frame, size_t len, int verify_crc, float* image_dst, size_t image_floats,
                      float* depth_dst, size_t depth_floats, a3d_example_view* view);
int a3d_record_decode_u8(const uint8_t* frame, size_t len, int verify_crc, uint8_t* image_u8, float* image_f32,
                         size_t image_count, uint8_t* depth_u8, float* depth_f32, size_t depth_count,
                         a3d_example_view* view, int* kinds);
int a3d_records_decode(const void* const* frames, const size_t* lens, int n, int verify_crc, const int64_t* dims,
                       uint8_t* image_u8_pool, float* image_f32_pool, uint8_t* depth_u8_pool, float* depth_f32_pool,
                       const int32_t* slots, int nslots, int32_t* kinds);
int a3d_h2d_gather(void* dst, const void* src_pool, const int32_t* slots, int n, int nslots, size_t bytes_each, void* stream);
int64_t a3d_example_write(const float* image, int ih, int iw, int ic, const float* depth, int dh, int dw, int dc,
                          uint8_t* dst, size_t cap);

#ifdef __cplusplus
}
#endif
#endif
```

Measured before the change: 11480.

## Add Winograd F(2x2,3x3) path for backward-data of coarse 3x3 convs

Adds a Winograd F(2,3) convolution path with filter, input and output transform kernels and a batched 16-slice GEMM that reuses the implicit-GEMM kernel config. A new precision mode selects it, and the model enables it for the bwd-data pass of two coarse 3x3 stride-1 layers with enough tiles, using a prepared, transformed filter. The aim is to cut the multiply count of those backward-data convolutions. The cost is extra workspace, three additional launches with their memory traffic, and slightly different fp32 rounding.

```diff
diff --git a/ann3depth_amd/_lib.py b/ann3depth_amd/_lib.py
--- a/ann3depth_amd/_lib.py
+++ b/ann3depth_amd/_lib.py
@@ -163,6 +163,11 @@
     'a3db_crf_band_map': (c_int, [c_int, c_int, c_int, _P, _P, _P, _P, c_int, _P, _P, _P]),
 }
 
+WINO_SIGNATURES = {
+    'a3dw_conv2d_bwd_data_prepared_filter_bytes': (c_size_t, [_D]),
+    'a3dw_conv2d_bwd_data_prepare_filter': (c_int, [_D, _P, _P, c_size_t, _P]),
+}
+
 _lib = None
 
 
@@ -178,7 +183,7 @@
     for name, (res, args) in (list(SIGNATURES.items()) + list(EXT_SIGNATURES.items()) + list(PAIR_SIGNATURES.items())
                               + list(TEXTURE_SIGNATURES.items()) + list(GRADLOSS_SIGNATURES.items())
                               + list(CRF_VALID_SIGNATURES.items()) + list(FCSP_SIGNATURES.items())
-                              + list(CRF_BAND_SIGNATURES.items())):
+                              + list(CRF_BAND_SIGNATURES.items()) + list(WINO_SIGNATURES.items())):
         try:
             fn = getattr(lib, name)
         except AttributeError as e:
diff --git a/ann3depth_amd/csrc/a3d_internal.h b/ann3depth_amd/csrc/a3d_internal.h
--- a/ann3depth_amd/csrc/a3d_internal.h
+++ b/ann3depth_amd/csrc/a3d_internal.h
@@ -105,4 +105,19 @@
 int conv3b_fwd(const a3d_conv_desc* d, const void* x, const float* w, const float* bias, void* y, int act, int pool, int ld_out,
                uint8_t* argmax, void* ws, size_t ws_bytes, hipStream_t st, bool prepared);
 
+struct WinoGeom {
+  int oh, ow, th, tw;
+  size_t T;
+  int K, N, Kp, Np;
+  size_t v_bytes, m_bytes, u_bytes;
+};
+WinoGeom wino_geom(const a3d_conv_desc* d, bool bwd);
+bool wino_applicable(const a3d_conv_desc* d);
+int wino_filter(const a3d_conv_desc* d, bool bwd, const float* w, float* U, hipStream_t st);
+int wino_input(const a3d_conv_desc* d, bool bwd, const float* src, float* V, hipStream_t st);
+int wino_output(const a3d_conv_desc* d, bool bwd, const float* M, float* out, const float* bias, const float* mask, int act,
+                hipStream_t st);
+a3d_timing_record wino_record(int mode, const WinoGeom& g);
+int wino_gemm(IgemmParams& p, const WinoGeom& g, hipStream_t st);
+
 }
diff --git a/ann3depth_amd/csrc/dense.hip b/ann3depth_amd/csrc/dense.hip
--- a/ann3depth_amd/csrc/dense.hip
+++ b/ann3depth_amd/csrc/dense.hip
@@ -716,6 +716,7 @@
                                                 float* v_w, float* var_b, float* m_b, float* v_b, float lr, float beta1,
                                                 float beta2, float beta1_power, float beta2_power, float grad_scale,
                                                 int precision, void* stream) {
+  if (precision == A3D_PREC_F32_WINOGRAD) precision = A3D_PREC_F32;
   A3D_CHECK_ARG(precision == A3D_PREC_F32 || precision == A3D_PREC_BF16, "dense_bwd_filter_adam: precision %d (float32 or bf16)", precision);
   A3D_CHECK_ARG(m > 0 && k > 0 && n > 0 && x && dz && var_w && m_w && v_w, "dense_bwd_filter_adam: bad arguments");
   A3D_CHECK_ARG((var_b && m_b && v_b) || (!var_b && !m_b && !v_b), "dense_bwd_filter_adam: bias slots come as a set");
diff --git a/ann3depth_amd/csrc/igemm_host.hip b/ann3depth_amd/csrc/igemm_host.hip
--- a/ann3depth_amd/csrc/igemm_host.hip
+++ b/ann3depth_amd/csrc/igemm_host.hip
@@ -1,5 +1,6 @@
 #include <algorithm>
 
+#include "../../include/a3d_wino.h"
 #include "a3d_internal.h"
 #include "igemm.h"
 #include "igemm_cfgs.h"
@@ -117,13 +118,21 @@
   A3D_CHECK_ARG((d->ho - 1) * d->stride - d->pad_t < d->h && (d->wo - 1) * d->stride - d->pad_l < d->w,
                 "conv: output size inconsistent with input");
   A3D_CHECK_ARG(d->ldx >= d->c && d->ldy >= d->k, "conv: pixel strides smaller than channel counts");
-  A3D_CHECK_ARG(d->precision >= A3D_PREC_F32 && d->precision <= A3D_PREC_BF16, "conv: unknown precision %d", d->precision);
+  A3D_CHECK_ARG(d->precision >= A3D_PREC_F32 && d->precision <= A3D_PREC_F32_WINOGRAD, "conv: unknown precision %d", d->precision);
   const double lim = 2147483647.0;
   A3D_CHECK_ARG((double)d->n * d->h * d->w * d->ldx < lim && (double)d->n * d->ho * d->wo * d->ldy < lim &&
                     (double)d->r * d->s * d->c * d->k < lim,
                 "conv: tensor too large for 31-bit indexing");
   return A3D_OK;
 }
+
+#define A3D_AS_F32(d)                                          \
+  a3d_conv_desc d##_f32;                                       \
+  if ((d) && (d)->precision == A3D_PREC_F32_WINOGRAD) {        \
+    d##_f32 = *(d);                                            \
+    d##_f32.precision = A3D_PREC_F32;                          \
+    (d) = &d##_f32;                                            \
+  }
 
 static GemmProblem fwd_problem(const a3d_conv_desc* d) {
   GemmProblem g;
@@ -292,8 +301,50 @@
 
 extern "C" {
 
+static size_t wino_bytes(const a3d_conv_desc* d, bool bwd, bool prepared) {
+  const WinoGeom g = wino_geom(d, bwd);
+  return (prepared ? 0 : g.u_bytes) + g.v_bytes + g.m_bytes;
+}
+static int wino_conv(const a3d_conv_desc* d, bool bwd, const float* src, const float* w, float* out, const float* bias, const float* mask,
+                     int act, bool prepared, void* ws, size_t ws_bytes, hipStream_t st) {
+  const WinoGeom g = wino_geom(d, bwd);
+  const size_t need = wino_bytes(d, bwd, prepared);
+  if (!ws || need > ws_bytes) return set_error(A3D_EWORKSPACE, "conv2d (Winograd): need %zu workspace bytes", need);
+  A3D_CHECK_ARG(!prepared || aligned16(w), "conv2d (Winograd): the prepared filter must be 16-byte aligned");
+  char* base = static_cast<char*>(ws);
+  const float* U = w;
+  int rc;
+  if (!prepared) {
+    rc = wino_filter(d, bwd, w, reinterpret_cast<float*>(base), st);
+    if (rc != A3D_OK) return rc;
+    U = reinterpret_cast<const float*>(base);
+    base += g.u_bytes;
+  }
+  float* V = reinterpret_cast<float*>(base);
+  float* M = reinterpret_cast<float*>(base + g.v_bytes);
+  rc = wino_input(d, bwd, src, V, st);
+  if (rc != A3D_OK) return rc;
+  a3d_conv_desc e{};
+  e.n = (int)g.T; e.h = e.w = e.ho = e.wo = 1; e.c = g.Kp; e.k = g.Np; e.r = e.s = 1; e.stride = 1; e.ldx = g.Kp; e.ldy = g.Np;
+  GemmProblem gp = fwd_problem(&e);
+  IgemmParams p;
+  fill_common(p, gp);
+  p.A = V; p.B = U; p.C = M;
+  p.npix = gp.M; p.nrsc = gp.K;
+  fill_gather(p, &e, g.Kp, 1, g.Kp);
+  p.ldb = g.Np; p.ldc = g.Np;
+  fill_staging(p, MODE_FWD, (unsigned long long)g.T * g.Kp, (unsigned long long)g.Kp * g.Np, 1, 1);
+  rc = timed_launch(wino_record(bwd ? MODE_BWD_D : MODE_FWD, g), st, [&] { return wino_gemm(p, g, st); });
+  if (rc != A3D_OK) return rc;
+  return wino_output(d, bwd, M, out, bias, mask, act, st);
+}
+
 size_t a3d_conv2d_fwd_ws_bytes(const a3d_conv_desc* d) {
-  if (check_desc(d) != A3D_OK || stencil1_applicable(d)) return 0;
+  if (check_desc(d) != A3D_OK) return 0;
+  const size_t wino = wino_applicable(d) ? wino_bytes(d, false, (d->hints & A3D_HINT_W_PREPARED) != 0) : 0;
+  A3D_AS_F32(d);
+  if (stencil1_applicable(d)) return 0;
+  if (wino) return std::max(wino, a3d_conv2d_fwd_ws_bytes(d));
   size_t need = 0;
   for (GemmForm form : {kAsStored, kLdsDma, kRunForm, kBf16Image}) need = upto(need, fwd_gemm(d, kOnGrid, form));
   RunForm rf;
@@ -308,6 +359,16 @@
   int rc = check_desc(d);
   if (rc != A3D_OK) return rc;
   if (!ws) ws_bytes = 0;
+  if (wino_applicable(d) && !pool && !(out2 && out2->ptr)) {
+    A3D_CHECK_ARG(x && w && y, "conv2d_fwd: null tensor");
+    A3D_CHECK_WS(ws, "conv2d_fwd");
+    A3D_CHECK_ARG(act == A3D_ACT_NONE || act == A3D_ACT_RELU || act == A3D_ACT_SIGMOID, "conv2d_fwd: bad act");
+    return wino_conv(d, false, x, w, y, bias, nullptr, act, (d->hints & A3D_HINT_W_PREPARED) != 0, ws, ws_bytes,
+                     static_cast<hipStream_t>(stream));
+  }
+  A3D_CHECK_ARG(!(wino_applicable(d) && (d->hints & A3D_HINT_W_PREPARED)),
+                "conv2d_fwd: A3D_HINT_W_PREPARED with A3D_PREC_F32_WINOGRAD is for the plain forward only (no fused pool, no second output)");
+  A3D_AS_F32(d);
   Operands o = launch_operands(x, w, y, argmax);
   o.act = act; o.pool = pool; o.ld_out = ld_out; o.argmax = argmax != nullptr;
   o.prepared = (d->hints & A3D_HINT_W_PREPARED) != 0;
@@ -394,6 +455,8 @@
 }
 
 size_t a3d_conv2d_fwd_prepared_filter_bytes(const a3d_conv_desc* d) {
+  if (check_desc(d) == A3D_OK && wino_applicable(d)) return wino_geom(d, false).u_bytes;
+  A3D_AS_F32(d);
   RunForm rf{};
   switch (fwd_filter_form(d, &rf)) {
     case 1: return conv3b_applicable(d) ? conv3b_filter_bytes(d) : rf.bytes;
@@ -411,6 +474,8 @@
   A3D_CHECK_ARG(need > 0, "conv2d_fwd_prepare_filter: this forward reads the filter as stored");
   if (prepared_bytes < need) return set_error(A3D_EWORKSPACE, "conv2d_fwd_prepare_filter: need %zu bytes", need);
   hipStream_t st = static_cast<hipStream_t>(stream);
+  if (wino_applicable(d)) return wino_filter(d, false, w, static_cast<float*>(prepared), st);
+  A3D_AS_F32(d);
   RunForm rf{};
   switch (fwd_filter_form(d, &rf)) {
     case 1: return conv3b_applicable(d) ? conv3b_pack(d, w, prepared, st) : pad_filter(d, rf, true, w, prepared, st);
@@ -474,6 +539,8 @@
 
 size_t a3d_conv2d_bwd_data_ws_bytes(const a3d_conv_desc* d) {
   if (check_desc(d) != A3D_OK) return 0;
+  if (wino_applicable(d)) return wino_bytes(d, true, (d->hints & A3D_HINT_W_PREPARED) != 0);
+  A3D_AS_F32(d);
   BwdDClass cls[16];
   const int ncls = bwd_d_classes(d, cls);
   size_t need = 0;
@@ -506,6 +573,10 @@
   A3D_CHECK_ARG(dz && w && dx, "conv2d_bwd_data: null tensor");
   A3D_CHECK_WS(ws, "conv2d_bwd_data");
   if (!ws) ws_bytes = 0;
+  if (wino_applicable(d))
+    return wino_conv(d, true, dz, w, dx, nullptr, relu_mask, A3D_ACT_NONE, (d->hints & A3D_HINT_W_PREPARED) != 0, ws, ws_bytes,
+                     static_cast<hipStream_t>(stream));
+  A3D_AS_F32(d);
   const Operands o = launch_operands(dx, w, dz, relu_mask);
   hipStream_t st = static_cast<hipStream_t>(stream);
   BwdDClass cls[16];
@@ -565,6 +636,20 @@
   });
 }
 
+size_t a3dw_conv2d_bwd_data_prepared_filter_bytes(const a3d_conv_desc* d) {
+  return check_desc(d) == A3D_OK && wino_applicable(d) ? wino_geom(d, true).u_bytes : 0;
+}
+
+int a3dw_conv2d_bwd_data_prepare_filter(const a3d_conv_desc* d, const float* w, void* prepared, size_t prepared_bytes, void* stream) {
+  int rc = check_desc(d);
+  if (rc != A3D_OK) return rc;
+  A3D_CHECK_ARG(w && prepared && aligned16(prepared), "conv2d_bwd_data_prepare_filter: null or misaligned buffer");
+  const size_t need = a3dw_conv2d_bwd_data_prepared_filter_bytes(d);
+  A3D_CHECK_ARG(need > 0, "conv2d_bwd_data_prepare_filter: this bwd-data reads the filter as stored");
+  if (prepared_bytes < need) return set_error(A3D_EWORKSPACE, "conv2d_bwd_data_prepare_filter: need %zu bytes", need);
+  return wino_filter(d, true, w, static_cast<float*>(prepared), static_cast<hipStream_t>(stream));
+}
+
 static bool bwd_f_ring_ok(const a3d_conv_desc* d, const Operands& o) {
   return d->precision == A3D_PREC_BF16 && stored16(d, A3D_STORE_X_BF16 | A3D_STORE_Y_BF16) && d->c % 8 == 0 && d->ldx % 8 == 0 &&
          d->k % 8 == 0 && d->ldy % 8 == 0 && (double)d->n * d->h * d->w * d->ldx * 2.0 < 2147483647.0 && colsum_bf16_ok(d->k) &&
@@ -591,6 +676,7 @@
 }
 
 int a3d_conv2d_bwd_both_supported(const a3d_conv_desc* d) {
+  A3D_AS_F32(d);
   return check_desc(d) == A3D_OK && !d->storage && stencil1_bwd_both_applicable(d);
 }
 
@@ -601,6 +687,7 @@
 int a3d_conv2d_bwd_both(const a3d_conv_desc* d, const float* x, const float* dz, const float* w, float* dw, float* db,
                         void* dx, int lddx, int dx_bf16, int relu_mask, uint32_t* state, void* ws, size_t ws_bytes,
                         void* stream) {
+  A3D_AS_F32(d);
   int rc = check_desc(d);
   if (rc != A3D_OK) return rc;
   A3D_CHECK_ARG(x && dz && w && dw && dx && state, "conv2d_bwd_both: null tensor");
@@ -630,6 +717,7 @@
 static bool fewch_pooled_ok(const a3d_conv_desc* d) { return !d->storage && fewch_bwdf_applicable(d, true); }
 
 size_t a3d_conv2d_bwd_filter_pooled_ws_bytes(const a3d_conv_desc* d) {
+  A3D_AS_F32(d);
   if (check_desc(d) != A3D_OK) return 0;
   if (fewch16_wanted(d, true)) return fewch16_bwdf_ws_bytes(d, true);
   return fewch_pooled_ok(d) ? fewch_bwdf_ws_bytes(d, true) : 0;
@@ -638,6 +726,7 @@
 int a3d_conv2d_bwd_filter_pooled(const a3d_conv_desc* d, const float* x, const void* dpool, int ld_dpool, const void* pooled,
                                  const uint8_t* argmax, int ld_argmax, int pooled_bf16, float* dw, float* db, void* ws,
                                  size_t ws_bytes, void* stream) {
+  A3D_AS_F32(d);
   int rc = check_desc(d);
   if (rc != A3D_OK) return rc;
   A3D_CHECK_ARG(x && dpool && argmax && dw, "conv2d_bwd_filter_pooled: null tensor");
@@ -667,6 +756,7 @@
 }
 
 size_t a3d_conv2d_bwd_filter_ws_bytes(const a3d_conv_desc* d) {
+  A3D_AS_F32(d);
   if (check_desc(d) != A3D_OK) return 0;
   if (stencil1_applicable(d)) return stencil1_bwdf_ws_bytes(d);
   size_t need = fewch_wanted(d, false) ? fewch_bwdf_ws_bytes(d, false) : 0;
@@ -676,6 +766,7 @@
 
 int a3d_conv2d_bwd_filter(const a3d_conv_desc* d, const float* x, const float* dz, float* dw, float* db, void* ws,
                           size_t ws_bytes, void* stream) {
+  A3D_AS_F32(d);
   int rc = check_desc(d);
   if (rc != A3D_OK) return rc;
   A3D_CHECK_ARG(x && dz && dw, "conv2d_bwd_filter: null tensor");
@@ -758,6 +849,7 @@
   A3D_CHECK_ARG(m > 0 && k > 0 && n > 0, "dense_fwd: bad dims");
   A3D_CHECK_ARG(ncols_y > 0 && ncols_y <= n && ldy >= ncols_y, "dense_fwd: y rows of %d columns at pitch %d from a GEMM of %d", ncols_y, ldy, n);
   A3D_CHECK_ARG((storage & ~(A3D_STORE_W_BF16 | A3D_STORE_X_BF16)) == 0, "dense_fwd: the weights and x may be bf16, y is float32");
+  if (precision == A3D_PREC_F32_WINOGRAD) precision = A3D_PREC_F32;
   a3d_conv_desc d = dense_desc(m, k, n);
   d.precision = precision;
   int rc = check_desc(&d);
@@ -812,6 +904,7 @@
                            float scale, int precision, int storage, const a3d_second_output* out2, void* ws, size_t ws_bytes,
                            void* stream) {
   A3D_CHECK_ARG(m > 0 && k > 0 && n > 0, "dense_bwd_data: bad dims");
+  if (precision == A3D_PREC_F32_WINOGRAD) precision = A3D_PREC_F32;
   A3D_CHECK_ARG(precision >= A3D_PREC_F32 && precision <= A3D_PREC_BF16, "dense_bwd_data: unknown precision %d", precision);
   A3D_CHECK_ARG(!mask || mask_act == A3D_ACT_RELU || mask_act == A3D_ACT_SIGMOID, "dense_bwd_data: bad mask_act");
   a3d_conv_desc d = dense_desc(m, k, n);
diff --git a/ann3depth_amd/csrc/wino.hip b/ann3depth_amd/csrc/wino.hip
--- /dev/null
+++ b/ann3depth_amd/csrc/wino.hip
@@ -0,0 +1,246 @@
+#include "a3d_internal.h"
+#include "igemm.h"
+#include "igemm_cfgs.h"
+
+namespace a3d {
+
+typedef float f4 __attribute__((ext_vector_type(4)));
+
+__global__ __launch_bounds__(256) void wino_filter_kernel(const float* w, float* U, int c, int k, int Rp, int Cp, int bwd) {
+  const int total = Rp * Cp;
+  for (int i = blockIdx.x * 256 + threadIdx.x; i < total; i += gridDim.x * 256) {
+    const int col = i % Cp, row = i / Cp;
+    const int rows = bwd ? k : c, cols = bwd ? c : k;
+    float g[3][3];
+#pragma unroll
+    for (int r = 0; r < 3; ++r)
+#pragma unroll
+      for (int s = 0; s < 3; ++s) {
+        float v = 0.f;
+        if (row < rows && col < cols)
+          v = bwd ? w[((size_t)((2 - r) * 3 + (2 - s)) * c + col) * k + row] : w[((size_t)(r * 3 + s) * c + row) * k + col];
+        g[r][s] = v;
+      }
+    float t[4][3];
+#pragma unroll
+    for (int s = 0; s < 3; ++s) {
+      const float a = g[0][s] + g[2][s];
+      t[0][s] = g[0][s];
+      t[1][s] = (a + g[1][s]) * 0.5f;
+      t[2][s] = (a - g[1][s]) * 0.5f;
+      t[3][s] = g[2][s];
+    }
+#pragma unroll
+    for (int a4 = 0; a4 < 4; ++a4) {
+      const float a = t[a4][0] + t[a4][2];
+      const float u[4] = {t[a4][0], (a + t[a4][1]) * 0.5f, (a - t[a4][1]) * 0.5f, t[a4][2]};
+#pragma unroll
+      for (int b4 = 0; b4 < 4; ++b4) U[(size_t)(a4 * 4 + b4) * total + i] = u[b4];
+    }
+  }
+}
+
+template <bool VEC>
+__global__ __launch_bounds__(256) void wino_input_kernel(const float* __restrict__ x, float* __restrict__ V, int h, int w, int c, int ld,
+                                                         int th, int tw, int pad_t, int pad_l, int Cp, size_t T) {
+  const int cqn = Cp / 4;
+  const size_t total = T * (size_t)cqn;
+  for (size_t i = (size_t)blockIdx.x * 256 + threadIdx.x; i < total; i += (size_t)gridDim.x * 256) {
+    const int cq = (int)(i % cqn);
+    const size_t t = i / cqn;
+    const int tj = (int)(t % tw), ti = (int)((t / tw) % th);
+    const size_t img = t / ((size_t)tw * th);
+    const int y0 = 2 * ti - pad_t, x0 = 2 * tj - pad_l;
+    f4 d[4][4];
+#pragma unroll
+    for (int a = 0; a < 4; ++a)
+#pragma unroll
+      for (int b = 0; b < 4; ++b) {
+        f4 v = f4(0.f);
+        const int yy = y0 + a, xx = x0 + b;
+        if (yy >= 0 && yy < h && xx >= 0 && xx < w) {
+          const float* src = x + ((img * h + yy) * w + xx) * (size_t)ld + cq * 4;
+          if (VEC) {
+            v = *reinterpret_cast<const f4*>(src);
+          } else {
+#pragma unroll
+            for (int e = 0; e < 4; ++e)
+              if (cq * 4 + e < c) v[e] = src[e];
+          }
+        }
+        d[a][b] = v;
+      }
+    f4 r[4][4];
+#pragma unroll
+    for (int b = 0; b < 4; ++b) {
+      r[0][b] = d[0][b] - d[2][b];
+      r[1][b] = d[1][b] + d[2][b];
+      r[2][b] = d[2][b] - d[1][b];
+      r[3][b] = d[1][b] - d[3][b];
+    }
+#pragma unroll
+    for (int a = 0; a < 4; ++a) {
+      const f4 v[4] = {r[a][0] - r[a][2], r[a][1] + r[a][2], r[a][2] - r[a][1], r[a][1] - r[a][3]};
+#pragma unroll
+      for (int b = 0; b < 4; ++b) *reinterpret_cast<f4*>(V + ((size_t)(a * 4 + b) * T + t) * Cp + cq * 4) = v[b];
+    }
+  }
+}
+
+template <bool VEC>
+__global__ __launch_bounds__(256) void wino_output_kernel(const float* __restrict__ M, float* __restrict__ out, const float* __restrict__ bias,
+                                                          const float* __restrict__ mask, int act, int oh, int ow, int ncols, int ld,
+                                                          int th, int tw, int Np, size_t T) {
+  const int cqn = Np / 4;
+  const size_t total = T * (size_t)cqn;
+  for (size_t i = (size_t)blockIdx.x * 256 + threadIdx.x; i < total; i += (size_t)gridDim.x * 256) {
+    const int cq = (int)(i % cqn);
+    const size_t t = i / cqn;
+    const int tj = (int)(t % tw), ti = (int)((t / tw) % th);
+    const size_t img = t / ((size_t)tw * th);
+    f4 m[4][4];
+#pragma unroll
+    for (int a = 0; a < 4; ++a)
+#pragma unroll
+      for (int b = 0; b < 4; ++b) m[a][b] = *reinterpret_cast<const f4*>(M + ((size_t)(a * 4 + b) * T + t) * Np + cq * 4);
+    f4 r[2][4];
+#pragma unroll
+    for (int b = 0; b < 4; ++b) {
+      r[0][b] = (m[0][b] + m[1][b]) + m[2][b];
+      r[1][b] = (m[1][b] - m[2][b]) - m[3][b];
+    }
+    f4 bv = f4(0.f);
+    if (bias) {
+#pragma unroll
+      for (int e = 0; e < 4; ++e)
+        if (cq * 4 + e < ncols) bv[e] = bias[cq * 4 + e];
+    }
+#pragma unroll
+    for (int a = 0; a < 2; ++a) {
+      const f4 y2[2] = {(r[a][0] + r[a][1]) + r[a][2], (r[a][1] - r[a][2]) - r[a][3]};
+#pragma unroll
+      for (int b = 0; b < 2; ++b) {
+        const int oy = 2 * ti + a, ox = 2 * tj + b;
+        if (oy >= oh || ox >= ow) continue;
+        const size_t o = ((img * oh + oy) * ow + ox) * (size_t)ld + cq * 4;
+        f4 v = y2[b] + bv;
+        if (act == EPI_RELU) {
+#pragma unroll
+          for (int e = 0; e < 4; ++e) v[e] = fmaxf(v[e], 0.f);
+        } else if (act == EPI_SIGMOID) {
+#pragma unroll
+          for (int e = 0; e < 4; ++e) v[e] = 1.f / (1.f + expf(-v[e]));
+        }
+        if (VEC) {
+          if (mask) {
+            const f4 y = *reinterpret_cast<const f4*>(mask + o);
+#pragma unroll
+            for (int e = 0; e < 4; ++e) v[e] = apply_act_grad(v[e], y[e], EPI_RELU, 1.f);
+          }
+          *reinterpret_cast<f4*>(out + o) = v;
+        } else {
+#pragma unroll
+          for (int e = 0; e < 4; ++e)
+            if (cq * 4 + e < ncols) out[o + e] = mask ? apply_act_grad(v[e], mask[o + e], EPI_RELU, 1.f) : v[e];
+        }
+      }
+    }
+  }
+}
+
+constexpr int kBM = 128, kBN = 128, kWavesM = 4, kNWaves = 8, kBK = 32;
+__global__ __launch_bounds__(64 * kNWaves, 2 * kNWaves / 4) void wino_gemm_kernel(const IgemmParams p, const size_t batch_a,
+                                                                                   const size_t batch_b, const size_t batch_c) {
+  IgemmParams q = p;
+  q.A = p.A + (size_t)blockIdx.y * batch_a;
+  q.B = p.B + (size_t)blockIdx.y * batch_b;
+  q.C = p.C + (size_t)blockIdx.y * batch_c;
+  igemm_body<MODE_FWD, kBM, kBN, kWavesM, kNWaves, kBK, 4, 4>(q, gridDim.x, blockIdx.x);
+}
+
+WinoGeom wino_geom(const a3d_conv_desc* d, bool bwd) {
+  WinoGeom g{};
+  g.oh = bwd ? d->h : d->ho;
+  g.ow = bwd ? d->w : d->wo;
+  g.th = (g.oh + 1) / 2;
+  g.tw = (g.ow + 1) / 2;
+  g.T = (size_t)d->n * g.th * g.tw;
+  g.K = bwd ? d->k : d->c;
+  g.N = bwd ? d->c : d->k;
+  g.Kp = (g.K + 3) / 4 * 4;
+  g.Np = (g.N + 3) / 4 * 4;
+  auto up = [](size_t b) { return (b + 255) / 256 * 256; };
+  g.v_bytes = up((size_t)16 * g.T * g.Kp * 4);
+  g.m_bytes = up((size_t)16 * g.T * g.Np * 4);
+  g.u_bytes = up((size_t)16 * g.Kp * g.Np * 4);
+  return g;
+}
+
+bool wino_applicable(const a3d_conv_desc* d) {
+  if (d->precision != A3D_PREC_F32_WINOGRAD || d->storage || d->r != 3 || d->s != 3 || d->stride != 1 || d->pad_t > 1 || d->pad_l > 1)
+    return false;
+  for (bool bwd : {false, true}) {
+    const WinoGeom g = wino_geom(d, bwd);
+    if ((double)g.T * std::max(g.Kp, g.Np) * 4.0 >= 2147483647.0 || g.T >= ((size_t)1 << 30)) return false;
+  }
+  return true;
+}
+
+int wino_filter(const a3d_conv_desc* d, bool bwd, const float* w, float* U, hipStream_t st) {
+  const WinoGeom g = wino_geom(d, bwd);
+  clear_stale_error();
+  hipLaunchKernelGGL(wino_filter_kernel, dim3(grid_for((size_t)g.Kp * g.Np)), dim3(256), 0, st, w, U, d->c, d->k, g.Kp, g.Np, bwd ? 1 : 0);
+  return check_launch("wino_filter");
+}
+
+int wino_input(const a3d_conv_desc* d, bool bwd, const float* src, float* V, hipStream_t st) {
+  const WinoGeom g = wino_geom(d, bwd);
+  const int h = bwd ? d->ho : d->h, w = bwd ? d->wo : d->w, ld = bwd ? d->ldy : d->ldx;
+  const int pad_t = bwd ? 2 - d->pad_t : d->pad_t, pad_l = bwd ? 2 - d->pad_l : d->pad_l;
+  const bool vec = g.K % 4 == 0 && ld % 4 == 0 && aligned16(src);
+  const dim3 grid(grid_for(g.T * (size_t)(g.Kp / 4), 256, 1u << 20)), block(256);
+  clear_stale_error();
+  if (vec) hipLaunchKernelGGL(wino_input_kernel<true>, grid, block, 0, st, src, V, h, w, g.K, ld, g.th, g.tw, pad_t, pad_l, g.Kp, g.T);
+  else hipLaunchKernelGGL(wino_input_kernel<false>, grid, block, 0, st, src, V, h, w, g.K, ld, g.th, g.tw, pad_t, pad_l, g.Kp, g.T);
+  return check_launch("wino_input");
+}
+
+int wino_output(const a3d_conv_desc* d, bool bwd, const float* M, float* out, const float* bias, const float* mask, int act,
+                hipStream_t st) {
+  const WinoGeom g = wino_geom(d, bwd);
+  const int ld = bwd ? d->ldx : d->ldy;
+  const bool vec = g.N % 4 == 0 && ld % 4 == 0 && aligned16(out) && aligned16(mask);
+  const dim3 grid(grid_for(g.T * (size_t)(g.Np / 4), 256, 1u << 20)), block(256);
+  clear_stale_error();
+  if (vec) hipLaunchKernelGGL(wino_output_kernel<true>, grid, block, 0, st, M, out, bias, mask, act, g.oh, g.ow, g.N, ld, g.th, g.tw, g.Np, g.T);
+  else hipLaunchKernelGGL(wino_output_kernel<false>, grid, block, 0, st, M, out, bias, mask, act, g.oh, g.ow, g.N, ld, g.th, g.tw, g.Np, g.T);
+  return check_launch("wino_output");
+}
+
+a3d_timing_record wino_record(int mode, const WinoGeom& g) {
+  return timing_record(mode, A3D_PREC_F32, kBM, kBN, kWavesM, kNWaves, kBK, 4, 4, 0, (int)(16 * g.T), g.N, g.K);
+}
+
+int wino_gemm(IgemmParams& p, const WinoGeom& g, hipStream_t st) {
+  using Cfg = IgemmCfg<MODE_FWD, kBM, kBN, kWavesM, kNWaves, kBK, 4, 4>;
+  static bool attr_done[64] = {};
+  int dev = 0;
+  (void)hipGetDevice(&dev);
+  if (dev < 0 || dev >= 64 || !attr_done[dev]) {
+    hipError_t e = hipFuncSetAttribute(reinterpret_cast<const void*>(wino_gemm_kernel), hipFuncAttributeMaxDynamicSharedMemorySize,
+                                       (int)Cfg::LDS_BYTES);
+    if (e != hipSuccess) return set_error(A3D_ELAUNCH, "hipFuncSetAttribute: %s", hipGetErrorString(e));
+    if (dev >= 0 && dev < 64) attr_done[dev] = true;
+  }
+  p.splitk = 1;
+  p.ktiles_per_split = (p.K + kBK - 1) / kBK;
+  p.tiles_m = (p.M + kBM - 1) / kBM;
+  p.tiles_n = (p.N + kBN - 1) / kBN;
+  p.slab = (size_t)p.M * p.N;
+  clear_stale_error();
+  hipLaunchKernelGGL(wino_gemm_kernel, dim3((unsigned)(p.tiles_m * p.tiles_n), 16), dim3(Cfg::NT), Cfg::LDS_BYTES, st, p,
+                     g.T * (size_t)g.Kp, (size_t)g.Kp * g.Np, g.T * (size_t)g.Np);
+  return check_launch("wino_gemm");
+}
+
+}
diff --git a/ann3depth_amd/models.py b/ann3depth_amd/models.py
--- a/ann3depth_amd/models.py
+++ b/ann3depth_amd/models.py
@@ -8,6 +8,7 @@
 import torch
 
 from . import _lib, augment as augment_, ops
+from ._lib import ConvDesc
 
 NET_H, NET_W = 228, 304
 OUT_H, OUT_W = 55, 74
@@ -239,6 +240,13 @@
             'fine/second/conv2d': D(B, OUT_H, OUT_W, 64, 64, 5, 5, 1, 'SAME'),
             'fine/third': D(B, OUT_H, OUT_W, 64, 1, 5, 5, 1, 'SAME'),
         }
+        self.d_wino = {}
+        if precision == 'fp32' and dev.type == 'cuda':
+            for n in self.WINO_LAYERS:
+                d = self.d[n]
+                if d.n * -(-d.ho // 2) * -(-d.wo // 2) >= self.WINO_MIN_TILES:
+                    e = self.d_wino[n] = ConvDesc.from_buffer_copy(d)
+                    e.precision = ops.PREC['fp32w']
         self.d_few = {}
         if dev.type == 'cuda':
             few_prec = 'bf16' if self.bf16s else 'fp32'
@@ -278,6 +286,8 @@
                 pass
 
     SHARE_CU = ('fine/first/conv2d', 'fine/second/conv2d')
+    WINO_LAYERS = ('coarse/conv/conv2d_2', 'coarse/conv/conv2d_3')
+    WINO_MIN_TILES = 504
 
     def _desc(self, name, which):
         d = self.d[name]
@@ -296,12 +306,12 @@
             return self.wcopy[name]
         return self._v(name + '/kernel')
 
-    def _prepared(self, key, desc, w):
+    def _prepared(self, key, desc, w, which='fwd'):
         if self.device.type != 'cuda':
             return desc, w
         pf = self._prep.get(key)
         if pf is None:
-            pf = self._prep[key] = ops.PreparedFilter(desc, self.device)
+            pf = self._prep[key] = ops.PreparedFilter(desc, self.device, which)
             pf.source = w
             if pf.ok:
                 pf.refresh(w)
@@ -718,7 +728,10 @@
         return not self.keep_dense_grads and self.groups['CoarseDense'].frozen()
 
     def _bwd_data(self, name, dz, dx, relu_mask=None):
-        ops.conv2d_bwd_data(self._desc(name, 'bwd_d'), dz, self._w(name, 'bwd_d'), dx, relu_mask=relu_mask)
+        d, w = self._desc(name, 'bwd_d'), self._w(name, 'bwd_d')
+        if name in self.d_wino:
+            d, w = self._prepared((name, 'bwd_d', 'fp32w'), self.d_wino[name], w, 'bwd_d')
+        ops.conv2d_bwd_data(d, dz, w, dx, relu_mask=relu_mask)
 
     def _bwd_filter(self, name, x, dz):
         if name in self.d:
diff --git a/ann3depth_amd/ops.py b/ann3depth_amd/ops.py
--- a/ann3depth_amd/ops.py
+++ b/ann3depth_amd/ops.py
@@ -6,7 +6,7 @@
 from ._lib import ConvDesc, check
 
 ACT = {None: 0, 'relu': 1, 'sigmoid': 2}
-PREC = {'fp32': 0, 'f32': 0, 'bf16x3': 1, 'bf16': 2}
+PREC = {'fp32': 0, 'f32': 0, 'bf16x3': 1, 'bf16': 2, 'fp32w': 3}
 
 
 def _ptr(t):
@@ -64,9 +64,10 @@
 
 class PreparedFilter:
 
-    def __init__(self, desc, device):
+    def __init__(self, desc, device, which='fwd'):
         lib = _lib.load()
-        nbytes = lib.a3d_conv2d_fwd_prepared_filter_bytes(ctypes.byref(desc))
+        self.stem = {'fwd': 'a3d_conv2d_fwd', 'bwd_d': 'a3dw_conv2d_bwd_data'}[which]
+        nbytes = getattr(lib, self.stem + '_prepared_filter_bytes')(ctypes.byref(desc))
         self.ok = nbytes > 0
         self.desc = desc
         if self.ok:
@@ -75,8 +76,8 @@
             self.desc_prepared.hints = desc.hints | HINT_W_PREPARED
 
     def refresh(self, w):
-        check(_lib.load().a3d_conv2d_fwd_prepare_filter(ctypes.byref(self.desc), _ptr(w), _ptr(self.buf), self.buf.numel(), _stream()),
-              'a3d_conv2d_fwd_prepare_filter')
+        name = self.stem + '_prepare_filter'
+        check(getattr(_lib.load(), name)(ctypes.byref(self.desc), _ptr(w), _ptr(self.buf), self.buf.numel(), _stream()), name)
 
 
 def conv_desc(n, h, w, c, k, r, s, stride, padding, ldx=None, ldy=None, precision='fp32', storage=0, hints=0):
diff --git a/include/a3d.h b/include/a3d.h
--- a/include/a3d.h
+++ b/include/a3d.h
@@ -42,6 +42,7 @@
 #define A3D_PREC_F32 0
 #define A3D_PREC_BF16X3 1
 #define A3D_PREC_BF16 2
+#define A3D_PREC_F32_WINOGRAD 3
 
 const char* a3d_version(void);
 int a3d_last_error(char* buf, size_t len);
diff --git a/include/a3d_wino.h b/include/a3d_wino.h
--- /dev/null
+++ b/include/a3d_wino.h
@@ -0,0 +1,16 @@
+#ifndef A3D_WINO_H_
+#define A3D_WINO_H_
+
+#include "a3d.h"
+
+#ifdef __cplusplus
+extern "C" {
+#endif
+
+size_t a3dw_conv2d_bwd_data_prepared_filter_bytes(const a3d_conv_desc* d);
+int a3dw_conv2d_bwd_data_prepare_filter(const a3d_conv_desc* d, const float* w, void* prepared, size_t prepared_bytes, void* stream);
+
+#ifdef __cplusplus
+}
+#endif
+#endif
```

Result: faster. 11870 (median of 6 runs) (+3.3%).
